# zertovitch/zip-ada

Hardware: AMD Instinct MI355X
Metric: Deflate encode MB/s (Deflate_3; stream bit-exact with the CPU restatement of the reference, Ada parity unpinned) (higher is better)
Workload: dtype u8

## Files before the change

__graft_entry__.py:

```python
import importlib
import os
import subprocess
import sys

ROOT = os.path.dirname(os.path.abspath(__file__))
if ROOT not in sys.path:
    sys.path.insert(0, ROOT)


def build():
    env = dict(os.environ)
    subprocess.run(["make", "-C", os.path.join(ROOT, "zip-ada_amd", "csrc"), "-j4"], check=True, env=env)
    subprocess.run(["make", "-C", os.path.join(ROOT, "oracle")], check=True, env=env)
    subprocess.run(["g++", "-O2", "-std=c++17", "-fPIC", "-shared", "-o",
                    os.path.join(ROOT, "tests", "hostcheck", "libzada_hostcheck.so"),
                    os.path.join(ROOT, "tests", "hostcheck", "hostcheck.cpp")], check=True)
    subprocess.run(["gcc", "-O2", "-fPIC", "-shared", "-o", os.path.join(ROOT, "tests", "hostcheck", "libzada_mix.so"),
                    os.path.join(ROOT, "zip-ada_amd", "csrc", "silesia_mix.c"), "-lm"], check=True)
    subprocess.run(["gcc", "-O2", "-fPIC", "-shared", "-o", os.path.join(ROOT, "tests", "crypt", "libcrypt_model.so"),
                    os.path.join(ROOT, "tests", "crypt", "crypt_model.c")], check=True)
    subprocess.run(["g++", "-O2", "-std=c++17", "-fPIC", "-shared", "-o", os.path.join(ROOT, "tests", "inflate", "libinflate_host.so"),
                    os.path.join(ROOT, "tests", "inflate", "inflate_host.cpp")], check=True)
    subprocess.run(["g++", "-O2", "-std=c++17", "-fPIC", "-shared", "-o", os.path.join(ROOT, "tests", "inflate_par", "libinflate_par_host.so"),
                    os.path.join(ROOT, "tests", "inflate_par", "inflate_par_host.cpp")], check=True)
    subprocess.run(["g++", "-O2", "-std=c++17", "-fPIC", "-shared", "-o", os.path.join(ROOT, "tests", "bunzip2", "libbunzip2_host.so"),
                    os.path.join(ROOT, "tests", "bunzip2", "bunzip2_host.cpp")], check=True)
    subprocess.run(["g++", "-O2", "-std=c++17", "-fPIC", "-shared", "-o", os.path.join(ROOT, "tests", "unlzma", "libunlzma_host.so"),
                    os.path.join(ROOT, "tests", "unlzma", "unlzma_host.cpp")], check=True)
    subprocess.run(["g++", "-O2", "-std=c++17", "-fPIC", "-shared", "-o", os.path.join(ROOT, "tests", "unzip", "libunzip_plan_host.so"),
                    os.path.join(ROOT, "tests", "unzip", "unzip_plan_host.cpp")], check=True)
    subprocess.run(["g++", "-O2", "-std=c++17", "-fPIC", "-shared", "-o", os.path.join(ROOT, "tests", "zip", "libzip_plan_host.so"),
                    os.path.join(ROOT, "tests", "zip", "zip_plan_host.cpp")], check=True)
    subprocess.run(["g++", "-O2", "-std=c++17", "-fPIC", "-shared", "-o", os.path.join(ROOT, "tests", "zip", "libzip_plan_ex_host.so"),
                    os.path.join(ROOT, "tests", "zip", "zip_plan_ex_host.cpp")], check=True)
    subprocess.run(["g++", "-O2", "-std=c++17", "-fPIC", "-shared", "-o", os.path.join(ROOT, "tests", "rezip", "librezip_plan_host.so"),
                    os.path.join(ROOT, "tests", "rezip", "rezip_plan_host.cpp")], check=True)
    subprocess.run(["g++", "-O2", "-std=c++17", "-fPIC", "-shared", "-o", os.path.join(ROOT, "tests", "find", "libfind_plan_host.so"),
                    os.path.join(ROOT, "tests", "find", "find_plan_host.cpp")], check=True)
    subprocess.run(["g++", "-O2", "-std=c++17", "-fPIC", "-shared", "-o", os.path.join(ROOT, "tests", "trained", "libtrained_host.so"),
                    os.path.join(ROOT, "tests", "trained", "trained_host.cpp")], check=True)
    for name in ("shrink_model", "reduce_model"):
        subprocess.run(["gcc", "-O2", "-fPIC", "-shared", "-o", os.path.join(ROOT, "tests", "legacy", "lib%s.so" % name),
                        os.path.join(ROOT, "tests", "legacy", name + ".c")], check=True)
    subprocess.run(["g++", "-O2", "-std=c++17", "-fPIC", "-shared", "-o", os.path.join(ROOT, "tests", "unlegacy", "libunlegacy_host.so"),
                    os.path.join(ROOT, "tests", "unlegacy", "unlegacy_host.cpp")], check=True)
    subprocess.run(["g++", "-O2", "-std=c++17", "-fPIC", "-shared", "-o", os.path.join(ROOT, "tests", "unlegacy", "libunzip_legacy_plan_host.so"),
                    os.path.join(ROOT, "tests", "unlegacy", "unzip_legacy_plan_host.cpp")], check=True)
    subprocess.run(["gcc", "-O2", "-fPIC", "-shared", "-o", os.path.join(ROOT, "tests", "unlegacy", "libunlegacy_model.so"),
                    os.path.join(ROOT, "tests", "unlegacy", "unlegacy_model.c")], check=True)
    subprocess.run(["g++", "-O2", "-std=c++17", "-fPIC", "-shared", "-o", os.path.join(ROOT, "tests", "zip_legacy", "libzip_legacy_plan_host.so"),
                    os.path.join(ROOT, "tests", "zip_legacy", "zip_legacy_plan_host.cpp")], check=True)
    za = importlib.import_module("zip-ada_amd")
    za.load_library()
    return None


def smoke():
    import zlib
    sys.path.insert(0, os.path.join(ROOT, "tests"))
    from _common import oracle_deflate
    za = importlib.import_module("zip-ada_amd")
    enc = za.Encoder(0)
    for n, mask in ((1 << 20, 0x1F), (1 << 20, 1), (1, 1), (0, 1)):
        d = za.silesia_mix(n, class_mask=mask).tobytes()
        for method in (za.Method.Deflate_3, za.Method.Deflate_1):
            rc, ref, crc = oracle_deflate(d, method)
            try:
                out, c2 = enc.deflate(d, method)
                rc2 = 0
            except za.CompressionInefficient:
                rc2, out, c2 = 1, b"", crc
            assert rc == rc2, (n, method, rc, rc2)
            if rc == 0:
                assert out == ref, "GPU stream differs from the oracle (n=%d method=%d)" % (n, method)
                assert zlib.decompress(out, -15) == d
            assert c2 == crc
    datas = [za.silesia_mix(k, class_mask=1).tobytes() for k in (0, 1, 5000, 40000, 70000)]
    for d, (rc2, out, c2) in zip(datas, enc.deflate_batch(datas, za.Method.Deflate_1)):
        rc, ref, crc = oracle_deflate(d, za.Method.Deflate_1)
        assert rc == rc2 and crc == c2 and (rc != 0 or out == ref), "batch entry differs from the oracle (n=%d)" % len(d)
    packed = [(d, out, c2) for d, (rc2, out, c2) in zip(datas, enc.deflate_batch(datas, za.Method.Deflate_1)) if rc2 == 0]
    assert len(packed) >= 3
    for (d, out, c2), (rc, back, _, used, reg) in zip(packed, enc.inflate_batch([p[1] for p in packed], [len(p[0]) for p in packed])):
        assert rc == 0 and back == d and used == len(out) and reg == c2, "inflated entry differs from the input (n=%d)" % len(d)
    d = za.silesia_mix(1 << 20).tobytes()
    s, c2 = enc.deflate(d, za.Method.Deflate_3)
    enc.set_knob("inflate_par_chunk_kib", 16)
    assert enc.inflate_par(s, len(d)) == (d, len(s), c2), "stream read back on many waves differs from the input"
    assert enc.inflate_par_last()["fell_back"] == 0 and enc.inflate_par_last()["live_chunks"] >= 2, "the stream did not run on many waves"
    enc.set_knob("inflate_par_chunk_kib", 64)
    import bz2
    from _bzip2 import oracle_encode
    d = za.silesia_mix(1 << 20).tobytes()
    ref, blocks = oracle_encode(d, 2)
    rc, out, crc = enc.bzip2(d, 14)
    assert rc == 0 and out == ref and enc.bz2_last_blocks() == blocks, "GPU BZip2 stream differs from the oracle"
    assert bz2.decompress(out) == d and (crc ^ 0xFFFFFFFF) == zlib.crc32(d)
    back, used, reg = enc.bunzip2(out, len(d))
    assert back == d and used == len(out) and reg == crc, "BZip2 stream read back differs from the input"
    from _lzmah import oracle_lzma, lzma_decode
    datas = [d[i * 6000:i * 6000 + k] for i, k in enumerate((0, 1, 300, 6000, 6000, 6000))]
    for e, got in zip(datas, enc.lzma_batch(datas, 18)):
        assert got == oracle_lzma(e, 18), "GPU LZMA payload differs from the oracle (n=%d)" % len(e)
        assert lzma_decode(got[1], 4) == e
    packed = enc.lzma_batch(datas, 18)
    for e, p, (rc, back, _, used, reg) in zip(datas, packed, enc.unlzma_batch([p[1] for p in packed], [len(e) for e in datas], True)):
        assert rc == 0 and back == e and used == len(p[1]) and reg == p[2], "LZMA entry read back differs from the input (n=%d)" % len(e)
    enc.set_knob("lzma_chunk", 3000)
    seen = []
    assert enc.lzma(d[:20000], 18, feedback=lambda pct: seen.append(pct) and False) == oracle_lzma(d[:20000], 18), "chunked LZMA stream differs from the oracle"
    assert seen[0] == 0 and seen[-1] == 100 and seen == sorted(seen) and len(seen) > 5
    from _crypt import compress_data_pw
    h11 = bytes(range(1, 12))
    for e in (d[:300000], d[:1], b""):
        want, crc, zt, _ = compress_data_pw(e, za.Method.Deflate_3, "smoke", h11)
        assert enc.compress_data(e, za.Method.Deflate_3, password="smoke", header=h11) == (want, crc, zt), "encrypted payload differs from the model (n=%d)" % len(e)
    import io
    import zipfile
    b = io.BytesIO()
    with zipfile.ZipFile(b, "w", zipfile.ZIP_DEFLATED) as z:
        z.writestr("a.txt", d[:40000])
        z.writestr("b.txt", b"x" + d[1000:1020].lower())
    r = za.FindZip(enc).find(b.getvalue(), b" X" + d[1000:1008])
    assert [(e[4], e[1], e[2]) for e in r.entries] == [(b"a.txt", 0, 40000), (b"b.txt", 1, 8)] and r.damaged == 0, "Find_Zip on the device differs from the host's search"
    from _trained import message_of, stub_of
    tc = za.TrainedCompression(enc, d[:20000])
    msgs = tc.encode([d[20000:23000], b""])
    assert tc.stub == stub_of(d[:20000]) and msgs == [message_of(d[:20000], e, tc.skip) for e in (d[20000:23000], b"")], "trained messages differ from the oracle"
    td = za.TrainedCompression.for_decoding(enc, tc.stub, tc.skip, tc.trainer_len)
    assert td.decode(msgs, [3000, 0]) == [d[20000:23000], b""] and td.info()["forked"] == 2, "trained messages read back differ from the data"
    tc.close(); td.close()
    from _legacy import model_result
    datas = [d[:6000], d[6000:6300] * 20, d[:1], b""]
    assert enc.shrink_batch(datas) == [(r, s if r == 0 else None, c) for r, s, c in (model_result(e, za.Method.Shrink_1) for e in datas)], "Shrink_1 batch differs from the model"
    assert enc.reduce_batch(datas, za.Method.Reduce_4) == [(r, s if r == 0 else None, c) for r, s, c in (model_result(e, za.Method.Reduce_4) for e in datas)], "Reduce_4 batch differs from the model"
    packed = [(e, s, 1) for e, (r, s, _) in zip(datas, enc.shrink_batch(datas)) if r == 0] + [(e, s, 5) for e, (r, s, _) in zip(datas, enc.reduce_batch(datas, za.Method.Reduce_4)) if r == 0]
    assert len(packed) >= 3
    for (e, s, m), (rc, back, _, used, reg) in zip(packed, enc.unlegacy_batch([p[1] for p in packed], [len(p[0]) for p in packed], [p[2] for p in packed])):
        assert rc == 0 and back == e and used == len(s) and reg == zlib.crc32(e) ^ 0xFFFFFFFF, "Shrink / Reduce entry read back differs from the input (n=%d)" % len(e)
    enc.close()
    print("smoke ok")
    return None


if __name__ == "__main__":
    build()
    if len(sys.argv) > 1 and sys.argv[1] == "smoke":
        smoke()
```

zip-ada_amd/csrc/zada_api.hip:

```cpp
#include <hip/hip_runtime.h>
#include <stdint.h>
#include <stdio.h>
#include <string.h>
#include <algorithm>
#include <new>
#include <atomic>
#include <mutex>
#include <condition_variable>
#include <functional>
#include <thread>
#include "../../include/zada.h"
#include "zada_internal.h"
#include "zada_bt4.h"
#include "zada_legacy.h"

struct zada_ctx { zada::Ctx c; };

namespace zada {

thread_local std::string *tls_err = nullptr;
int hip_check(Ctx *c, hipError_t e, const char *what) {
  if (e == hipSuccess) return 0;
  char buf[256];
  snprintf(buf, sizeof buf, "%s: %s", what, hipGetErrorString(e));
  if (tls_err) *tls_err = buf; else c->err = buf;
  return ZADA_E_HIP_;
}

void Ctx::tbegin() {
  marks.clear();
  timing.clear();
}
void Ctx::tmark(const char *name) {
  if (!timing_on) return;
  size_t k = marks.size();
  if (k >= ev_pool.size()) { hipEvent_t e; hipEventCreate(&e); ev_pool.push_back(e); }
  hipEventRecord(ev_pool[k], stream);
  marks.push_back({name, ev_pool[k]});
}
void Ctx::tend() {
  if (!timing_on || marks.empty()) return;
  hipEventSynchronize(marks.back().second);
  for (size_t i = 1; i < marks.size(); i++) {
    float ms = 0;
    hipEventElapsedTime(&ms, marks[i - 1].second, marks[i].second);
    timing.push_back({marks[i].first, ms});
  }
  timing.push_back({"#demand_rounds", (float)demand_rounds});
  timing.push_back({"#splice_rounds", (float)parse_rounds});
  timing.push_back({"#bt4_reruns", (float)bt4_reruns});
  timing.push_back({"#lzma_launches", (float)lzma_launches});
  timing.push_back({"#bt4_pool_grown", (float)bt4_pool_grown});
  timing.push_back({"#atoms_grown", (float)atoms_grown});
  timing.push_back({"#fix_grown", (float)fix_grown});
}

#ifndef ZADA_COPY_LANES
#define ZADA_COPY_LANES 4
#endif
constexpr int ARR_LANES = ZADA_COPY_LANES;
struct Arrival {
  Ctx *c; const uint8_t *src; uint8_t *dst; uint64_t n; int T;
  std::vector<std::thread> th;
  std::mutex m; std::condition_variable cv;
  uint64_t sent[ARR_LANES] = {};
  bool failed = false;
  void lane(int t) {
    hipSetDevice(c->device);
    uint64_t i = 0;
    for (uint64_t o = (uint64_t)t * STAGE_BYTES; o < n; o += (uint64_t)T * STAGE_BYTES, i++) {
      const int b = 2 * t + (int)(i & 1);
      if (i >= 2) hipEventSynchronize(c->ev_stage[b]);
      const uint64_t k = n - o < STAGE_BYTES ? n - o : STAGE_BYTES;
      memcpy(c->stage[b], src + o, k);
      const bool ok = hipMemcpyAsync(dst + o, c->stage[b], k, hipMemcpyHostToDevice, c->stream_in[t]) == hipSuccess &&
                      hipEventRecord(c->ev_stage[b], c->stream_in[t]) == hipSuccess;
      std::lock_guard<std::mutex> g(m);
      if (!ok || hipEventRecord(c->ev_in[t], c->stream_in[t]) != hipSuccess) failed = true;
      sent[t]++;
      cv.notify_all();
    }
  }
  void start() { for (int t = 0; t < T; t++) th.emplace_back([this, t] { lane(t); }); }
  void join() { for (auto &x : th) if (x.joinable()) x.join(); th.clear(); }
  ~Arrival() { join(); }
};
static bool ensure_arrival_streams(Ctx *c) {
  for (int t = 0; t < ARR_LANES; t++) {
    if (c->stream_in[t]) continue;
    if (hipStreamCreateWithFlags(&c->stream_in[t], hipStreamNonBlocking) != hipSuccess || hipEventCreateWithFlags(&c->ev_in[t], hipEventDisableTiming) != hipSuccess) {
      (void)hipGetLastError();
      return false;
    }
  }
  return true;
}
static int arrival_order(Ctx *c, hipStream_t st, uint64_t upto) {
  Arrival *A = (Arrival *)c->arrival;
  if (!A) return 0;
  if (upto > A->n) upto = A->n;
  const uint64_t P = (upto + STAGE_BYTES - 1) / STAGE_BYTES;
  std::unique_lock<std::mutex> g(A->m);
  for (int t = 0; t < A->T; t++) {
    const uint64_t want = P > (uint64_t)t ? (P - 1 - t) / A->T + 1 : 0;
    if (want == 0) continue;
    A->cv.wait(g, [&] { return A->sent[t] >= want || A->failed; });
    if (A->failed) { c->err = "host to device copy of the input"; return ZADA_E_HIP; }
    if (hipStreamWaitEvent(st, c->ev_in[t], 0) != hipSuccess) { c->err = "hipStreamWaitEvent (input arrival)"; return ZADA_E_HIP; }
  }
  return 0;
}


template <typename T>
static int dalloc(Ctx *c, std::vector<void *> &group, T **p, uint64_t count) {
  void *q = nullptr;
  hipError_t e = hipMalloc(&q, count * sizeof(T) + 256);
  if (e != hipSuccess) { hip_check(c, e, "hipMalloc"); (void)hipGetLastError(); return ZADA_E_NOMEM; }
  group.push_back(q);
  *p = (T *)q;
  return 0;
}

static void free_group(std::vector<void *> &group) {
  for (void *p : group) hipFree(p);
  group.clear();
}

int ensure_lz_workspace(Ctx *c, uint64_t nbuf) {
  Workspace &W = c->ws;
  if (W.cap_n >= nbuf && W.cap_n > 0) return 0;
  hipStreamSynchronize(c->stream); hipStreamSynchronize(c->stream2);
  free_group(W.allocs);
  W.cap_n = 0;
  uint64_t cap = nbuf < (1u << 20) ? (1u << 20) : nbuf;
  cap = (cap + 65535) & ~65535ull;
  const uint64_t nch = cap / PCHUNK + 2, nseg32 = cap / 32768 + 2;
  int rc = 0;
#define A(ptr, cnt) if (!rc) rc = dalloc(c, W.allocs, &W.ptr, (cnt))
#define A2(ptr, cnt) if (!rc) rc = dalloc(c, W.allocs, &ptr, (cnt))
  A(in, cap + IN_PAD + 64);
  static_assert(NLEVELS >= 2, "spec_tok shares the block of ltails[0], S3, T3, bsc3: the first level's tails table must be dead when the first parse starts");
  {
    const uint64_t b_tails0 = nseg32 * 65536 * 2, b_s3 = nseg32 * 32768 * 2, b_t3 = nseg32 * 32768, b_bsc = nseg32 * 32768 * 4, b_spec = nch * (uint64_t)PTOK_STRIDE * 4;
    const uint64_t links = b_tails0 + b_s3 + b_t3 + b_bsc + 1024, bytes = links > b_spec ? links : b_spec;
    uint8_t *blk = nullptr;
    A2(blk, bytes);
    if (!rc) {
      uint8_t *q = blk;
      W.ltails[0] = (uint16_t *)q; q += b_tails0 + 256;
      W.S3 = (uint16_t *)q; q += b_s3 + 256;
      W.bsc3 = (uint32_t *)q; q += b_bsc + 256;
      W.T3 = q;
      W.spec_tok = (uint32_t *)blk;
    }
  }
  for (int l = 0; l < NLEVELS; l++) { A(lprev[l], cap + IN_PAD); if (l > 0) A(ltails[l], nseg32 * 65536); }
  A(segmax, nseg32 + 16); A(heavy, nseg32 * 2048);
  A(bloom4, nseg32 * 4096);
  W.cd_cap = cap / 256 + 4096; A(cd_list, W.cd_cap + W.cd_cap / 4);
  for (int l = 0; l < NLEVELS; l++) A(dplane[l], cap + 64);
  A(dlim, cap + 64); A(dlim_bits, cap / 32 + 64);
  A(M, cap + 64);
  A(SK, nseg32 * 32768); A(idxK, cap + 64); A(cntK, cap + 64);
  W.fix_stride = c->knob_fix_stride > 0 ? (uint32_t)c->knob_fix_stride : FIX_STRIDE_SMALL;
  if (W.fix_stride > PTOK_STRIDE) W.fix_stride = PTOK_STRIDE;
  A(fix_tok, nch * W.fix_stride);
  A(spec_cnt, nch); A(fix_cnt, nch); A(take_from, nch); A(start_pos, nch); A(counts, nch); A(offsets, nch);
  A(scan_sums, nch / 1024 + 1024);
  A(Fbits, cap / 32 + 64); A(Lbits, cap / 32 + 64);
  A(spec_exits, nch); A(true_exits, nch);
  A(dirty[0], nch + 64); A(dirty[1], nch + 64);
  A(n_changed, 16);
  A(blk_demand, cap / 4096 + 64); A(dbits, cap / 32 + 4096); A(n_demand, 16); A(chg, nch + 64);
  A(dbg, 128);
#undef A
#undef A2
  if (rc) { free_group(W.allocs); return rc; }
  W.cap_n = cap;
  hipMemsetAsync(W.dbg, 0, 128 * 8, c->stream);
  return hip_check(c, hipStreamSynchronize(c->stream), "workspace init");
}

int ensure_entropy_workspace(Ctx *c, uint64_t atoms, uint64_t flushes, uint64_t out_bytes) {
  Workspace &W = c->ws;
  const EntropyRoom room = sizing_entropy_room(EntropyRequest{atoms, out_bytes});
  if (out_bytes < atoms) out_bytes = atoms;
  if (W.cap_atoms >= atoms && W.cap_flush >= flushes && W.cap_atoms > 0 && W.cap_out >= room.out_need) return 0;
  hipStreamSynchronize(c->stream); hipStreamSynchronize(c->stream2);
  free_group(W.en_allocs);
  W.cap_atoms = 0; W.cap_flush = 0;
  const uint64_t cap = room.cap_atoms;
  const uint64_t nflush = (cap / FLUSH > flushes ? cap / FLUSH : flushes + flushes / 4) + 3;
  int rc = 0;
#define A(ptr, cnt) if (!rc) rc = dalloc(c, W.en_allocs, &W.ptr, (cnt))
  A(ea_atoms, LB_CAP + cap + LA_CAP + 64); A(ea_apos, LB_CAP + cap + LA_CAP + 64);
  A(descr, nflush * SLOTS * 320);
  A(seg_nblk, nflush); A(seg_cut, nflush * MAXBLK_PER_SEG); A(seg_blk_off, nflush);
  A(cut_trace, nflush * SLOTS * 2);
  W.cap_blocks = nflush * MAXBLK_PER_SEG;
  A(blocks, W.cap_blocks);
  A(binfo, W.cap_blocks);
  A(emit, W.cap_blocks);
  A(chrec, W.cap_blocks * 16 + 16);
  A(chw, W.cap_blocks * 4 + 16); A(piece_base, W.cap_blocks + 16);
  A(codes, (W.cap_blocks + 2) * 320);
  W.cap_pieces = cap / 2048 + W.cap_blocks + 64;
  A(pieces, W.cap_pieces);
  W.cap_tiles = cap / TILE + W.cap_blocks + 64;
  A(tile_block, W.cap_tiles); A(tile_bitpos, W.cap_tiles); A(tile_bits, W.cap_tiles);
  A(blk_entry, W.cap_blocks + 16);
  A(chooser, 1); A(carry, 2);
  A(scan2, nflush / 1024 + 1024); A(total2, 16);
  W.cap_out = room.cap_out;
  A(out, W.cap_out);
#undef A
  if (!rc) rc = ensure_crc_workspace(c, out_bytes > cap ? out_bytes : cap);
  if (rc) { free_group(W.en_allocs); return rc; }
  W.cap_atoms = cap; W.cap_flush = nflush - 3;
  return 0;
}

int ensure_crc_workspace(Ctx *c, uint64_t n) {
  Workspace &W = c->ws;
  if (W.cap_crc >= n && W.cap_crc > 0) return 0;
  hipStreamSynchronize(c->stream); hipStreamSynchronize(c->stream2);
  free_group(W.crc_allocs);
  W.cap_crc = 0;
  const uint64_t cap = ((n < (1u << 20) ? (1u << 20) : n) + 65535) & ~65535ull;
  int rc = 0;
  for (int l = 0; l < 4 && !rc; l++) rc = dalloc(c, W.crc_allocs, &W.crc_lvl[l], (cap >> (4 * l)) / CRC_SUB + 64);
  if (!rc) rc = dalloc(c, W.crc_allocs, &W.crc_mat, 128);
  W.crc_mat_ready = false;
  if (rc) { free_group(W.crc_allocs); return rc; }
  W.cap_crc = cap;
  return 0;
}

int ensure_batch_workspace(Ctx *c, uint64_t entries, uint64_t fslots, uint64_t segs) {
  Workspace &W = c->ws;
  if (W.cap_ent >= entries && W.cap_fslots >= fslots && W.cap_bseg >= segs && W.cap_ent > 0) return 0;
  hipStreamSynchronize(c->stream); hipStreamSynchronize(c->stream2);
  free_group(W.bt_allocs);
  W.cap_ent = W.cap_fslots = W.cap_bseg = 0;
  const uint64_t ce = entries + entries / 4 + 1024, cf = fslots + fslots / 4 + 1024, cs = segs + segs / 4 + 1024;
  int rc = 0;
#define A(ptr, cnt) if (!rc) rc = dalloc(c, W.bt_allocs, &W.ptr, (cnt))
  A(ftab, cf); A(ent_out, ce);
  A(ent_chunk0, ce + 1); A(ent_fl0, ce + 1); A(ent_start, ce + 1); A(ent_len, ce + 1); A(ent_bytes, ce + 1); A(ent_base, ce + 1); A(ent_crc, ce + 1);
  A(segend, cs + 1);
#undef A
  if (rc) { free_group(W.bt_allocs); return rc; }
  W.cap_ent = ce; W.cap_fslots = cf; W.cap_bseg = cs;
  return 0;
}

static int ensure_rin(Ctx *c, uint64_t n) {
  Workspace &W = c->ws;
  if (W.cap_rin >= n && W.rin_own) return 0;
  hipStreamSynchronize(c->stream); hipStreamSynchronize(c->stream2);
  if (W.rin_own) hipFree(W.rin_own);
  W.rin_own = nullptr; W.cap_rin = 0;
  const uint64_t cap = ((n < (1u << 20) ? (1u << 20) : n) + 65535) & ~65535ull;
  if (hipMalloc((void **)&W.rin_own, cap + 256) != hipSuccess) { (void)hipGetLastError(); c->err = "hipMalloc (input)"; return ZADA_E_NOMEM; }
  W.cap_rin = cap;
  return 0;
}

static void free_workspace(Ctx *c) {
  free_group(c->ws.allocs); free_group(c->ws.en_allocs); free_group(c->ws.bt_allocs); free_group(c->ws.crc_allocs);
  if (c->ws.rin_own) hipFree(c->ws.rin_own);
  c->ws = Workspace();
}

constexpr int CRC_WG = 64, CRC_ROW = CRC_SUB + 16;
__global__ void __launch_bounds__(CRC_WG) k_crc_chunks(const uint8_t *__restrict__ in, uint64_t n, uint32_t nsub, uint32_t *__restrict__ sub) {
  __shared__ uint32_t tab[256];
  __shared__ __attribute__((aligned(16))) uint8_t rows[CRC_WG * CRC_ROW];
  for (uint32_t t = threadIdx.x; t < 256; t += CRC_WG) {
    uint32_t l = t;
    for (int b = 0; b < 8; b++) l = (l & 1) ? (l >> 1) ^ 0xEDB88320u : l >> 1;
    tab[t] = l;
  }
  const uint64_t tile0 = (uint64_t)blockIdx.x * CRC_WG * CRC_SUB;
  {
    const uint4 *src = (const uint4 *)(in + tile0);
    const uint64_t left = tile0 < n ? n - tile0 : 0, words = left / 16;
#pragma unroll
    for (int j = 0; j < CRC_SUB / 16; j++) {
      const uint32_t wq = j * CRC_WG + threadIdx.x;
      if (wq < words) *(uint4 *)(rows + (wq >> 4) * CRC_ROW + (wq & 15) * 16) = src[wq];
    }
    if (words < (uint64_t)CRC_WG * CRC_SUB / 16 && threadIdx.x < (left & 15)) {
      const uint64_t o = words * 16 + threadIdx.x;
      rows[(o / CRC_SUB) * CRC_ROW + (o % CRC_SUB)] = in[tile0 + o];
    }
  }
  __syncthreads();
  uint32_t k = blockIdx.x * CRC_WG + threadIdx.x;
  if (k >= nsub) return;
  uint64_t p0 = (uint64_t)k * CRC_SUB, p1 = p0 + CRC_SUB < n ? p0 + CRC_SUB : n;
  uint32_t r = 0;
  const uint8_t *row = rows + threadIdx.x * CRC_ROW;
  const uint4 *w = (const uint4 *)row;
  uint64_t len = p1 - p0, i = 0;
  for (; i + 16 <= len; i += 16) {
    const uint4 v = w[i >> 4];
    const uint32_t xs[4] = {v.x, v.y, v.z, v.w};
#pragma unroll
    for (int q = 0; q < 4; q++) {
      uint32_t x = xs[q];
      r = tab[(r ^ x) & 0xFF] ^ (r >> 8); x >>= 8;
      r = tab[(r ^ x) & 0xFF] ^ (r >> 8); x >>= 8;
      r = tab[(r ^ x) & 0xFF] ^ (r >> 8); x >>= 8;
      r = tab[(r ^ x) & 0xFF] ^ (r >> 8);
    }
  }
  for (; i < len; i++) r = tab[(r ^ row[i]) & 0xFF] ^ (r >> 8);
  sub[k] = r;
}

__global__ void __launch_bounds__(256) k_crc_fold(const uint32_t *__restrict__ src, uint32_t ngroups, const uint32_t *__restrict__ mat,
                                                  uint32_t *__restrict__ out) {
  __shared__ uint32_t m[32];
  if (threadIdx.x < 32) m[threadIdx.x] = mat[threadIdx.x];
  __syncthreads();
  uint32_t k = blockIdx.x * 256 + threadIdx.x;
  if (k >= ngroups) return;
  uint32_t r = 0;
  for (uint32_t j = 0; j < 16; j++) {
    uint32_t s = 0, v = r;
    for (int b = 0; v; b++, v >>= 1) if (v & 1) s ^= m[b];
    r = s ^ src[k * 16 + j];
  }
  out[k] = r;
}

static void gf2_square(uint32_t *sq, const uint32_t *m) {
  for (int i = 0; i < 32; i++) { uint32_t v = m[i], s = 0; for (int j = 0; v; j++, v >>= 1) if (v & 1) s ^= m[j]; sq[i] = s; }
}
static uint32_t gf2_apply(const uint32_t *m, uint32_t v) { uint32_t s = 0; for (int j = 0; v; j++, v >>= 1) if (v & 1) s ^= m[j]; return s; }
static void zero_advance_matrix(uint64_t len, uint32_t *out) {
  uint32_t op[32], tmp[32], acc[32];
  op[0] = 0xEDB88320u;
  for (int i = 1; i < 32; i++) op[i] = 1u << (i - 1);
  for (int i = 0; i < 32; i++) acc[i] = 1u << i;
  uint64_t bits = len * 8;
  while (bits) {
    if (bits & 1) { for (int i = 0; i < 32; i++) tmp[i] = gf2_apply(op, acc[i]); memcpy(acc, tmp, sizeof acc); }
    gf2_square(tmp, op); memcpy(op, tmp, sizeof op);
    bits >>= 1;
  }
  memcpy(out, acc, sizeof acc);
}

constexpr int CRC_NLEV = 4;
static uint32_t crc_M[CRC_NLEV][32];
int crc_launch(Ctx *c, const uint8_t *d_in, uint64_t n) {
  if (n == 0) return 0;
  Workspace &W = c->ws;
  CrcPending &P = c->crc;
  static std::once_flag mats;
  std::call_once(mats, [] { for (int l = 0; l < CRC_NLEV; l++) zero_advance_matrix((uint64_t)CRC_SUB << (4 * l), crc_M[l]); });
  hipStream_t s2 = c->stream2;
  hipEventRecord(c->ev_input, c->stream);
  hipStreamWaitEvent(s2, c->ev_input, 0);
  P.nsub = (uint32_t)((n + CRC_SUB - 1) / CRC_SUB);
  P.nfull0 = (uint32_t)(n / CRC_SUB);
  P.cnt[0] = P.nfull0;
  for (int l = 1; l < CRC_NLEV; l++) P.cnt[l] = P.cnt[l - 1] / 16;
  if (!W.crc_mat_ready) { hipMemcpyAsync(W.crc_mat, crc_M, sizeof(uint32_t) * 32 * (CRC_NLEV - 1), hipMemcpyHostToDevice, s2); W.crc_mat_ready = true; }
  hipLaunchKernelGGL(k_crc_chunks, dim3((P.nsub + CRC_WG - 1) / CRC_WG), dim3(CRC_WG), 0, s2, d_in, n, P.nsub, W.crc_lvl[0]);
  for (int l = 1; l < CRC_NLEV; l++)
    if (P.cnt[l]) hipLaunchKernelGGL(k_crc_fold, dim3((P.cnt[l] + 255) / 256), dim3(256), 0, s2, W.crc_lvl[l - 1], P.cnt[l], W.crc_mat + 32 * (l - 1), W.crc_lvl[l]);
  if (P.cnt[CRC_NLEV - 1] > CRC_HOST_TOP) { c->err = "crc: too many top-level values"; return ZADA_E_TOO_LARGE; }
  if (P.cnt[CRC_NLEV - 1]) hipMemcpyAsync(c->crc_host, W.crc_lvl[CRC_NLEV - 1], (size_t)P.cnt[CRC_NLEV - 1] * 4, hipMemcpyDeviceToHost, s2);
  for (int l = 0; l < CRC_NLEV - 1; l++) {
    const uint32_t first = P.cnt[l + 1] * 16;
    P.nrest[l] = (l == 0 ? P.nsub : P.cnt[l]) - first;
    if (P.nrest[l]) hipMemcpyAsync(c->crc_host + CRC_HOST_TOP + 16 * l, W.crc_lvl[l] + first, (size_t)P.nrest[l] * 4, hipMemcpyDeviceToHost, s2);
  }
  return hip_check(c, hipGetLastError(), "crc launch");
}

int crc_finish(Ctx *c, uint64_t n, uint32_t *crc_inout) {
  if (n == 0) return 0;
  constexpr int NLEV = CRC_NLEV;
  CrcPending &P = c->crc;
  const uint32_t *cnt = P.cnt, *nrest = P.nrest;
  const uint32_t nfull0 = P.nfull0;
  const uint32_t *top = c->crc_host; const uint32_t (*rest)[16] = (const uint32_t (*)[16])(c->crc_host + CRC_HOST_TOP); auto &M = crc_M;
  if (hip_check(c, hipStreamSynchronize(c->stream2), "crc")) return ZADA_E_HIP_;
  uint32_t r = *crc_inout;
  for (uint32_t k = 0; k < cnt[NLEV - 1]; k++) r = gf2_apply(M[NLEV - 1], r) ^ top[k];
  for (int l = NLEV - 2; l >= 0; l--) {
    for (uint32_t j = 0; j < nrest[l]; j++) {
      if (l == 0 && cnt[1] * 16 + j == nfull0) {
        uint32_t Ml[32];
        zero_advance_matrix(n - (uint64_t)nfull0 * CRC_SUB, Ml);
        r = gf2_apply(Ml, r) ^ rest[0][j];
      } else r = gf2_apply(M[l], r) ^ rest[l][j];
    }
  }
  *crc_inout = r;
  return 0;
}

static int method_level(int method) {
  switch (method) {
    case ZADA_DEFLATE_FIXED: return 4;
    case ZADA_DEFLATE_0: return 0;
    case ZADA_DEFLATE_1: return 6;
    case ZADA_DEFLATE_2: return 8;
    case ZADA_DEFLATE_3: return 10;
    case ZADA_DEFLATE_R: return RICH_LEVEL;
    default: return -1;
  }
}

uint32_t crc32_advance(uint32_t reg, uint64_t len) {
  if (len == 0) return reg;
  uint32_t m[32];
  zero_advance_matrix(len, m);
  return gf2_apply(m, reg);
}

constexpr uint32_t SHARD_HALO = 32768, SHARD_TAIL = 4096;
constexpr uint64_t RANGE_POST = 1u << 20;

__global__ void __launch_bounds__(256) k_copy16(const uint4 *__restrict__ src, uint4 *__restrict__ dst, uint64_t n16) {
  const uint64_t stride = (uint64_t)gridDim.x * 256;
  uint64_t i = (uint64_t)blockIdx.x * 256 + threadIdx.x;
  for (; i + 3 * stride < n16; i += 4 * stride) {
    const uint4 a = src[i], b = src[i + stride], c = src[i + 2 * stride], d = src[i + 3 * stride];
    dst[i] = a; dst[i + stride] = b; dst[i + 2 * stride] = c; dst[i + 3 * stride] = d;
  }
  for (; i < n16; i += stride) dst[i] = src[i];
}

struct PadArgs { uint8_t *in_end; uint32_t n_in; uint16_t *link_end[NLEVELS]; };
__global__ void k_pad_init(PadArgs a) {
  for (uint32_t i = threadIdx.x; i < a.n_in; i += blockDim.x) a.in_end[i] = 0;
  for (int l = 0; l < NLEVELS; l++)
    if (threadIdx.x < 64) a.link_end[l][threadIdx.x] = 0;
}

int range_open(Ctx *c, int method, const uint8_t *rin, uint64_t stream_size, uint64_t lo, uint64_t n, uint64_t pre, uint64_t post, uint64_t carry_atoms = 0) {
  const int level = method_level(method);
  if (level < 0) { c->err = "unsupported method"; return ZADA_E_INVALID; }
  if (lo + n > stream_size || n > stream_size) { c->err = "range outside the stream"; return ZADA_E_INVALID; }
  const uint64_t behind = stream_size - (lo + n);
  const bool pre_ok = pre == (lo > 0 ? SHARD_HALO : 0u) || (carry_atoms > 0 && pre <= lo && pre >= SHARD_HALO && (pre % 32768) == 0) || (lo > 0 && pre == 65536);
  if (!pre_ok || post != (behind < RANGE_POST ? behind : RANGE_POST) ||
      (lo % 65536) != 0 || (behind > 0 && (n % 65536) != 0) || (behind > 0 && n == 0)) {
    c->err = "range: boundaries must be multiples of 64 KiB, with 32 KiB before and min(1 MiB, rest of the stream) behind it resident";
    return ZADA_E_INVALID;
  }
  if (pre + n + post >= (1ull << 32) - (1ull << 26)) { c->err = "range too large for one context (4 GiB - 64 MiB): split the stream into ranges"; return ZADA_E_TOO_LARGE; }
  if (((uintptr_t)rin & 15) != 0) { c->err = "range: input must be 16-byte aligned"; return ZADA_E_INVALID; }
  const uint64_t shard = (uint64_t)c->knob_shard_kib << 10;
  const EntropyRequest want = sizing_range_request(n, sizing_pct(c->knob_atoms_pct), carry_atoms);
  int rc = ensure_entropy_workspace(c, want.atoms, 0, want.out_bytes);
  if (!rc) rc = ensure_lz_workspace(c, (n < shard ? n : shard) + SHARD_HALO + SHARD_TAIL);
  if (rc) return rc;
  Range &R = c->rg;
  R = Range();
// ... 2050 lines not shown
```

zip-ada_amd/csrc/zada_internal.h:

```cpp
#pragma once
#ifndef ZADA_NLEVELS
#define ZADA_NLEVELS 2
#endif
#include <hip/hip_runtime.h>
#include <stdint.h>
#include <string>
#include <functional>
#include <vector>
#include "zada_logic.h"
#include "zada_sizing.h"

struct zada_inflate_par_info;

namespace zada {

constexpr int ZADA_E_HIP_ = -3;

#ifndef ZADA_PCHUNK
#define ZADA_PCHUNK 512
#endif
constexpr uint32_t PCHUNK = ZADA_PCHUNK;
static_assert(PCHUNK > 258, "k_fix_forward: a 258-byte step crosses at most one chunk boundary");
constexpr uint32_t PTOK_STRIDE = PCHUNK + 640;
constexpr uint32_t FIX_STRIDE_SMALL = 128;
constexpr uint32_t CRC_CHUNK = 4096, CRC_SUB = 256;
constexpr uint64_t IN_PAD = 1024;

constexpr int NLEVELS = ZADA_NLEVELS;
struct LevelPtrs { uint16_t *prev[NLEVELS]; uint16_t *tails[NLEVELS]; };
struct RunPtrs { uint16_t *S, *idx, *cnt; };
struct DistPlanes {
  uint16_t *d[NLEVELS]; uint32_t *dlim; uint32_t *dlim_bits;
  __device__ __forceinline__ uint32_t limits(uint64_t p) const { return ((dlim_bits[p >> 5] >> (p & 31)) & 1u) ? dlim[p] : 0xFFFFFFFFu; }
};

constexpr uint32_t FLUSH = 65536;
static_assert(FLUSH == SIZING_FLUSH, "zada_sizing.h books the carried atoms by the flush");
constexpr uint32_t MIN_STEP = 750, HALF_SLIDER = 2048, SLIDER = 4096;
constexpr uint32_t SLOTS = 88;
constexpr uint32_t MAXBLK_PER_SEG = 86;
constexpr uint32_t TILE = 2048;

enum { FMT_STORED = 0, FMT_FIXED = 1, FMT_DYN1 = 2, FMT_DYN2 = 3, FMT_RECYCLE = 4 };
enum { BT_STORED = 0, BT_FIXED = 1, BT_DYNAMIC = 2, BT_RESERVED = 3 };

struct BlockRange { uint32_t first, count; uint32_t last_flush; uint32_t pad; };

struct BlockInfo {
  uint32_t stats[320];
  uint8_t bl1[320], bl2[320];
  uint8_t truc1[20], truc2[20];
  uint32_t hdr1_bits, hdr2_bits;
  uint64_t fixed_data, dyn1_data, dyn2_data;
  uint32_t bytes;
  uint32_t stored_possible;
};

struct EmitRec {
  uint64_t hdr_bitpos;
  uint64_t data_bitpos;
  uint64_t cost_bits;
  uint32_t fmt;
  int32_t code_block;
  uint32_t code_variant;
  uint32_t tile_base;
  uint64_t pre_pos;
  uint32_t pre_eob;
  uint32_t pre_flags;
};
constexpr int32_t CODE_FIXED = -1, CODE_CARRIED = -2;

struct StoredPiece { uint64_t dst_byte; uint32_t src_byte, nbytes; };

struct ChooserCarry {
  uint64_t pos;
  int32_t last_type, block_to_finish, last_marked;
  uint32_t cur_eob;
  uint8_t bl[320];
  uint32_t pad[2];
};
static_assert(sizeof(ChooserCarry) == 352, "ChooserCarry is exchanged between ranks as bytes");

struct ChooserOut {
  uint64_t total_bits;
  uint32_t n_tiles, n_pieces, n_blocks, overflow;
};

struct FlushGeom {
  uint32_t F, to;
  uint32_t gj;
  uint32_t flags;
  uint32_t end_byte;
  uint32_t entry;
  uint32_t pad[2];
};
enum { FG_EMPTY = 1, FG_LAST_PARTIAL = 2, FG_ENTRY_FIRST = 4, FG_ENTRY_LAST = 8 };
enum { BR_LAST_FLUSH = 1, BR_ENTRY_FIRST = 2, BR_ENTRY_LAST = 4 };
struct EntOut {
  uint64_t bits;
  uint32_t eob;
  uint32_t fake;
};

struct EntropyView {
  const FlushGeom *ftab;
  const uint32_t *atoms, *apos;
  uint32_t foff;
  uint32_t nflush;
  uint32_t lvalid;
  uint32_t stream_final;
  uint64_t j0;
};

constexpr uint32_t LB_CAP = HALF_SLIDER, LA_CAP = FLUSH;

struct Workspace {
  uint64_t cap_n = 0;
  uint8_t *in = nullptr;
  uint16_t *lprev[NLEVELS] = {}, *ltails[NLEVELS] = {};
  uint16_t *S3 = nullptr; uint8_t *T3 = nullptr; uint32_t *bsc3 = nullptr;
  uint32_t *segmax = nullptr;
  uint16_t *heavy = nullptr;
  uint32_t *bloom4 = nullptr;
  uint32_t *cd_list = nullptr; uint64_t cd_cap = 0;
  uint16_t *dplane[NLEVELS] = {}; uint32_t *dlim = nullptr, *dlim_bits = nullptr;
  uint16_t *SK = nullptr, *idxK = nullptr, *cntK = nullptr;
  MatchPair *M = nullptr;
  uint32_t *spec_tok = nullptr, *fix_tok = nullptr;
  uint32_t fix_stride = 0;
  uint32_t *spec_cnt = nullptr, *fix_cnt = nullptr, *take_from = nullptr, *start_pos = nullptr;
  uint32_t *counts = nullptr, *offsets = nullptr, *scan_sums = nullptr;
  uint32_t *Fbits = nullptr, *Lbits = nullptr;
  ExitState *spec_exits = nullptr, *true_exits = nullptr;
  uint8_t *dirty[2] = {nullptr, nullptr};
  uint32_t *n_changed = nullptr;
  uint32_t *blk_demand = nullptr, *n_demand = nullptr;
  uint32_t *dbits = nullptr;
  uint8_t *chg = nullptr;
  uint32_t *crc_lvl[4] = {nullptr, nullptr, nullptr, nullptr}, *crc_mat = nullptr;
  bool crc_mat_ready = false;
  uint64_t *dbg = nullptr;
  std::vector<void *> allocs;
  uint64_t cap_atoms = 0, cap_flush = 0;
  uint32_t *ea_atoms = nullptr, *ea_apos = nullptr;
  uint8_t *descr = nullptr;
  uint32_t *seg_nblk = nullptr, *seg_cut = nullptr, *seg_blk_off = nullptr;
  uint32_t *cut_trace = nullptr;
  BlockRange *blocks = nullptr;
  BlockInfo *binfo = nullptr;
  EmitRec *emit = nullptr;
  uint64_t *chrec = nullptr;
  uint64_t *chw = nullptr;
  uint32_t *piece_base = nullptr;
  uint32_t *codes = nullptr;
  StoredPiece *pieces = nullptr;
  uint32_t *tile_block = nullptr;
  uint64_t *tile_bitpos = nullptr;
  uint32_t *tile_bits = nullptr;
  ChooserOut *chooser = nullptr;
  ChooserCarry *carry = nullptr;
  uint32_t *scan2 = nullptr, *total2 = nullptr;
  uint64_t cap_blocks = 0, cap_tiles = 0, cap_pieces = 0;
  uint32_t *blk_entry = nullptr;
  std::vector<void *> en_allocs;
  std::vector<void *> crc_allocs;
  uint64_t cap_crc = 0;
  uint64_t cap_ent = 0, cap_fslots = 0, cap_bseg = 0;
  FlushGeom *ftab = nullptr;
  EntOut *ent_out = nullptr;
  uint32_t *ent_chunk0 = nullptr, *ent_fl0 = nullptr, *ent_start = nullptr, *ent_len = nullptr, *ent_bytes = nullptr, *ent_base = nullptr, *ent_crc = nullptr;
  uint32_t *segend = nullptr;
  std::vector<void *> bt_allocs;
  uint8_t *rin_own = nullptr; uint64_t cap_rin = 0;
  uint8_t *out = nullptr; uint64_t cap_out = 0;
};

struct GlobalState { uint64_t pos; uint32_t kind, pad; };
struct Range {
  bool open = false;
  bool batch = false;
  uint32_t n_entries = 0;
  const uint8_t *rin = nullptr;
  uint64_t lo = 0, pre = 0, n = 0, post = 0;
  bool first = true, last = true;
  int method = 0, level = 0;
  uint64_t T = 0;
  uint64_t T_carried = 0;
  uint64_t T_view = ~0ull;
  uint32_t n_lb = 0, n_la = 0;
  GlobalState exit{}, warm{};
  bool entry_known = true;
  uint64_t G = 0, T_total = 0;
  bool placed = false;
  uint32_t nflush = 0, foff = 0, nblocks = 0;
  uint64_t j0 = 0;
  uint64_t base_bits = 0;
  ChooserCarry carry_in{}, carry_out{};
  ChooserOut co{};
  bool analyzed = false, chosen = false;
  uint32_t crc_raw = 0;
};

constexpr uint32_t CRC_HOST_TOP = 4096;
struct CrcPending { uint32_t nsub = 0, nfull0 = 0, cnt[4] = {0, 0, 0, 0}, nrest[4] = {0, 0, 0, 0}; };

constexpr uint64_t STAGE_BYTES = 8ull << 20;
constexpr int MAX_COPY_LANES = 8;
struct Ctx {
  int device = 0;
  hipStream_t stream = nullptr, stream2 = nullptr;
  hipStream_t stream_in[MAX_COPY_LANES] = {};
  hipEvent_t ev_in[MAX_COPY_LANES] = {};
  void *arrival = nullptr;
  hipEvent_t ev_input = nullptr, ev_out = nullptr, ev_dlim = nullptr;
  CrcPending crc;
  uint32_t *crc_host = nullptr;
  uint8_t *stage[2 * MAX_COPY_LANES] = {};
  uint8_t *bstage = nullptr; uint64_t cap_bstage = 0;
  uint32_t *btab = nullptr; uint64_t cap_btab = 0;
  hipEvent_t ev_stage[2 * MAX_COPY_LANES] = {};
  Workspace ws;
  Range rg;
  std::string err;
  int parse_rounds = 0, demand_rounds = 0;
  int atoms_grown = 0, fix_grown = 0;
  bool lz_attrs_set = false;
  void *bz = nullptr;
  void *zc = nullptr;
  void *inf = nullptr;
  void *infp = nullptr;
  int knob_infp_chunk_kib = 64;
  int knob_infp_repair_pct = 25;
  int knob_infp_min_kib = 0;
  void *bzd = nullptr;
  void *ulz = nullptr;
  void *ulg = nullptr;
  void *uz = nullptr;
  void *zw = nullptr;
  void *rz = nullptr;
  void *fz = nullptr;
  void *lg = nullptr;
  int knob_reduce_group_mib = 4096;
  int knob_unzip_legacy = 0;
  int knob_zip_legacy = 0;
  int knob_unzip_piece = 14;
  void *lz_tab = nullptr; size_t cap_lz_tab = 0;
  void *lz_save = nullptr; size_t cap_lz_save = 0;
  void *lz_lit = nullptr; size_t cap_lz_lit = 0;
  bool lz_last_lit_hbm = false;
  int knob_lzma_lit_mib = 12288;
  int lzma_launches = 0;
  std::vector<uint8_t> lz_resume;
  bool lz_stopped = false;
  bool lz_run_stopped = false;
  uint64_t lz_last_n = 0, lz_last_out_off = 0;
  void *bt4 = nullptr;
  uint32_t bt4_buckets = 0, bt4_long = 0, bt4_overflow = 0;
  uint32_t bt4_pool_grown = 0;
  int knob_lzma_pool_fixed = 0;
  uint32_t bt4_reruns = 0;
  int knob_trained_fork = 1;
  int knob_lzma_waves = 0;
  int knob_lzma_segment = 0;
  int knob_lzma_pool = 0;
  std::vector<hipEvent_t> ev_pool;
  std::vector<std::pair<const char *, hipEvent_t>> marks;
  std::vector<std::pair<const char *, float>> timing;
  bool timing_on = true;
  uint32_t last_nblocks = 0;
  int knob_budget = -1;
  int knob_max_demand_rounds = 12;
  int knob_atoms_pct = 50;
  int knob_fix_stride = 0;
  int knob_cd_list_cap = 0;
  int knob_cd_filter = 1;
  int knob_exact_respec = 32768;
  int knob_bz_pipe_prio = 0;
  int knob_link_run = 0;
  int knob_inner_budget = 0;
  int knob_span_mib = 2048;
  int knob_batch_mib = 512;
  int knob_bunzip_batch_mib = 8192;
  int knob_bz_batch_mib = 256;
  int knob_bz_span_mib = 1024;
  int knob_bz_text_order = 1;
  int knob_bz_tail_pct = 0;
  int knob_bz_batch_melems = 768;
  int knob_bz_lists = -1;
  int knob_bz_pipeline = 1;
  int knob_bz_list_rows = 0;
  int knob_bz_split = 1;
  int knob_bz_small_wg = 1;
  int knob_lzma_dict = 0;
  int knob_lzma_chunk = 0;
  int knob_shard_kib = 1 << 20;
  void tmark(const char *name);
  void tbegin();
  void tend();
};

extern thread_local std::string *tls_err;
int hip_check(Ctx *c, hipError_t e, const char *what);
constexpr const char *ERR_OUTPUT_TOO_SMALL = "output buffer too small";
void bz2_destroy(Ctx *c);
void crypt_destroy(Ctx *c);
void inflate_destroy(Ctx *c);
int inflate_crc_entries(Ctx *c, uint32_t E, const uint64_t *out, const uint64_t *out_len, uint32_t *regs);
void inflate_par_destroy(Ctx *c);
int inflate_par_try(Ctx *c, int format, const void *d_in, uint64_t n_in, void *d_out, uint64_t cap, uint64_t *out_len, uint64_t *in_used, uint32_t *crc_inout);
void inflate_par_record(Ctx *c, ::zada_inflate_par_info *get, const ::zada_inflate_par_info *set);
void bunzip2_destroy(Ctx *c);
void unlzma_destroy(Ctx *c);
void unlegacy_destroy(Ctx *c);
void unzip_destroy(Ctx *c);
void zip_destroy(Ctx *c);
void rezip_destroy(Ctx *c);
void find_destroy(Ctx *c);
int unzip_store_entries(Ctx *c, uint32_t ns, const uint64_t *src, const uint64_t *dst, const uint64_t *len, uint32_t *crc);
struct ReaderJob { uint64_t in, out, n_in, cap; int32_t format; uint32_t eos; uint64_t lit_elems; int32_t index, pad; };
struct ReaderRes { int32_t rc; uint32_t crc; uint64_t out_len, in_used; };
int inflate_run_jobs(Ctx *c, uint32_t E, const ReaderJob *jobs, ReaderRes *res, bool *described);
int bunzip2_run_jobs(Ctx *c, uint32_t E, const ReaderJob *jobs, ReaderRes *res, bool *described);
int unlzma_run_jobs(Ctx *c, uint32_t E, const ReaderJob *jobs, ReaderRes *res, bool *described);
uint64_t unlzma_hbm_elems(const uint8_t *h9, uint64_t n_in);
int unlegacy_run_jobs(Ctx *c, uint32_t E, const ReaderJob *jobs, ReaderRes *res, bool *described);
struct UlzTrainedJob { uint64_t in, out, n_in, cap; };
struct UlzResult;
uint64_t unlzma_snap_bytes();
int unlzma_snap_info(const uint8_t *snap, uint64_t *in_pos, uint64_t *out_pos, uint64_t *lit_elems);
int unlzma_trained_launch(Ctx *c, const UlzTrainedJob *d_jobs, const uint32_t *d_order, uint32_t E, UlzResult *d_res, const void *d_start, void *d_stop, uint64_t stop_in);
int lzma_plain_stream(Ctx *c, const uint8_t *in, uint64_t n, uint8_t *out, uint64_t cap, uint64_t *out_len, uint32_t dictionary_size, bool end_marker);
void crypt_update_keys(uint32_t keys[3], uint8_t by);
uint8_t crypt_code(const uint32_t keys[3]);
constexpr uint64_t CRYPT_WAVE_MAX = 256u << 10;
int crypt_io(Ctx *c, uint64_t bytes, uint8_t **p);
int crypt_encode_device(Ctx *c, uint32_t keys[3], uint8_t *d_buf, uint64_t n);
struct ZcPlaceJob { uint64_t src, dst, len; uint32_t keys[3], pad; };
int crypt_encode_place(Ctx *c, uint32_t E, const ZcPlaceJob *jobs);
int crypt_encode_small(Ctx *c, const int *idx, uint32_t E, uint32_t (*keys)[3], uint8_t *const *buf, const uint64_t *n);
int bz2_encode_device(Ctx *c, int option, const uint8_t *d_in, uint64_t n, int64_t size_hint, uint8_t *d_out, uint64_t cap, uint64_t *out_len,
                      int (*fb)(int, void *), void *user);
uint64_t bz2_last_blocks(Ctx *c, uint64_t *dst, uint64_t cap_items);
int bz2_batch_encode(Ctx *c, int option, const uint8_t *d_arena, uint32_t E, const uint64_t *starts, const uint32_t *lens, uint8_t *h_out, uint64_t cap,
                     uint64_t *out_off, uint64_t *out_bytes, uint8_t **d_streams = nullptr);
int bz2_range_open(Ctx *c, int option, const uint8_t *d_buf, uint64_t buf_len, uint64_t buf_off, uint64_t stream_total, uint64_t start, uint64_t own_end,
                   uint64_t *next_start, uint64_t *nblocks);
int bz2_range_encode(Ctx *c);
uint64_t bz2_range_table(Ctx *c, uint64_t *tab, uint64_t cap_blocks);
int bz2_range_assemble(Ctx *c, const uint8_t *choice, uint64_t nblk, uint64_t bit_begin, int flags, uint32_t footer_crc, uint8_t *d_out, uint64_t cap, uint64_t *nbytes);
struct LzmaJob {
  uint64_t in_off, n;
  uint64_t tok_off, ntok;
  uint64_t out_off, cap;
  uint64_t verify;
  uint32_t sbs, hash4_size;
  int32_t level, zip_prefix;
  int32_t lc, lp, pb;
  int32_t lit_home;
  uint64_t lit_off;
};
struct Bt4Sets { const uint8_t *cnt; const uint16_t *sl; const uint32_t *sd; const uint16_t *ol; const uint32_t *od; };
int bt4_produce(Ctx *c, const std::vector<LzmaJob> &jobs, const uint8_t *d_arena, uint64_t arena_bytes, Bt4Sets *out, std::vector<uint32_t> *weights = nullptr,
                uint32_t seg_shift = 32, uint32_t *nseg = nullptr);
int bt4_walk_segment(Ctx *c, uint32_t k, hipStream_t st);
int bt4_segments_overflowed(Ctx *c, hipStream_t st, Bt4Sets *out = nullptr);
void bt4_destroy(Ctx *c);
uint32_t lzma_string_buffer_size(int level, uint64_t dictionary_size);
uint32_t lzma_hash4_size(uint32_t sbs);
int lzma_token_ranges(Ctx *c, uint32_t E, const uint32_t *d_apos, uint32_t T, const uint32_t *d_ent_start, LzmaJob *d_jobs);
int lzma_launch(Ctx *c, const LzmaJob *d_jobs, const uint32_t *d_order, uint32_t count, const uint8_t *d_in, const uint32_t *d_tok, uint8_t *d_out, const Bt4Sets &sets, uint64_t *d_result,
                uint8_t *d_save = nullptr, uint64_t budget = 0, uint64_t pos_cap = ~0ull, int waves = 1, int lit_home = 0, uint16_t *d_lit = nullptr);
uint64_t lzma_save_stride();
struct LzFork { const uint8_t *d_snap, *d_head; uint64_t head_len; const uint8_t *d_forked; };
int lzma_fork_fill(Ctx *c, const LzmaJob *d_jobs, uint32_t count, const uint8_t *d_forked, const uint8_t *d_snap, const uint8_t *d_head, uint64_t head_len, uint8_t *d_save,
                   uint8_t *d_out);
int lzma_fork_snapshot(Ctx *c, const uint8_t *d_in, uint64_t n, uint64_t pos_cap, uint32_t dictionary_size, uint8_t *d_out, uint64_t cap, uint8_t *d_snap, uint64_t *pos,
                       uint64_t *olen);
int lzma_save_info(const uint8_t *blob, uint64_t *pos, uint64_t *olen, uint64_t *n);
int lzma_save_fits(const uint8_t *blob, const LzmaJob &J);
int ensure_lz_workspace(Ctx *c, uint64_t nbuf);
int ensure_entropy_workspace(Ctx *c, uint64_t atoms, uint64_t flushes, uint64_t out_bytes = 0);
int ensure_crc_workspace(Ctx *c, uint64_t n);

struct ShardJob {
  uint64_t nbuf = 0;
  uint32_t tok_lo = 0, tok_hi = 0;
  bool final = false;
  bool entry_known = true;
  ExitState entry{0, SYNC_F};
  uint32_t *dst_atoms = nullptr, *dst_apos = nullptr;
  uint32_t apos_bias = 0;
  uint64_t cap_atoms = 0;
  std::function<int(uint64_t, uint32_t **, uint32_t **)> grow_atoms;
  const uint32_t *segend = nullptr;
  std::function<int(uint64_t)> need;
  uint64_t gpos = 0;
};
struct ShardResult { uint32_t ntok = 0; ExitState exit{0, SYNC_F}, warm{0, SYNC_F}; };
int lz_shard(Ctx *c, int level, const ShardJob &job, ShardResult *res);
constexpr int RICH_LEVEL = 11;
int rich_shard(Ctx *c, const ShardJob &job, ShardResult *res);

int ensure_batch_workspace(Ctx *c, uint64_t entries, uint64_t fslots, uint64_t segs);
struct BatchLayout { uint32_t E = 0, nseg = 0; uint64_t total = 0, nfs = 0; std::vector<uint32_t> start, len; };
int batch_layout(Ctx *c, uint32_t E, const uint64_t *n, const uint32_t *crc_in, BatchLayout &L);
void batch_segends_all(Ctx *c, const BatchLayout &L);
int batch_launch(Ctx *c, int method, const BatchLayout &L, uint64_t *obytes, uint32_t **h_bytes, uint32_t **h_base, uint32_t **h_crc);
int deflate_device_one(Ctx *c, int method, const void *d_in, uint64_t n, void *d_out, uint64_t cap, uint64_t *out_len, uint32_t *crc_inout);
int bzip2_device_one(Ctx *c, int method, const void *d_in, uint64_t n, void *d_out, uint64_t cap, uint64_t *out_len, uint32_t *crc_inout);
int lzma_device_one(Ctx *c, int method, const void *d_in, uint64_t n, void *d_out, uint64_t cap, uint64_t *out_len, uint32_t *crc_inout);
struct DevBatch {
  uint32_t E = 0;
  int kind = 0;
  uint64_t total = 0, ototal = 0, nfs = 0;
  uint8_t *d_in = nullptr, *d_out = nullptr;
  std::vector<uint64_t> start, off, bytes, cap;
  std::vector<uint32_t> len, reg;
  std::vector<uint8_t> refused;
  const LzFork *fork = nullptr;
};
int bzip2_batch_layout(Ctx *c, int method, uint32_t E, const uint64_t *n, const uint32_t *crc_in, DevBatch &D);
int bzip2_batch_launch(Ctx *c, int method, DevBatch &D, uint8_t *h_out, uint64_t h_cap);
int lzma_batch_layout(Ctx *c, int method, uint32_t E, const uint64_t *n, const uint32_t *crc_in, DevBatch &D);
int lzma_batch_launch(Ctx *c, int method, DevBatch &D);
int legacy_batch_layout(Ctx *c, uint32_t E, const uint64_t *n, const uint32_t *crc_in, DevBatch &D);
int legacy_batch_launch(Ctx *c, int method, DevBatch &D);
bool lzma_batch_refused(Ctx *c, const DevBatch &D);
int batch_geometry(Ctx *c, uint32_t E, const uint32_t *d_total_atoms);
int entropy_analyze(Ctx *c);
int entropy_choose(Ctx *c);
// ... 10 lines not shown
```

zip-ada_amd/csrc/zada_logic.h:

```cpp
#pragma once
#include <type_traits>
#include <stdint.h>

#if defined(__HIPCC__)
#define ZADA_HD __host__ __device__ __forceinline__
#else
#define ZADA_HD inline
#endif

namespace zada {

constexpr uint32_t TOK_MATCH = 0x80000000u;
ZADA_HD uint32_t tok_match(uint32_t len, uint32_t dist) { return TOK_MATCH | (len << 16) | dist; }
ZADA_HD bool tok_is_match(uint32_t t) { return (t & TOK_MATCH) != 0; }
ZADA_HD uint32_t tok_len(uint32_t t) { return tok_is_match(t) ? ((t >> 16) & 0x1FF) : 1u; }
ZADA_HD uint32_t tok_dist(uint32_t t) { return t & 0xFFFF; }

constexpr int MIN_MATCH = 3, MAX_MATCH = 258, MAX_DIST = 32506, TOO_FAR = 4096;
constexpr int WSIZE = 32768;

struct LzConfig { int good, lazy, nice, chain; };
ZADA_HD LzConfig lz_config(int level) {
  switch (level) {
    case 4: return {4, 4, 16, 16};
    case 5: return {8, 16, 32, 32};
    case 6: return {8, 16, 128, 128};
    case 7: return {8, 32, 128, 256};
    case 8: return {32, 128, 258, 1024};
    case 9: return {32, 258, 258, 4096};
    default: return {34, 258, 258, 4096};
  }
}

ZADA_HD int clz32(uint32_t x) {
#if defined(__HIP_DEVICE_COMPILE__)
  return __clz((int)x);
#else
  return x ? __builtin_clz(x) : 32;
#endif
}

ZADA_HD int len_symbol(int len) {
  if (len == 258) return 285;
  int l = len - 3;
  if (l < 8) return 257 + l;
  int k = 31 - clz32((uint32_t)l);
  return 257 + 4 * (k - 1) + ((l >> (k - 2)) & 3);
}
ZADA_HD int len_extra_bits(int len) {
  if (len == 258) return 0;
  int l = len - 3;
  if (l < 8) return 0;
  return 31 - clz32((uint32_t)l) - 2;
}
ZADA_HD uint32_t len_extra_val(int len) { int e = len_extra_bits(len); return (uint32_t)(len - 3) & ((1u << e) - 1); }
ZADA_HD int dist_symbol(int dist) {
  if (dist <= 4) return dist - 1;
  uint32_t d = (uint32_t)dist - 1;
  int k = 31 - clz32(d);
  return 2 * k + (int)((d >> (k - 1)) & 1);
}
ZADA_HD int dist_extra_bits(int dist) {
  if (dist <= 4) return 0;
  return 31 - clz32((uint32_t)dist - 1) - 1;
}
ZADA_HD uint32_t dist_extra_val(int dist) { int e = dist_extra_bits(dist); return ((uint32_t)dist - 1) & ((1u << e) - 1); }
ZADA_HD int litlen_sym_extra(int sym) { return (sym < 265 || sym == 285) ? 0 : (sym - 261) / 4; }
ZADA_HD int dist_sym_extra(int sym) { return sym < 4 ? 0 : (sym >> 1) - 1; }
ZADA_HD int fixed_litlen_bl(int i) { return i <= 143 ? 8 : i <= 255 ? 9 : i <= 279 ? 7 : 8; }

struct ParseState { uint32_t p; uint32_t avail; uint32_t mlen; uint32_t mdist; };

enum { SYNC_NONE = 0, SYNC_F = 1, SYNC_L = 2 };
ZADA_HD int sync_kind(const ParseState &s) { return !s.avail ? SYNC_F : (s.mlen == 2 ? SYNC_L : SYNC_NONE); }

ZADA_HD bool parse_need_quarter(const ParseState &s, const LzConfig &c) { return (int)s.mlen >= c.good; }
ZADA_HD bool parse_searches(const ParseState &s, const LzConfig &c, uint64_t la) { return la >= 3 && (int)s.mlen < c.lazy; }

ZADA_HD uint32_t parse_step(ParseState &s, uint32_t mfq, bool searched, uint32_t byte_before) {
  const uint32_t L0 = s.mlen, pd = s.mdist;
  bool improved = false;
  uint32_t ml = 2, md = s.mdist;
  if (searched) {
    uint32_t len = mfq >> 16, dist = mfq & 0xFFFF;
    if (len > L0) { improved = true; ml = len; md = dist; if (ml == 3 && dist > (uint32_t)TOO_FAR) ml = 2; }
  }
  if (L0 >= 3 && !improved) {
    uint32_t t = tok_match(L0, pd);
    s.p += L0 - 1; s.avail = 0; s.mlen = 2; s.mdist = 0;
    return t;
  }
  s.mlen = ml; s.mdist = md; s.p += 1;
  if (s.avail) return byte_before;
  s.avail = 1;
  return 0xFFFFFFFFu;
}


struct MatchPair { uint32_t full, quarter; };
constexpr uint32_t M_GUESS = 0x80000000u, M_DEMAND = 0x40000000u, M_BYSPEC = 0x20000000u, M_HAVEQ = 0x10000000u, M_VALUE = 0x01FFFFFFu;
constexpr uint32_t M_BEAT_SHIFT = 25, M_BEAT_MAX = 127;
struct NoGuess { ZADA_HD void operator()(uint32_t, uint32_t, uint32_t, uint32_t) const {} };
struct ParseIO { const uint8_t *in; uint64_t n; const MatchPair *M; LzConfig cfg; const uint32_t *segend; };
struct Layout { const uint32_t *segend; uint64_t n; };
struct ExitState { uint32_t pos, kind; };

struct BitmapWriter {
  uint32_t *bits; uint64_t word; uint32_t acc;
  ZADA_HD void init(uint32_t *b, uint64_t first) { bits = b; acc = 0; word = first; }
  ZADA_HD void set(uint64_t p) {
    uint64_t w = p >> 5;
    while (word < w) { bits[word] = acc; acc = 0; word++; }
    acc |= 1u << (p & 31);
  }
  ZADA_HD void finish(uint64_t last) {
    while (word < last) { bits[word] = acc; acc = 0; word++; }
    bits[word] = acc;
  }
};

struct DirectFetch { const MatchPair *M; ZADA_HD MatchPair operator()(uint32_t p) const { return M[p]; } };
template <typename F> struct has_byte { template <typename U> static auto test(int) -> decltype(((U *)0)->byte(0u), char()); template <typename U> static long test(...); static const bool value = sizeof(test<F>(0)) == 1; };
template <typename F> ZADA_HD typename std::enable_if<has_byte<typename std::remove_reference<F>::type>::value, uint32_t>::type fetch_byte(F &f, const uint8_t *, uint32_t p) { return f.byte(p); }
template <typename F> ZADA_HD typename std::enable_if<!has_byte<typename std::remove_reference<F>::type>::value, uint32_t>::type fetch_byte(F &, const uint8_t *in, uint32_t p) { return in[p]; }
struct DirectSink { uint32_t *tok; uint32_t &ntok; ZADA_HD void push(uint32_t t) { tok[ntok++] = t; } };
struct CappedSink { uint32_t *tok; uint32_t &ntok; uint32_t cap; uint32_t *overflow; ZADA_HD void push(uint32_t t) { if (ntok < cap) tok[ntok] = t; else if (overflow) *overflow = 1u; ntok++; } };
template <typename Sink, typename OnTop, typename OnGuess, typename Fetch>
ZADA_HD void run_parser(ParseState &s, const ParseIO &io, Sink &&sink, OnTop &&on_top, OnGuess &&on_guess, Fetch &&fetch) {
  for (;;) {
    if ((uint64_t)s.p >= io.n) {
      if (s.avail) { sink.push(io.in[io.n - 1]); s.avail = 0; s.mlen = 2; }
      return;
    }
    if (on_top(s)) return;
    const uint64_t la = io.n - s.p;
    const bool srch = parse_searches(s, io.cfg, la);
    uint32_t m = 0;
    if (srch) {
      const MatchPair mm = fetch(s.p);
      if (mm.full & M_GUESS) on_guess(s.p, mm.full, mm.quarter, s.mlen);
      m = (parse_need_quarter(s, io.cfg) ? mm.quarter : mm.full) & M_VALUE;
    }
    const uint32_t bb = s.avail ? fetch_byte(fetch, io.in, s.p - 1) : 0;
    const uint32_t t = parse_step(s, m, srch, bb);
    if (t != 0xFFFFFFFFu) sink.push(t);
  }
}

template <typename Sink, typename OnGuess, typename Fetch>
ZADA_HD void parse_spec_chunk_to(const ParseIO &io, uint32_t k, uint32_t chunk, Sink &&sink,
                                 uint32_t *Fbits, uint32_t *Lbits, ExitState &ex, OnGuess on_guess, Fetch &&fetch) {
  const uint64_t c0 = (uint64_t)k * chunk, c1 = (c0 + chunk < io.n) ? c0 + chunk : io.n;
  ParseState s{(uint32_t)c0, 0, 2, 0};
  BitmapWriter fw, lw;
  fw.init(Fbits, c0 >> 5); lw.init(Lbits, c0 >> 5);
  ExitState e; e.pos = (uint32_t)io.n; e.kind = SYNC_F;
  run_parser(s, io, sink, [&](const ParseState &st) {
    int kind = sync_kind(st);
    if (kind == SYNC_NONE) return false;
    if ((uint64_t)st.p >= c1) { e.pos = st.p; e.kind = (uint32_t)kind; return true; }
    if (kind == SYNC_F) fw.set(st.p); else lw.set(st.p);
    return false;
  }, on_guess, fetch);
  const uint64_t lastw = c1 > c0 ? (c1 - 1) >> 5 : c0 >> 5;
  fw.finish(lastw);
  lw.finish(lastw);
  ex = e;
}
template <typename OnGuess, typename Fetch>
ZADA_HD void parse_spec_chunk(const ParseIO &io, uint32_t k, uint32_t chunk, uint32_t *tok, uint32_t &ntok,
                              uint32_t *Fbits, uint32_t *Lbits, ExitState &ex, OnGuess on_guess, Fetch &&fetch) {
  parse_spec_chunk_to(io, k, chunk, DirectSink{tok, ntok}, Fbits, Lbits, ex, on_guess, fetch);
}
ZADA_HD void parse_spec_chunk(const ParseIO &io, uint32_t k, uint32_t chunk, uint32_t *tok, uint32_t &ntok,
                              uint32_t *Fbits, uint32_t *Lbits, ExitState &ex) {
  parse_spec_chunk_to(io, k, chunk, DirectSink{tok, ntok}, Fbits, Lbits, ex, NoGuess(), DirectFetch{io.M});
}

template <typename OnGuess, typename Fetch>
ZADA_HD void parse_fix_chunk(const ParseIO &io, uint32_t k, uint32_t chunk, ExitState entry,
                             const uint32_t *spec_tok, uint32_t spec_cnt, const uint32_t *Fbits, const uint32_t *Lbits,
                             ExitState spec_exit, uint32_t *tok, uint32_t &ntok, uint32_t &take, uint32_t &u0, ExitState &new_exit,
                             OnGuess on_guess, Fetch &&fetch, uint32_t tok_cap = 0xFFFFFFFFu, uint32_t *tok_overflow = nullptr) {
  const uint64_t c0 = (uint64_t)k * chunk, c1 = (c0 + chunk < io.n) ? c0 + chunk : io.n;
  u0 = entry.kind == SYNC_L ? entry.pos - 1 : entry.pos;
  ntok = 0;
  if ((uint64_t)entry.pos >= c1) {
    new_exit = entry; take = spec_cnt;
    return;
  }
  ParseState s{entry.pos, entry.kind == SYNC_L ? 1u : 0u, 2, 0};
  bool synced = false;
  ExitState e; e.pos = (uint32_t)io.n; e.kind = SYNC_F;
  run_parser(s, io, CappedSink{tok, ntok, tok_cap, tok_overflow}, [&](const ParseState &st) {
    int kind = sync_kind(st);
    if (kind == SYNC_NONE) return false;
    if ((uint64_t)st.p >= c1) { e.pos = st.p; e.kind = (uint32_t)kind; return true; }
    uint32_t wbits = (kind == SYNC_F ? Fbits : Lbits)[st.p >> 5];
    if ((wbits >> (st.p & 31)) & 1) { synced = true; e.pos = st.p; e.kind = (uint32_t)kind; return true; }
    return false;
  }, on_guess, fetch);
  if (synced) {
    const uint32_t u = e.kind == SYNC_L ? e.pos - 1 : e.pos;
    uint32_t cur = (uint32_t)c0, j = 0;
    while (cur < u) { cur += tok_len(spec_tok[j]); j++; }
    take = j;
    new_exit = spec_exit;
  } else {
    take = spec_cnt;
    new_exit = e;
  }
}
ZADA_HD void parse_fix_chunk(const ParseIO &io, uint32_t k, uint32_t chunk, ExitState entry,
                                    const uint32_t *spec_tok, uint32_t spec_cnt, const uint32_t *Fbits, const uint32_t *Lbits,
                                    ExitState spec_exit, uint32_t *tok, uint32_t &ntok, uint32_t &take, uint32_t &u0, ExitState &new_exit) {
  parse_fix_chunk(io, k, chunk, entry, spec_tok, spec_cnt, Fbits, Lbits, spec_exit, tok, ntok, take, u0, new_exit, NoGuess(), DirectFetch{io.M});
}

template <typename T>
ZADA_HD void patch_dist_stats(T *sd) {
  int used = 0;
  for (int i = 0; i < 32; i++) if (sd[i] != 0) used++;
  if (used == 0) { sd[0] = 1; sd[1] = 1; }
  else if (used == 1) { if (sd[0] == 0) sd[0] = 1; else sd[1] = 1; }
}

ZADA_HD void tweak_for_better_rle(uint32_t *counts, int counts_len, uint8_t *good) {
  int length = counts_len, stride;
  uint32_t symbol, sum, limit, new_count;
  for (int i = 0; i < counts_len; i++) good[i] = 0;
  for (;;) { if (length == 0) return; if (counts[length - 1] != 0) break; length--; }
  symbol = counts[0]; stride = 0;
  for (int i = 0; i <= length; i++) {
    if (i == length || counts[i] != symbol) {
      if ((symbol == 0 && stride >= 5) || (symbol != 0 && stride >= 7))
        for (int k = 0; k < stride; k++) good[i - k - 1] = 1;
      stride = 1;
      if (i != length) symbol = counts[i];
    } else stride++;
  }
  stride = 0; limit = counts[0]; sum = 0;
  for (int i = 0; i <= length; i++) {
    bool brk = (i == length) || good[i] || (i > 0 && good[i - 1]);
    if (!brk) { int64_t d = (int64_t)counts[i] - (int64_t)limit; if (d < 0) d = -d; brk = d >= 4; }
    if (brk) {
      if (stride >= 4 || (stride >= 3 && sum == 0)) {
        new_count = (sum + (uint32_t)stride / 2) / (uint32_t)stride;
        if (new_count < 1) new_count = 1;
        if (sum == 0) new_count = 0;
        for (int k = 0; k < stride; k++) counts[i - k - 1] = new_count;
      }
      stride = 0; sum = 0;
      if (i < length - 3) limit = (counts[i] + counts[i + 1] + counts[i + 2] + counts[i + 3] + 2) / 4;
      else if (i < length) limit = counts[i];
      else limit = 0;
    }
    stride++;
    if (i != length) sum += counts[i];
  }
}

ZADA_HD uint32_t bit_reverse(uint32_t code, int len) {
  uint32_t b = 0;
  for (int i = 0; i < len; i++) { b = (b << 1) | (code & 1); code >>= 1; }
  return b;
}
ZADA_HD void canonical_codes(const uint8_t *bl, int n, uint16_t *codes) {
  uint32_t bl_count[16], next_code[16];
  for (int i = 0; i < 16; i++) bl_count[i] = 0;
  for (int i = 0; i < n; i++) bl_count[bl[i]]++;
  bl_count[0] = 0;
  uint32_t code = 0; next_code[0] = 0;
  for (int bits = 1; bits <= 15; bits++) { code = (code + bl_count[bits - 1]) << 1; next_code[bits] = code; }
  for (int k = 0; k < n; k++) {
    int l = bl[k];
    codes[k] = l ? (uint16_t)bit_reverse(next_code[l]++, l) : 0;
  }
}

struct HeaderPlan {
  uint8_t cs_bl[320];
  uint16_t last_cs_bl;
  uint8_t hlit_m257, hdist_m1, a_non_zero;
  uint8_t truc_bl[19];
  uint32_t truc_freq[19];
  uint32_t bits;
};

template <typename Sink>
ZADA_HD void header_rle_walk(const uint8_t *cs_bl, int last, Sink &&sink) {
  int idx = 0;
  for (;;) {
    int rep = 1;
    for (int j = idx + 1; j < last; j++) { if (cs_bl[j] != cs_bl[idx]) break; rep++; }
    if (idx > 0 && cs_bl[idx] == cs_bl[idx - 1] && rep >= 3 && !(cs_bl[idx] == 0 && rep > 6)) {
      rep = rep < 6 ? rep : 6;
      sink(16, (uint32_t)(rep - 3));
      idx += rep;
    } else if (cs_bl[idx] == 0 && rep >= 3) {
      if (rep <= 10) sink(17, (uint32_t)(rep - 3));
      else { rep = rep < 138 ? rep : 138; sink(18, (uint32_t)(rep - 11)); }
      idx += rep;
    } else {
      sink((int)cs_bl[idx], 0u);
      idx++;
    }
    if (idx >= last) break;
  }
}

ZADA_HD int header_perm(int a) {
  const uint8_t perm[19] = {16, 17, 18, 0, 8, 7, 9, 6, 10, 5, 11, 4, 12, 3, 13, 2, 14, 1, 15};
  return perm[a];
}
ZADA_HD int header_extra_bits(int x) { return x == 16 ? 2 : x == 17 ? 3 : x == 18 ? 7 : 0; }

ZADA_HD int tweak_value(int bl) {
  const int16_t t[17] = {1600, 100, 255, 379, 490, 594, 694, 791, 885, 978, 1069, 1159, 1249, 1338, 1426, 1513, 1600};
  return t[bl];
}

}
```

zip-ada_amd/csrc/zada_lz.hip:

```cpp
#include <hip/hip_runtime.h>
#include <mutex>
#include <stdint.h>
#include "zada_logic.h"
#include "zada_internal.h"
#include <chrono>
#include <stdio.h>
#include <stdlib.h>
#include <vector>

namespace zada {

typedef uint32_t __attribute__((aligned(1))) u32u;
typedef uint64_t __attribute__((aligned(1))) u64u;
#define RL(v, j) ((uint32_t)__builtin_amdgcn_readlane((int)(v), (j)))
#define RL64(v, j) ((uint64_t)RL((uint32_t)(v), (j)) | ((uint64_t)RL((uint32_t)((v) >> 32), (j)) << 32))

#ifndef ZADA_NO_XCD_MAP
__device__ __forceinline__ uint32_t xcd_block() {
  const uint32_t n = gridDim.x, full = n & ~7u, b = blockIdx.x;
  return b < full ? (b & 7u) * (full >> 3) + (b >> 3) : b;
}
#else
__device__ __forceinline__ uint32_t xcd_block() { return blockIdx.x; }
#endif
// ... 636 lines not shown
#define ZADA_CD_THREADS 64
#endif
constexpr int CD_THREADS = ZADA_CD_THREADS;
#ifdef ZADA_CD_STATS
__device__ unsigned long long g_cd_dbg[16];
#endif
constexpr uint32_t BLOOM_BITS = 1u << 17, BLOOM_WORDS = BLOOM_BITS / 32;
__device__ __forceinline__ uint32_t bloom4_of(uint32_t x) { return (x * 0x85EBCA6Bu) >> 15; }
__global__ void __launch_bounds__(256) k_bloom4(const uint8_t *__restrict__ in, Layout L, uint32_t *__restrict__ bloom, uint32_t seg0) {
  __shared__ uint32_t bits[BLOOM_WORDS];
  const uint64_t seg = (uint64_t)blockIdx.x + seg0, base = seg * 32768ull;
  const uint32_t m = lay_inserted(L, seg);
  const int tid = threadIdx.x;
  for (int i = tid; i < (int)BLOOM_WORDS; i += 256) bits[i] = 0;
  __syncthreads();
  const uint32_t *w = (const uint32_t *)(in + base);
  for (uint32_t i = tid; i < 32768u / 4u; i += 256) {
    const uint32_t a = w[i], b = w[i + 1], e = 4u * i;
    const uint32_t x[4] = {a, __builtin_amdgcn_alignbyte(b, a, 1), __builtin_amdgcn_alignbyte(b, a, 2), __builtin_amdgcn_alignbyte(b, a, 3)};
#pragma unroll
    for (int j = 0; j < 4; j++) if (e + (uint32_t)j < m) { const uint32_t h = bloom4_of(x[j]); atomicOr(&bits[h >> 5], 1u << (h & 31u)); }
  }
  __syncthreads();
  uint4 *dst = (uint4 *)(bloom + seg * BLOOM_WORDS);
  for (int i = tid; i < (int)BLOOM_WORDS / 4; i += 256) dst[i] = ((const uint4 *)bits)[i];
}

struct CdTail { const uint32_t *bloom; uint32_t *list; uint32_t *count; uint32_t cap; uint32_t *list2; uint32_t *count2; uint32_t cap2; };
enum { CD_SWEEP = 0, CD_LIST = 1, CD_ALL = 2 };
#ifndef ZADA_CD_CAP
#define ZADA_CD_CAP 16
#endif
#ifndef ZADA_CD_CAP2
#define ZADA_CD_CAP2 256
#endif
constexpr uint32_t CD_CAP = ZADA_CD_CAP, CD_CAP2 = ZADA_CD_CAP2;
template <int MODE>
__global__ void __launch_bounds__(CD_THREADS) k_cross_dist(const uint8_t *__restrict__ in, Layout L, LevelPtrs lv,
                                                    const uint16_t *__restrict__ S3, const uint8_t *__restrict__ T3, const uint32_t *__restrict__ bsc3,
                                                    DistPlanes dp, uint64_t p0, uint64_t p1, CdTail tl) {
  uint64_t p = p0 + (uint64_t)blockIdx.x * blockDim.x + threadIdx.x;
  if (MODE == CD_LIST) {
    const uint32_t i = blockIdx.x * blockDim.x + threadIdx.x, nc = *tl.count, nl = nc < tl.cap ? nc : tl.cap;
    if (i >= nl) return;
    p = tl.list[i];
  }
  if (p >= p1 || p >= L.n) return;
  const uint64_t seg = p >> 15, pbase = (seg - 1) * 32768ull;
  if (lay_first(L, seg) || (uint32_t)(p & 32767u) >= lay_inserted(L, seg)) return;
  const bool prev_first = lay_first(L, seg - 1);
  const uint32_t d3_stored = dp.d[0][p];
  uint32_t dl_first[NLEVELS > 1 ? NLEVELS - 1 : 1], link_first[NLEVELS > 1 ? NLEVELS - 1 : 1];
#pragma unroll
  for (int l = 0; l + 1 < NLEVELS; l++) { dl_first[l] = dp.d[1 + l][p]; link_first[l] = lv.prev[l][p]; }
  const uint64_t mine = *(const u64u *)(in + p);
  const uint32_t far24 = (d3_stored == DIST3_HEADCHK || d3_stored == DIST3_CONT_FIRST) ? *(const u32u *)(in + p - (uint64_t)MAX_DIST) & 0xFFFFFFu : 0xFFFFFFFFu;
  bool need = d3_stored >= DIST3_CONT_FIRST;
#ifdef ZADA_CD_SKIP3
  need = false;
#endif
#pragma unroll
  for (int l = 0; l + 1 < NLEVELS; l++) need = need || (dl_first[l] & DISTL_CONTINUE) || dl_first[l] == DISTL_GAVEUP;
#ifdef ZADA_CD_SKIP4
  need = d3_stored >= DIST3_CONT_FIRST;
#endif
  if (!need) return;
  uint32_t bloom_bit = 1u;
  if (MODE == CD_SWEEP && tl.bloom && NLEVELS > 1 && (dl_first[0] & DISTL_CONTINUE)) {
    const uint32_t hb = bloom4_of((uint32_t)mine);
    bloom_bit = (tl.bloom[(seg - 1) * BLOOM_WORDS + (hb >> 5)] >> (hb & 31u)) & 1u;
  }
  uint32_t dprev = d3_stored >= DIST3_CONT_FIRST ? 0u : d3_stored;
  const uint32_t my24 = (uint32_t)mine & 0xFFFFFFu;
  const uint32_t b0 = my24 & 0xFF, b1 = (my24 >> 8) & 0xFF;
  const uint32_t h = ((b0 << 10) ^ (b1 << 5) ^ (my24 >> 16)) & 0x7FFFu;
#ifdef ZADA_CD_NOL3
  if (false) {
#else
  if (d3_stored == DIST3_CONTINUE || d3_stored == DIST3_CONT_FIRST) {
#endif
    const uint32_t bsc = bsc3[pbase + h];
    const uint32_t pst = bsc & 0xFFFF, pct = bsc >> 16;
    const uint16_t *ps = S3 + pbase;
    const uint8_t *pt = T3 + pbase;
    const uint32_t mytag = (b0 >> 5) | ((b1 & 7u) << 3) | ((b0 & 3u) << 6);
    uint32_t d3 = 0;
    const uint64_t tagx8 = 0x0101010101010101ull * mytag;
    for (uint32_t hi = pct; hi > 0 && d3 == 0;) {
      const uint32_t lo = hi >= 8 ? hi - 8 : 0;
      const uint64_t x = *(const u64u *)(pt + pst + lo) ^ tagx8;
      uint64_t z = ~(((x & 0x7F7F7F7F7F7F7F7Full) + 0x7F7F7F7F7F7F7F7Full) | x | 0x7F7F7F7F7F7F7F7Full);
      if (hi - lo < 8) z &= ~(~0ull << (8 * (hi - lo)));
      bool stop = false;
      while (z) {
        const int byte = 7 - (__builtin_clzll(z) >> 3);
        z &= ~(0xFFull << (8 * byte));
        const uint32_t j = lo + (uint32_t)byte;
        const uint64_t q = pbase + ps[pst + j], d = p - q;
        if ((prev_first && q == pbase) || d > (uint64_t)TOO_FAR) { stop = true; break; }
        if ((*(const u32u *)(in + q) & 0xFFFFFFu) == my24) { d3 = (uint32_t)d; break; }
      }
      if (stop) break;
      if (lo > 0 && p - (pbase + ps[pst + lo - 1]) > (uint64_t)TOO_FAR) break;
      hi = lo;
    }
    dprev = d3;
  }
  if (dprev == 0 && (d3_stored == DIST3_HEADCHK || d3_stored == DIST3_CONT_FIRST) && (p & 32767u) < (uint32_t)MAX_DIST) {
    const uint64_t q = p - (uint64_t)MAX_DIST;
    if (!(prev_first && q == pbase) && far24 == my24) {
      const uint32_t prv = bsc3[pbase + h];
      const bool q_last = (prv >> 16) != 0 && S3[pbase + (prv & 0xFFFF) + (prv >> 16) - 1] == (uint16_t)(q & 32767);
      if (q_last) dprev = (uint32_t)MAX_DIST;
    }
  }
  if (dprev != d3_stored) dp.d[0][p] = (uint16_t)dprev;
#pragma unroll
  for (int l = 0; l + 1 < NLEVELS; l++) {
    uint32_t dl = dl_first[l];
#ifdef ZADA_CD_NOL4
    if (false) {
#else
    if ((dl & DISTL_CONTINUE) || dl == DISTL_GAVEUP) {
#endif
      const bool gaveup = dl == DISTL_GAVEUP;
      uint64_t q = gaveup ? p : p - (dl & 0x7FFFu);
      dl = 0;
      bool may_list = (MODE == CD_SWEEP && tl.list != nullptr) || (MODE == CD_LIST && tl.list2 != nullptr);
      uint32_t *const o_list = MODE == CD_LIST ? tl.list2 : tl.list, *const o_count = MODE == CD_LIST ? tl.count2 : tl.count;
      const uint32_t o_cap = MODE == CD_LIST ? tl.cap2 : tl.cap, step_cap = MODE == CD_LIST ? CD_CAP2 : CD_CAP;
      auto to_list = [&]() -> bool {
        const unsigned long long act = __ballot(1);
        const int leader = __ffsll((long long)act) - 1, lane_ = (int)(threadIdx.x & 63);
        uint32_t base = 0;
        if (lane_ == leader) base = atomicAdd(o_count, (uint32_t)__popcll(act));
        base = (uint32_t)__shfl((int)base, leader);
        const uint32_t k = base + (uint32_t)__popcll(act & ((1ull << lane_) - 1ull));
        if (k < o_cap) { o_list[k] = (uint32_t)p; return true; }
        may_list = false; return false;
      };
      if (MODE == CD_SWEEP && may_list && gaveup && to_list()) return;
      if (MODE == CD_SWEEP && l == 0 && !bloom_bit) { }
      else {
        const uint64_t mask = (1ull << (8 * (4 + l))) - 1ull;
        uint32_t d = q == p ? link_first[l] : (uint32_t)lv.prev[l][q];
        uint32_t nsteps = 0;
        for (;;) {
          if (d == 0) break;
          q -= d;
          if (p - q > (uint64_t)MAX_DIST) break;
          if (may_list && nsteps == step_cap && to_list()) return;
          const uint32_t dn = lv.prev[l][q];
          const uint64_t theirs = *(const u64u *)(in + q);
          nsteps++;
          if (p - q >= (uint64_t)dprev && ((theirs ^ mine) & mask) == 0) { dl = (uint32_t)(p - q); break; }
          d = dn;
        }
#ifdef ZADA_CD_STATS
        atomicAdd(&g_cd_dbg[0], 1ull); atomicAdd(&g_cd_dbg[1], (unsigned long long)nsteps); if (dl) atomicAdd(&g_cd_dbg[2], 1ull);
        if (nsteps == 0) atomicAdd(&g_cd_dbg[3], 1ull); if (nsteps > 8) atomicAdd(&g_cd_dbg[4], 1ull); if (nsteps > 64) atomicAdd(&g_cd_dbg[5], 1ull);
        if (dl == 0) atomicAdd(&g_cd_dbg[6], (unsigned long long)nsteps);
        if (dl_first[l] == DISTL_GAVEUP) atomicAdd(&g_cd_dbg[7], 1ull);
        if (nsteps > 32) atomicAdd(&g_cd_dbg[8], 1ull); if (nsteps > 128) atomicAdd(&g_cd_dbg[9], 1ull); if (nsteps > 256) atomicAdd(&g_cd_dbg[10], 1ull);
        if (nsteps > 512) atomicAdd(&g_cd_dbg[11], 1ull); if (nsteps > 1024) atomicAdd(&g_cd_dbg[12], 1ull); atomicMax(&g_cd_dbg[13], (unsigned long long)nsteps);
#endif
      }
      dp.d[1 + l][p] = (uint16_t)dl;
    }
    dprev = dl;
  }
}

__global__ void __launch_bounds__(256) k_cross_scan(const uint8_t *__restrict__ in, Layout L, DistPlanes dp, CdTail tl) {
  const uint32_t lane = threadIdx.x & 63, nc = *tl.count2, nl = nc < tl.cap2 ? nc : tl.cap2;
  for (uint32_t i = (blockIdx.x * blockDim.x + threadIdx.x) >> 6; i < nl; i += (gridDim.x * blockDim.x) >> 6) {
    const uint64_t p = tl.list2[i], seg = p >> 15;
    uint64_t first = (seg - 1) << 15;
    if (lay_first(L, seg - 1)) first += 1;
    const uint64_t lo = p - (uint64_t)MAX_DIST > first ? p - (uint64_t)MAX_DIST : first;
    const uint32_t mine = *(const u32u *)(in + p);
    uint32_t found = 0;
    for (uint64_t hi = p; hi > lo && !found; hi = hi - lo > 2048 ? hi - 2048 : lo) {
      uint64_t v[8];
#pragma unroll
      for (int u = 0; u < 8; u++) {
        const uint64_t q0 = hi - 256ull * (uint64_t)(u + 1) + 4ull * lane;
        v[u] = (q0 < hi && q0 + 3 >= lo) ? *(const u64u *)(in + q0) : 0ull;
      }
#pragma unroll
      for (int u = 0; u < 8; u++) {
        const uint64_t q0 = hi - 256ull * (uint64_t)(u + 1) + 4ull * lane;
        uint32_t mk = 0;
        if (q0 < hi && q0 + 3 >= lo) {
#pragma unroll
          for (int j = 0; j < 4; j++) if ((uint32_t)(v[u] >> (8 * j)) == mine && q0 + (uint64_t)j >= lo && q0 + (uint64_t)j < hi) mk |= 1u << j;
        }
        const unsigned long long m = __ballot(mk != 0);
        if (m && !found) {
          const int top = 63 - __builtin_clzll(m);
          const uint32_t tm = RL(mk, top);
          const uint64_t q = hi - 256ull * (uint64_t)(u + 1) + 4ull * (uint64_t)top + (uint64_t)(31 - __builtin_clz(tm));
          found = (uint32_t)(p - q);
        }
      }
    }
    if (lane == 0) dp.d[1][p] = (uint16_t)found;
  }
}

__global__ void __launch_bounds__(256) k_bucket_limits(Layout L, int kfull, int kquarter, const uint16_t *__restrict__ S3,
                                                       const uint32_t *__restrict__ bsc3, uint32_t *__restrict__ dlim, uint32_t *__restrict__ dlim_bits, const uint32_t *__restrict__ segmax,
                                                       const uint16_t *__restrict__ heavy, uint32_t seg0) {
  __shared__ uint32_t list[2048];
  __shared__ uint32_t nlist;
  __shared__ uint32_t lbits[1024];
  const uint64_t seg = (uint64_t)blockIdx.x + seg0, base = seg * 32768ull;
  const int tid = threadIdx.x;
  const bool has_prev = !lay_first(L, seg);
  {
    const uint32_t mo = segmax[seg], mp = has_prev ? segmax[seg - 1] : 0u;
    if (mo == 0 || mo - 1 + mp < (uint32_t)kquarter) return;
  }
  for (int i = tid; i < 1024; i += 256) lbits[i] = 0;
  auto flush_bits = [&]() { __syncthreads(); for (int i = tid; i < 1024; i += 256) { const uint32_t w = lbits[i]; if (w) dlim_bits[(base >> 5) + i] = w; } };
  const uint32_t *own = bsc3 + base, *prv = has_prev ? bsc3 + base - 32768 : nullptr;
  const uint16_t *s3 = S3 + base, *p3 = has_prev ? S3 + base - 32768 : nullptr;
  auto qualifies = [&](uint32_t h) -> bool {
    const uint32_t c = own[h] >> 16, cp = prv ? prv[h] >> 16 : 0u;
    return c > 0 && c - 1 + cp >= (uint32_t)kquarter;
  };
  auto process = [&]() {
    const uint32_t nl = nlist < 2048 ? nlist : 2048;
    for (uint32_t li = 0; li < nl; li++) {
      const uint32_t h = list[li];
      const uint32_t st = own[h] & 0xFFFF, c = own[h] >> 16;
      const uint32_t pst = prv ? prv[h] & 0xFFFF : 0u, cp = prv ? prv[h] >> 16 : 0u;
      const uint32_t r0 = (uint32_t)kquarter > cp ? (uint32_t)kquarter - cp : 0u;
      for (uint32_t r = r0 + tid; r < c; r += 256) {
        const uint32_t e = s3[st + r];
        uint32_t lim[2];
        const uint32_t ks[2] = {(uint32_t)kfull, (uint32_t)kquarter};
        for (int t = 0; t < 2; t++) {
          const uint32_t k = ks[t];
          uint64_t d = 0xFFFF;
          if (r >= k) d = e - s3[st + r - k];
          else if (cp >= k - r) d = (base + e) - (base - 32768 + p3[pst + cp - (k - r)]);
          lim[t] = d < 0xFFFF ? (uint32_t)d : 0xFFFFu;
        }
        dlim[base + e] = lim[0] | (lim[1] << 16);
        atomicOr(&lbits[e >> 5], 1u << (e & 31u));
      }
    }
  };
  const uint32_t heavy_thr = kquarter / 2 > 0 ? (uint32_t)kquarter / 2 : 1u;
  const uint16_t *ho = heavy + seg * HEAVY_STRIDE, *hp = has_prev ? heavy + (seg - 1) * HEAVY_STRIDE : nullptr;
  const uint32_t no = ho[0], np = hp ? hp[0] : 0u;
  if (no != 0xFFFFu && np != 0xFFFFu) {
    for (int phase = 0; phase < 2; phase++) {
      if (tid == 0) nlist = 0;
      __syncthreads();
      const uint16_t *hl = phase == 0 ? ho : hp;
      const uint32_t nh = phase == 0 ? no : np;
      for (uint32_t i = tid; i < nh; i += 256) {
        const uint32_t h = hl[1 + i];
        if (phase == 1 && (own[h] >> 16) >= heavy_thr) continue;
        if (qualifies(h)) { const uint32_t k = atomicAdd(&nlist, 1u); if (k < 2048) list[k] = h; }
      }
      __syncthreads();
      process();
      __syncthreads();
    }
    flush_bits();
    return;
  }
  for (uint32_t h0 = 0; h0 < 32768; h0 += 2048) {
    if (tid == 0) nlist = 0;
    __syncthreads();
    for (uint32_t h = h0 + tid; h < h0 + 2048; h += 256) {
      if (qualifies(h)) { const uint32_t k = atomicAdd(&nlist, 1u); if (k < 2048) list[k] = h; }
    }
    __syncthreads();
    process();
    __syncthreads();
  }
  flush_bits();
}

#ifndef ZADA_FAST
#define ZADA_FAST 12
#endif
#ifndef ZADA_CMP_TURNS
#define ZADA_CMP_TURNS 2
#endif
static_assert(ZADA_FAST % 2 == 0, "the fast phase is unrolled in pairs of steps");
constexpr int MB = 16384;
constexpr int HALO = 32512;
constexpr int WBYTES = HALO + MB + 272;
constexpr int WLINKS = HALO + MB;
constexpr int MATCH_LDS = WBYTES + WLINKS * 2 + 16 + 16 * 128 * 8;
static_assert(MATCH_LDS <= 160 * 1024, "k_match: one workgroup per CU");

#define LDS_U16(b, o) ((uint32_t)(b)[(o)] | ((uint32_t)(b)[(o) + 1] << 8))

__global__ void __launch_bounds__(1024) k_match(const uint8_t *__restrict__ in, Layout L,
                                                const uint16_t *__restrict__ prevd,
                                                DistPlanes dp,
                                                MatchPair *__restrict__ M,
                                                int nice_cfg, int budget, unsigned long long *__restrict__ dbg,
                                                uint16_t *__restrict__ resume, int short_budget) {
  extern __shared__ __attribute__((aligned(16))) uint8_t smem[];
  uint32_t *win = (uint32_t *)smem;
  uint16_t *lnk = (uint16_t *)(smem + WBYTES);
  uint32_t *next_pos = (uint32_t *)(smem + WBYTES + WLINKS * 2);
#ifdef ZADA_MATCH_STATS
  unsigned long long t_start = clock64(), t_empty = 0, iters = 0;
#endif
  const uint64_t B = (uint64_t)xcd_block() * MB;
  const uint64_t WB = B >= (uint64_t)HALO ? B - HALO : 0;
  const uint32_t woff = (uint32_t)(B - WB);
  const uint64_t n = lay_end(L, B >> 15);
  const uint32_t cnt = n > B ? (uint32_t)((n - B) < (uint64_t)MB ? (n - B) : (uint64_t)MB) : 0u;
  const int tid = threadIdx.x;
  if (cnt == 0) return;
  {
    const uint32_t nb = woff + cnt + 272;
    const uint4 *src = (const uint4 *)(in + WB);
    uint4 *dst = (uint4 *)win;
    for (uint32_t i = tid; i < (nb + 15) / 16; i += 1024) dst[i] = src[i];
    const uint32_t nl = woff + cnt;
    const uint4 *ls = (const uint4 *)(prevd + WB);
    uint4 *ld = (uint4 *)lnk;
    auto nil2 = [](uint32_t x) -> uint32_t { return x | ((x & 0xFFFFu) ? 0u : 0xFFFFu) | ((x >> 16) ? 0u : 0xFFFF0000u); };
    for (uint32_t i = tid; i < (nl * 2 + 15) / 16; i += 1024) { uint4 v = ls[i]; v.x = nil2(v.x); v.y = nil2(v.y); v.z = nil2(v.z); v.w = nil2(v.w); ld[i] = v; }
    if (tid < 4) next_pos[tid] = 0;
  }
  __syncthreads();
  const uint8_t *win8 = (const uint8_t *)win;
  uint32_t wi = woff, cur = woff, ncur = woff, bdist = 0, rq = 0, kpos = 0, s_end = 0;
  int best = 2, la = 3, nice = 3, state = 0;
  uint32_t lim_cur = 0, lim_full = 0;
  bool have_q = false, exhausted = false;
  uint32_t cmp_off = 0;
  int age = 0, mybudget = budget;
  static_assert(NLEVELS == 2 && MB == 16384 && MAX_DIST < 32768, "packing of the queue entries");
  constexpr uint32_t QCAP = 128;
  uint32_t *queue = next_pos + 4 + (threadIdx.x >> 6) * (2 * QCAP);
  const int lane = threadIdx.x & 63;
  uint32_t q_head = 0, q_tail = 0;
  bool blk_done = false;
  for (;;) {
    const bool need = (state == 0) && !exhausted;
    const unsigned long long need_mk = __ballot(need);
    if (need_mk) {
      const uint32_t nneed = (uint32_t)__popcll(need_mk);
      if (nneed > q_tail - q_head && !blk_done) {
        uint32_t k0 = 0;
        if (lane == 0) k0 = atomicAdd(&next_pos[0], 64u);
        k0 = (uint32_t)__builtin_amdgcn_readfirstlane((int)k0);
        if (k0 >= cnt) blk_done = true;
        else {
          const uint32_t k = k0 + (uint32_t)lane;
          bool ok = false;
          uint32_t e_lo = 0, e_hi = 0;
          if (k < cnt) {
            const uint64_t rem = n - (B + k);
            const int la_ = rem < 258 ? (int)rem : 258;
            const int nice_ = nice_cfg < la_ ? nice_cfg : la_;
            const uint32_t dlimv = dp.limits(B + k);
            const uint32_t df = dlimv & 0xFFFF, dq = dlimv >> 16;
            uint32_t dl[NLEVELS];
#pragma unroll
            for (int l = 0; l < NLEVELS; l++) dl[l] = dp.d[l][B + k];
            const uint32_t lf = dl[0] == (uint32_t)MAX_DIST ? (uint32_t)MAX_DIST : (df < (uint32_t)(MAX_DIST - 1) ? df : (uint32_t)(MAX_DIST - 1));
            const uint32_t lq = dq < lf ? dq : lf;
            int b_ = 2; uint32_t bd_ = 0, qbest = 0, qlev = 0;
            bool chain_ok = true;
#pragma unroll
            for (int l = 0; l < NLEVELS; l++) {
              const bool v = la_ >= 3 + l && dl[l] != 0 && dl[l] <= lf;
              if (v) { b_ = 3 + l; bd_ = dl[l]; if (dl[l] <= lq) { qbest = ((uint32_t)(3 + l) << 16) | dl[l]; qlev = 1u + l; } }
              chain_ok = v;
            }
            const bool hq = chain_ok && bd_ > lq;
            const uint32_t d0 = lnk[woff + k];
            ok = chain_ok && b_ < nice_ && d0 <= lf;
            if (!ok) {
              const uint32_t packed = b_ >= 3 ? ((uint32_t)b_ << 16) | bd_ : 0u;
              MatchPair r; r.full = packed; r.quarter = (hq || !chain_ok) ? qbest : packed;
              M[B + k] = r;
            }
            bool inner = false;
#ifndef ZADA_NO_INNER
            if (ok && k >= 2 && short_budget > 0) { const uint32_t m1 = dp.d[NLEVELS - 1][B + k - 1], m2 = dp.d[NLEVELS - 1][B + k - 2]; inner = dl[NLEVELS - 1] == m1 && m1 == m2; }
#endif
            e_lo = k | ((uint32_t)(b_ - 2) << 14) | ((uint32_t)inner << 16) | (bd_ << 17);
            e_hi = lf | (lq << 15) | (qlev << 30);
          }
          const unsigned long long okm = __ballot(ok);
          if (ok) { uint32_t *e = queue + 2 * ((q_tail + (uint32_t)__popcll(okm & ((1ull << lane) - 1ull))) & (QCAP - 1)); e[0] = e_lo; e[1] = e_hi; }
          q_tail += (uint32_t)__popcll(okm);
        }
      }
      const uint32_t avail = q_tail - q_head, rank = (uint32_t)__popcll(need_mk & ((1ull << lane) - 1ull));
      if (need) {
        if (rank < avail) {
          const uint32_t *e = queue + 2 * ((q_head + rank) & (QCAP - 1));
          const uint32_t e_lo = e[0], e_hi = e[1];
          kpos = e_lo & 0x3FFFu; wi = woff + kpos; age = 0;
          const uint64_t rem = n - (B + kpos);
          la = rem < 258 ? (int)rem : 258;
          nice = nice_cfg < la ? nice_cfg : la;
          best = 2 + (int)((e_lo >> 14) & 3u); bdist = e_lo >> 17;
          mybudget = ((e_lo >> 16) & 1u) ? short_budget : budget;
          lim_full = e_hi & 0x7FFFu;
          const uint32_t lim_q = (e_hi >> 15) & 0x7FFFu, qlev = e_hi >> 30;
          have_q = bdist > lim_q;
          rq = 0;
          if (qlev != 0) {
            const uint32_t qd = (int)qlev + 2 == best ? bdist : (uint32_t)dp.d[0][B + kpos];
            rq = ((qlev + 2u) << 16) | qd;
          }
          lim_cur = have_q ? lim_full : lim_q;
          const uint32_t d0 = lnk[wi];
          if (!have_q && d0 > lim_q) { have_q = true; rq = ((uint32_t)best << 16) | bdist; lim_cur = lim_full; }
          cur = wi - d0;
          s_end = LDS_U16(win8, wi + (uint32_t)best - 1u);
          state = 1;
        } else if (blk_done) {
#ifdef ZADA_MATCH_STATS
          if (t_empty == 0) t_empty = clock64();
#endif
          exhausted = true;
        }
      }
      q_head += nneed < avail ? nneed : avail;
    }
    if (!__any(state != 0)) { if (__all(exhausted)) break; continue; }
    {
      bool walk = state == 1, odd_stop = false;
      typedef const __attribute__((address_space(3))) uint8_t *lds_bytes;
      const uint32_t off = (uint32_t)(uintptr_t)(lds_bytes)win8 + (uint32_t)best - 1u;
      const int lim_pos = (int)wi - (int)lim_cur;
      uint32_t ca = cur, cb = ncur;
#pragma unroll
      for (int it = 0; it < ZADA_FAST; it += 2) {
        if (walk) {
#ifdef ZADA_MATCH_STATS
          iters++;
#endif
          const uint32_t dn = lnk[ca];
          uint32_t aa = ca + off;
          asm("" : "+v"(aa));
          const lds_bytes pa = (lds_bytes)(uintptr_t)aa;
          const uint32_t c16 = (uint32_t)pa[0] | ((uint32_t)pa[1] << 8);
          cb = ca - dn;
          walk = !(c16 == s_end || (int)cb < lim_pos);
        }
        if (walk) {
#ifdef ZADA_MATCH_STATS
          iters++;
#endif
          const uint32_t dn = lnk[cb];
          uint32_t ab = cb + off;
          asm("" : "+v"(ab));
          const lds_bytes pb = (lds_bytes)(uintptr_t)ab;
          const uint32_t c16 = (uint32_t)pb[0] | ((uint32_t)pb[1] << 8);
          ca = cb - dn;
          walk = !(c16 == s_end || (int)ca < lim_pos);
          odd_stop = !walk;
        }
      }
      cur = odd_stop ? cb : ca;
      ncur = odd_stop ? ca : cb;
      if (state == 1 && !walk) state = 2;
    }
    if (__any(state >= 2)) {
      bool ev_pass = false, ev_end = false, ev_lim = false;
      if (state >= 2) {
        ev_pass = LDS_U16(win8, cur + (uint32_t)best - 1u) == s_end;
        ev_end = lnk[cur] == 0xFFFFu;
        ev_lim = (int)ncur < (int)wi - (int)lim_cur;
      }
      bool cmpa = (state >= 2) && ev_pass;
      uint32_t off = state == 3 ? cmp_off : 0u;
      int len = 0;
#pragma unroll
      for (int t = 0; t < ZADA_CMP_TURNS; t++) {
        if (cmpa) {
#ifdef ZADA_MATCH_STATS
          iters++;
#endif
          const uint64_t x = lds_u64_at(win8, cur + off) ^ lds_u64_at(win8, wi + off);
          if (x) { len = (int)off + (int)(__builtin_ctzll(x) >> 3); cmpa = false; }
          else { off += 8; if ((int)off >= la) { len = la; cmpa = false; } }
        }
      }
      if (cmpa) { cmp_off = off; state = 3; }
      else if (state == 3) state = 2;
      if (state == 2) {
        len = len < la ? len : la;
        const bool improved = ev_pass && len > best;
        if (improved) {
          best = len; bdist = wi - cur;
          const uint32_t a = wi + (uint32_t)best;
          s_end = LDS_U16(win8, a - 1);
        }
        bool fin = (improved && len >= nice) || ev_end;
        const uint32_t packed = best >= 3 ? ((uint32_t)best << 16) | bdist : 0u;
        if (!fin && ev_lim) {
          if (!have_q) { have_q = true; rq = packed; lim_cur = lim_full; }
          if (wi - ncur > lim_full) fin = true;
        }
        if (fin) {
          MatchPair r; r.full = packed; r.quarter = have_q ? rq : packed;
          M[B + kpos] = r;
          state = 0;
        } else {
          cur = ncur;
          state = 1;
        }
      }
    }
    if (state == 1 && ++age >= mybudget) {
      const uint32_t packed = best >= 3 ? ((uint32_t)best << 16) | bdist : 0u;
      MatchPair r; r.full = packed | M_GUESS | (have_q ? M_HAVEQ : 0u); r.quarter = (have_q ? rq : packed) | (M_BEAT_MAX << M_BEAT_SHIFT);
      M[B + kpos] = r;
      resume[B + kpos] = (uint16_t)(wi - cur);
      state = 0;
    }
  }
#ifdef ZADA_MATCH_STATS
  {
    unsigned long long t_end = clock64();
    atomicAdd(&dbg[0], iters);
    atomicMax(&dbg[1], t_end - t_start);
    if ((threadIdx.x & 63) == 0) { atomicAdd(&dbg[2], t_end - t_start); atomicAdd(&dbg[3], 1ull); atomicAdd(&dbg[4], t_end - t_empty); }
    __syncthreads();
    if (threadIdx.x == 0) { atomicAdd(&dbg[5], clock64() - t_start); atomicAdd(&dbg[6], 1ull); }
  }
#endif
}

#ifndef ZADA_DM_THREADS
#define ZADA_DM_THREADS 512
#endif
static_assert(NLEVELS >= 2, "the links of level 0 are dead after k_cross_dist: their array carries the resume points of the guesses");
#ifndef ZADA_DM_AHEAD
#define ZADA_DM_AHEAD 1
#endif
#ifndef ZADA_DMB
#define ZADA_DMB 4096
#endif
constexpr int DM_THREADS = ZADA_DM_THREADS, DMB = ZADA_DMB, DM_SLICE = 256, DM_AHEAD = ZADA_DM_AHEAD;
constexpr int DM_WBYTES = HALO + DMB + 272;
#ifdef ZADA_DM_STATS
__device__ unsigned long long g_dm_dbg[8];
#endif
struct ScanDesc {
  uint16_t k, la, idx1, c1, idx2, c2, lim_full, lim_q;
  uint16_t bdist, best_hq;
  uint32_t rq, og_full, og_quarter;
};
constexpr int DM_LDS = DM_WBYTES + DMB * 2 + DM_SLICE * (int)sizeof(ScanDesc) + 64;
static_assert(MB % DMB == 0 && DM_WBYTES % 16 == 0 && sizeof(ScanDesc) == 32, "demand blocks tile the first-pass blocks");
__global__ void __launch_bounds__(DM_THREADS, 6) k_match_demand(const uint8_t *__restrict__ in, Layout L, DistPlanes dp, RunPtrs rp,
                                                             const uint16_t *__restrict__ tailsK, MatchPair *__restrict__ M, int nice_cfg,
                                                             const uint32_t *__restrict__ blk_demand, uint32_t *__restrict__ dbits, uint8_t *__restrict__ chg,
                                                             const ExitState *__restrict__ spec_exits, const uint16_t *__restrict__ resume, bool use_beat) {
  if (blk_demand[xcd_block()] == 0) return;
#ifdef ZADA_DM_STATS
  unsigned long long dm_t = clock64();
#define DM_STAMP(k) do { if (threadIdx.x == 0) { const unsigned long long t_ = clock64(); atomicAdd(&g_dm_dbg[k], t_ - dm_t); dm_t = t_; } } while (0)
#else
#define DM_STAMP(k) do {} while (0)
#endif
  const uint64_t B = (uint64_t)xcd_block() * DMB;
  extern __shared__ __attribute__((aligned(16))) uint8_t smem[];
  uint32_t *win = (uint32_t *)smem;
  uint16_t *list = (uint16_t *)(smem + DM_WBYTES);
  ScanDesc *desc = (ScanDesc *)(smem + DM_WBYTES + DMB * 2);
  uint32_t *ctr = (uint32_t *)(smem + DM_WBYTES + DMB * 2 + DM_SLICE * sizeof(ScanDesc));
  const uint64_t WB = B >= (uint64_t)HALO ? B - HALO : 0;
  const uint32_t woff = (uint32_t)(B - WB);
  const uint64_t n = lay_end(L, B >> 15);
  const uint32_t cnt = n > B ? (uint32_t)((n - B) < (uint64_t)DMB ? (n - B) : (uint64_t)DMB) : 0u;
  const bool seg_first = lay_first(L, B >> 15), prev_first = (B >> 15) > 0 && lay_first(L, (B >> 15) - 1);
  const int tid = threadIdx.x, lane = tid & 63, wave = tid >> 6;
#ifdef ZADA_DM_STAGE_FIRST
  constexpr bool STAGE_BESIDE = false;
#else
  constexpr bool STAGE_BESIDE = DM_THREADS > DM_SLICE;
#endif
  auto stage = [&](uint32_t t0, uint32_t stride) {
    const uint32_t nb = woff + cnt + 272;
    const uint4 *src = (const uint4 *)(in + WB);
    uint4 *dst = (uint4 *)win;
    for (uint32_t i = t0; i < (nb + 15) / 16; i += stride) dst[i] = src[i];
  };
  if (!STAGE_BESIDE) stage((uint32_t)tid, DM_THREADS);
  const uint8_t *win8 = (const uint8_t *)win;
  auto store_result = [&](uint64_t p, uint32_t full, uint32_t quarter, uint32_t og_full, uint32_t og_quarter, bool reach) {
    MatchPair r; r.full = full; r.quarter = quarter;
    M[p] = r;
    const uint32_t beat = use_beat ? og_quarter >> M_BEAT_SHIFT : 0u, ogq = og_quarter & M_VALUE;
    if ((og_full & M_BYSPEC) && ((full != (og_full & M_VALUE) && (full >> 16) > beat) || (quarter != ogq && (quarter >> 16) > beat))) {
      const uint64_t ch = p / PCHUNK;
      chg[ch] = 1;
      if (reach) chg[ch - 1] = 1;
    }
  };
  if (tid == 0) ctr[0] = 0;
  __syncthreads();
  DM_STAMP(0);
  if (tid < DMB / 32) {
    uint32_t *wp = dbits + (B >> 5) + tid;
    uint32_t bits = *wp;
    if (bits) {
      *wp = 0;
      uint32_t o = atomicAdd(&ctr[0], (uint32_t)__popc(bits));
      while (bits) { const int j = __ffs((int)bits) - 1; bits &= bits - 1; list[o++] = (uint16_t)(tid * 32 + j); }
    }
  }
  __syncthreads();
  DM_STAMP(1);
  const uint32_t nl = ctr[0];
#ifdef ZADA_DM_STATS
  if (tid == 0) { atomicAdd(&g_dm_dbg[4], 1ull); atomicAdd(&g_dm_dbg[5], (unsigned long long)nl); }
#endif
  for (uint32_t l0 = 0; l0 < nl; l0 += DM_SLICE) {
    if (tid == 0) { ctr[1] = 0; ctr[2] = DM_THREADS / 64; }
    __syncthreads();
    if (STAGE_BESIDE && l0 == 0 && tid >= DM_SLICE) stage((uint32_t)(tid - DM_SLICE), DM_THREADS - DM_SLICE);
    const bool win_ready = !(STAGE_BESIDE && l0 == 0);
    if ((uint32_t)tid < (uint32_t)DM_SLICE && l0 + tid < nl) {
      const uint32_t k = list[l0 + tid];
      const uint64_t p = B + k;
      const uint32_t wi = woff + k;
      const uint64_t rem = n - p;
      const int la = rem < 258 ? (int)rem : 258;
      const int nice = nice_cfg < la ? nice_cfg : la;
      const uint64_t seg = p >> 15, pbase = (seg << 15) - 32768;
      const uint32_t dlimv = dp.limits(p);
      uint32_t dl[NLEVELS];
#pragma unroll
      for (int l = 0; l < NLEVELS; l++) dl[l] = dp.d[l][p];
      const MatchPair og = M[p];
      const uint32_t idx1 = rp.idx[p], c1 = rp.cnt[p];
      uint32_t t = 0xFFFFu;
      if (!seg_first) {
        const uint32_t key = hashL_of(win_ready ? lds_u64_at(win8, wi) : *(const u64u *)(in + p), 3 + NLEVELS);
        const uint32_t tt = tailsK[(seg - 1) * 65536ull + key];
        const uint64_t q = pbase + tt;
        if (tt < lay_inserted(L, seg - 1) && p - q <= (uint64_t)MAX_DIST &&
            hashL_of(win_ready ? lds_u64_at(win8, (uint32_t)(q - WB)) : *(const u64u *)(in + q), 3 + NLEVELS) == key) t = tt;
      }
      uint32_t idx2 = 0, c2 = 0;
      if (t != 0xFFFFu) { idx2 = rp.idx[pbase + t]; c2 = (uint32_t)rp.cnt[pbase + t] + 1u; }
      const uint32_t df = dlimv & 0xFFFF, dq = dlimv >> 16;
      const uint32_t lim_full = dl[0] == (uint32_t)MAX_DIST ? (uint32_t)MAX_DIST : (df < (uint32_t)(MAX_DIST - 1) ? df : (uint32_t)(MAX_DIST - 1));
      const uint32_t lim_q = dq < lim_full ? dq : lim_full;
      int best = 2;
      uint32_t bdist = 0, qbest = 0;
      bool chain_ok = true;
#pragma unroll
      for (int l = 0; l < NLEVELS; l++) {
        const bool v = la >= 3 + l && dl[l] != 0 && dl[l] <= lim_full;
        if (v) { best = 3 + l; bdist = dl[l]; if (dl[l] <= lim_q) qbest = ((uint32_t)(3 + l) << 16) | dl[l]; }
        chain_ok = v;
      }
      bool have_q = chain_ok && bdist > lim_q;
      uint32_t idx1r = idx1, c1r = c1, idx2r = idx2, c2r = c2;
      if (chain_ok) {
        const uint32_t gl = (og.full & M_VALUE) >> 16;
        if (gl >= 3) { best = (int)gl; bdist = og.full & 0xFFFFu; }
        have_q = (og.full & M_HAVEQ) != 0;
        if (have_q) qbest = og.quarter & M_VALUE;
        const uint64_t q = p - resume[p];
        const uint32_t iq = rp.idx[q];
        const uint32_t skip = q >= (seg << 15) ? idx1 - 1 - iq : c1 + (idx2 - iq);
        if (skip < c1) { idx1r = idx1 - skip; c1r = c1 - skip; }
        else { const uint32_t s2 = skip - c1 < c2 ? skip - c1 : c2; c1r = 0; idx2r = idx2 - s2; c2r = c2 - s2; }
      }
      const uint64_t chk = p / PCHUNK;
      const bool reach = chk > 0 && spec_exits[chk - 1].pos >= (uint32_t)p;
      if (chain_ok && best < nice && c1r + c2r > 0) {
        ScanDesc ds;
        ds.k = (uint16_t)k; ds.la = (uint16_t)la; ds.idx1 = (uint16_t)idx1r; ds.c1 = (uint16_t)c1r; ds.idx2 = (uint16_t)idx2r; ds.c2 = (uint16_t)c2r;
        ds.lim_full = (uint16_t)lim_full; ds.lim_q = (uint16_t)lim_q; ds.bdist = (uint16_t)bdist; ds.best_hq = (uint16_t)((uint32_t)best | ((uint32_t)reach << 14) | ((uint32_t)have_q << 15));
        ds.rq = qbest; ds.og_full = og.full; ds.og_quarter = og.quarter;
        desc[atomicAdd(&ctr[1], 1u)] = ds;
      } else {
        const uint32_t packed = best >= 3 ? ((uint32_t)best << 16) | bdist : 0u;
        store_result(p, packed, !chain_ok ? qbest : (have_q ? qbest : packed), og.full, og.quarter, reach);
      }
    }
    __syncthreads();
    DM_STAMP(2);
#ifdef ZADA_DM_STATS
    if (tid == 0) atomicAdd(&g_dm_dbg[6], (unsigned long long)ctr[1]);
#endif
    const uint32_t ns = ctr[1];
    auto cand_load = [&](const ScanDesc &ds, uint32_t c) -> uint32_t {
      const uint16_t *sprev = rp.S + ((((B + ds.k) >> 15) << 15) - 32768);
      const bool in1 = c < ds.c1, in2 = !in1 && c - ds.c1 < ds.c2;
      const uint32_t a = in1 ? 32768u + ds.idx1 - 1u - c : (in2 ? (uint32_t)ds.idx2 - (c - ds.c1) : 32768u);
      return sprev[a];
    };
    auto cand_dist = [&](const ScanDesc &ds, uint32_t c, uint32_t raw) -> uint32_t {
      const uint64_t P_ = B + ds.k;
      const uint32_t po = (uint32_t)P_ & 32767u;
      const bool in1 = c < ds.c1, in2 = !in1 && c - ds.c1 < ds.c2;
      const bool q0 = raw == 0 && ((in1 && seg_first) || (in2 && prev_first));
      return q0 ? 0u : (in1 ? po - raw : (in2 ? po + 32768u - raw : 0u));
    };
#ifndef ZADA_DM_STATIC
    auto take = [&]() -> uint32_t { uint32_t t = 0; if (lane == 0) t = atomicAdd(&ctr[2], 1u); return (uint32_t)__builtin_amdgcn_readfirstlane((int)t); };
    uint32_t si = (uint32_t)wave, nxt = si < ns ? take() : ns;
    uint32_t rnext = si < ns ? cand_load(desc[si], (uint32_t)lane) : 0u;
    for (; si < ns; si = nxt, nxt = si < ns ? take() : ns) {
      const ScanDesc ds = desc[si];
      const uint32_t r0 = rnext;
      if (nxt < ns) rnext = cand_load(desc[nxt], (uint32_t)lane);
#else
    uint32_t rnext = (uint32_t)wave < ns ? cand_load(desc[wave], (uint32_t)lane) : 0u;
    for (uint32_t si = (uint32_t)wave; si < ns; si += DM_THREADS / 64) {
      const ScanDesc ds = desc[si];
      const uint32_t r0 = rnext;
      if (si + DM_THREADS / 64 < ns) rnext = cand_load(desc[si + DM_THREADS / 64], (uint32_t)lane);
#endif
      const uint32_t WI = woff + ds.k, LF = ds.lim_full, LQ = ds.lim_q, TT = (uint32_t)ds.c1 + ds.c2;
      const int LA = ds.la, NICE = nice_cfg < LA ? nice_cfg : LA;
      int bst = ds.best_hq & 0x3FFF;
      uint32_t bd = ds.bdist, rqq = ds.rq;
      bool hq = (ds.best_hq >> 15) != 0;
      auto lds_u32 = [&](uint32_t o) -> uint32_t {
        const uint32_t *w = (const uint32_t *)(win8 + (o & ~3u));
        return __builtin_amdgcn_alignbyte(w[1], w[0], o & 3u);
      };
      uint32_t s_end = lds_u32(WI + (uint32_t)bst - 3);
      bool over = false;
      auto batch = [&](uint32_t d) {
        const bool valid = d != 0;
        const bool inr = valid && d <= LF;
        bool pass = false;
        if (inr) pass = lds_u32(WI - d + (uint32_t)bst - 3) == s_end;
        unsigned long long pm = __ballot(pass);
        while (pm) {
          const int j = __ffsll((long long)pm) - 1;
          const uint32_t dj = RL(d, j);
          if (!hq && dj > LQ) { hq = true; rqq = bst >= 3 ? ((uint32_t)bst << 16) | bd : 0u; }
          const uint32_t o = 4u * (uint32_t)lane;
          const uint32_t x = lds_u32(WI - dj + o) ^ lds_u32(WI + o);
          const unsigned long long mm = __ballot(x != 0);
          int len;
          if (mm) { const int l0 = __ffsll((long long)mm) - 1; len = 4 * l0 + (int)(__builtin_ctz(RL(x, l0)) >> 3); }
          else { const uint32_t y = LDS_U16(win8, WI - dj + 256) ^ LDS_U16(win8, WI + 256); len = 256 + (y == 0 ? 2 : ((y & 0xFF) == 0 ? 1 : 0)); }
          len = len < LA ? len : LA;
          if (len > bst) {
            bst = len; bd = dj;
            if (len >= NICE) { over = true; break; }
            s_end = lds_u32(WI + (uint32_t)bst - 3);
            pass = pass && lane > j && lds_u32(WI - d + (uint32_t)bst - 3) == s_end;
          } else pass = pass && lane > j;
          pm = __ballot(pass);
        }
        if (!over && !hq && __any(valid && d > LQ)) { hq = true; rqq = bst >= 3 ? ((uint32_t)bst << 16) | bd : 0u; }
        if (__any(!inr)) over = true;
      };
      uint32_t dq[DM_AHEAD];
      dq[0] = r0;
#pragma unroll
      for (int u = 1; u < DM_AHEAD; u++) dq[u] = 64u * u < TT ? cand_load(ds, 64u * u + (uint32_t)lane) : 0u;
      for (uint32_t c0 = 0; c0 < TT && !over; c0 += 64 * DM_AHEAD) {
#pragma unroll
        for (int u = 0; u < DM_AHEAD; u++) {
          if (c0 + 64u * u < TT && !over) {
            const uint32_t dcur = cand_dist(ds, c0 + 64u * u + (uint32_t)lane, dq[u]);
            const uint32_t cn = c0 + 64u * (u + DM_AHEAD);
            if (cn < TT) dq[u] = cand_load(ds, cn + (uint32_t)lane);
            batch(dcur);
          }
        }
      }
      if (lane == 0) {
        const uint32_t packed = bst >= 3 ? ((uint32_t)bst << 16) | bd : 0u;
        store_result(B + ds.k, packed, hq ? rqq : packed, ds.og_full, ds.og_quarter, (ds.best_hq >> 14) & 1u);
      }
    }
    __syncthreads();
    DM_STAMP(3);
  }
}

__global__ void k_demand_all(Layout L, MatchPair *__restrict__ M, uint32_t *__restrict__ blk_demand, uint32_t *__restrict__ dbits) {
  const uint64_t p = (uint64_t)blockIdx.x * blockDim.x + threadIdx.x;
  if (p >= L.n || p >= lay_end(L, p >> 15)) return;
  const uint32_t f = M[p].full;
  if (f & M_GUESS) {
    if (!(f & M_DEMAND)) M[p].full = f | M_DEMAND | M_BYSPEC;
    atomicOr(&dbits[p >> 5], 1u << (p & 31));
    blk_demand[p / DMB] = 1;
  }
}

struct DemandMarker {
  MatchPair *M; uint32_t *blk_demand; uint32_t *n_demand; uint32_t by;
  bool track = false;
  uint32_t *dbits;
  __device__ void operator()(uint32_t p, uint32_t full, uint32_t quarter, uint32_t beat) const {
    if (track && (beat < M_BEAT_MAX ? beat : M_BEAT_MAX) < (quarter >> M_BEAT_SHIFT))
      __hip_atomic_fetch_min(&M[p].quarter, (quarter & M_VALUE) | ((beat < M_BEAT_MAX ? beat : M_BEAT_MAX) << M_BEAT_SHIFT), __ATOMIC_RELAXED, __HIP_MEMORY_SCOPE_AGENT);
    const uint32_t want = M_DEMAND | by;
    if ((full & want) == want) return;
    M[p].full = full | want;
    atomicOr(&dbits[p >> 5], 1u << (p & 31));
    blk_demand[p / DMB] = 1;
    *n_demand = 1;
  }
};

#ifndef ZADA_PS_BWORDS
#define ZADA_PS_BWORDS 16
#endif
#ifndef ZADA_PS_TOKS
#define ZADA_PS_TOKS 8
#endif
constexpr uint32_t PS_BWORDS = ZADA_PS_BWORDS, PS_TOKS = ZADA_PS_TOKS;
static_assert((PS_BWORDS == 8 || PS_BWORDS == 16) && (PS_TOKS == 4 || PS_TOKS == 8), "line sizes of the parser's LDS caches");
struct LineFetch {
  const MatchPair *M; uint64_t *slot;
  uint32_t tag;
  __device__ MatchPair operator()(uint32_t p) {
    const uint32_t t = p >> 3;
    if (t != tag) {
      const uint4 *src = (const uint4 *)(M + ((uint64_t)t << 3));
      const uint4 a = src[0], b = src[1], c = src[2], d = src[3];
      slot[0 * 64] = (uint64_t)a.x | ((uint64_t)a.y << 32); slot[1 * 64] = (uint64_t)a.z | ((uint64_t)a.w << 32);
      slot[2 * 64] = (uint64_t)b.x | ((uint64_t)b.y << 32); slot[3 * 64] = (uint64_t)b.z | ((uint64_t)b.w << 32);
      slot[4 * 64] = (uint64_t)c.x | ((uint64_t)c.y << 32); slot[5 * 64] = (uint64_t)c.z | ((uint64_t)c.w << 32);
      slot[6 * 64] = (uint64_t)d.x | ((uint64_t)d.y << 32); slot[7 * 64] = (uint64_t)d.z | ((uint64_t)d.w << 32);
      tag = t;
    }
    const uint64_t v = slot[(p & 7u) * 64];
    MatchPair r; r.full = (uint32_t)v; r.quarter = (uint32_t)(v >> 32);
    return r;
  }
  const uint8_t *in; uint32_t *bslot; uint32_t btag;
  __device__ uint32_t byte(uint32_t p) {
    constexpr uint32_t SH = PS_BWORDS == 16 ? 6 : 5;
    const uint32_t t = p >> SH;
    if (t != btag) {
      const uint4 *src = (const uint4 *)(in + ((uint64_t)t << SH));
      const uint4 a = src[0], b = src[1];
      bslot[0 * 64] = a.x; bslot[1 * 64] = a.y; bslot[2 * 64] = a.z; bslot[3 * 64] = a.w;
      bslot[4 * 64] = b.x; bslot[5 * 64] = b.y; bslot[6 * 64] = b.z; bslot[7 * 64] = b.w;
      if (PS_BWORDS == 16) {
        const uint4 c = src[2], d = src[3];
        bslot[8 * 64] = c.x; bslot[9 * 64] = c.y; bslot[10 * 64] = c.z; bslot[11 * 64] = c.w;
        bslot[12 * 64] = d.x; bslot[13 * 64] = d.y; bslot[14 * 64] = d.z; bslot[15 * 64] = d.w;
      }
      btag = t;
    }
    return (bslot[((p >> 2) & (PS_BWORDS - 1u)) * 64] >> (8 * (p & 3u))) & 0xFFu;
  }
};

struct TokSink {
  uint32_t *dst; uint32_t *buf; uint32_t n;
  __device__ void push(uint32_t t) {
    buf[(n & (PS_TOKS - 1u)) * 64] = t;
    n++;
    if ((n & (PS_TOKS - 1u)) == 0) {
      uint4 a;
      a.x = buf[0]; a.y = buf[64]; a.z = buf[128]; a.w = buf[192];
      uint4 *o = (uint4 *)(dst + n - PS_TOKS);
      o[0] = a;
      if (PS_TOKS == 8) { uint4 b; b.x = buf[256]; b.y = buf[320]; b.z = buf[384]; b.w = buf[448]; o[1] = b; }
    }
  }
  __device__ void flush() { for (uint32_t i = n & ~(PS_TOKS - 1u); i < n; i++) dst[i] = buf[(i & (PS_TOKS - 1u)) * 64]; }
};

__global__ void __launch_bounds__(1024) k_list_flagged(const uint8_t *__restrict__ flag, uint32_t n, uint32_t *__restrict__ list, uint32_t *__restrict__ count) {
  __shared__ uint32_t wcnt[16], wbase;
  const uint32_t i = blockIdx.x * 1024 + threadIdx.x, lane = threadIdx.x & 63, w = threadIdx.x >> 6;
  const bool f = i < n && flag[i];
  const unsigned long long mk = __ballot(f);
  if (lane == 0) wcnt[w] = (uint32_t)__popcll(mk);
  __syncthreads();
  if (threadIdx.x == 0) {
    uint32_t t = 0;
    for (int k = 0; k < 16; k++) { const uint32_t c = wcnt[k]; wcnt[k] = t; t += c; }
    wbase = t ? atomicAdd(count, t) : 0u;
  }
  __syncthreads();
  if (f) list[wbase + wcnt[w] + (uint32_t)__popcll(mk & ((1ull << lane) - 1ull))] = i;
}

#ifdef ZADA_RESPEC_STATS
__device__ unsigned long long g_respec_dbg[4];
#endif
__global__ void k_parse_spec(ParseIO io, uint32_t nchunks, uint32_t *__restrict__ spec_tok, uint32_t *__restrict__ spec_cnt,
                             uint32_t *__restrict__ Fbits, uint32_t *__restrict__ Lbits, ExitState *__restrict__ exits,
                             DemandMarker dm, const uint32_t *__restrict__ list , const uint32_t *__restrict__ list_n,
                             uint32_t exact_max ) {
  uint32_t k = blockIdx.x * blockDim.x + threadIdx.x;
  if (list) {
    const uint32_t nl = *list_n;
    if (nl <= exact_max || k >= nl) return;
    k = list[k];
  }
  if (k >= nchunks) return;
  if (io.segend) io.n = io.segend[((uint64_t)k * PCHUNK) >> 15] & 0x7FFFFFFFu;
  uint32_t ntok = 0;
  ExitState ex;
#ifdef ZADA_RESPEC_STATS
  uint32_t old_h = 0, old_n = 0; ExitState old_ex{0, 0};
  if (list) { old_n = spec_cnt[k]; old_ex = exits[k]; const uint32_t *ot = spec_tok + (uint64_t)k * PTOK_STRIDE; for (uint32_t i = 0; i < old_n; i++) old_h = old_h * 0x9E3779B1u + ot[i]; }
#endif
  __shared__ uint64_t lines[8 * 64];
  __shared__ uint32_t tbuf[PS_TOKS * 64];
  __shared__ uint32_t blines[PS_BWORDS * 64];
  LineFetch lf; lf.M = io.M; lf.slot = lines + threadIdx.x; lf.tag = 0xFFFFFFFFu; lf.in = io.in; lf.bslot = blines + threadIdx.x; lf.btag = 0xFFFFFFFFu;
  TokSink ts; ts.dst = spec_tok + (uint64_t)k * PTOK_STRIDE; ts.buf = tbuf + threadIdx.x; ts.n = 0;
  parse_spec_chunk_to(io, k, PCHUNK, ts, Fbits, Lbits, ex, dm, lf);
  ts.flush();
  ntok = ts.n;
  spec_cnt[k] = ntok;
  exits[k] = ex;
#ifdef ZADA_RESPEC_STATS
  if (list) {
    __threadfence();
    uint32_t new_h = 0; const uint32_t *nt = spec_tok + (uint64_t)k * PTOK_STRIDE; for (uint32_t i = 0; i < ntok; i++) new_h = new_h * 0x9E3779B1u + nt[i];
    atomicAdd(&g_respec_dbg[0], 1ull);
    if (new_h == old_h && ntok == old_n && ex.pos == old_ex.pos && ex.kind == old_ex.kind) atomicAdd(&g_respec_dbg[1], 1ull);
  }
#endif
}

struct WaveExact {
  const uint8_t *in; Layout L; DistPlanes dp; RunPtrs rp; const uint16_t *tailsK; MatchPair *M; int nice_cfg; const uint16_t *resume;
  __device__ __forceinline__ uint32_t g32(uint64_t o) const { return *(const u32u *)(in + o); }
  __device__ MatchPair search(uint64_t p, MatchPair og) const {
    const int lane = threadIdx.x & 63;
    const uint64_t seg = p >> 15, n = lay_end(L, seg);
    const bool seg_first = lay_first(L, seg), prev_first = seg > 0 && lay_first(L, seg - 1);
    const uint64_t rem = n - p;
    const int la = rem < 258 ? (int)rem : 258;
    const int nice = nice_cfg < la ? nice_cfg : la;
    const uint64_t pbase = (seg << 15) - 32768;
    const uint32_t dlimv = dp.limits(p);
    uint32_t dl[NLEVELS];
#pragma unroll
    for (int l = 0; l < NLEVELS; l++) dl[l] = dp.d[l][p];
    const uint32_t idx1 = rp.idx[p], c1 = rp.cnt[p];
    uint32_t t = 0xFFFFu;
    if (!seg_first) {
      const uint32_t key = hashL_of(*(const u64u *)(in + p), 3 + NLEVELS);
      const uint32_t tt = tailsK[(seg - 1) * 65536ull + key];
      const uint64_t q = pbase + tt;
      if (tt < lay_inserted(L, seg - 1) && p - q <= (uint64_t)MAX_DIST && hashL_of(*(const u64u *)(in + q), 3 + NLEVELS) == key) t = tt;
    }
    uint32_t idx2 = 0, c2 = 0;
    if (t != 0xFFFFu) { idx2 = rp.idx[pbase + t]; c2 = (uint32_t)rp.cnt[pbase + t] + 1u; }
    const uint32_t df = dlimv & 0xFFFF, dq = dlimv >> 16;
    const uint32_t LF = dl[0] == (uint32_t)MAX_DIST ? (uint32_t)MAX_DIST : (df < (uint32_t)(MAX_DIST - 1) ? df : (uint32_t)(MAX_DIST - 1));
    const uint32_t LQ = dq < LF ? dq : LF;
    int bst = 2;
    uint32_t bd = 0, rqq = 0;
    bool chain_ok = true;
#pragma unroll
    for (int l = 0; l < NLEVELS; l++) {
      const bool v = la >= 3 + l && dl[l] != 0 && dl[l] <= LF;
      if (v) { bst = 3 + l; bd = dl[l]; if (dl[l] <= LQ) rqq = ((uint32_t)(3 + l) << 16) | dl[l]; }
      chain_ok = v;
    }
    bool hq = chain_ok && bd > LQ;
    uint32_t i1 = idx1, n1 = c1, i2 = idx2, n2 = c2;
    if (chain_ok) {
      const uint32_t gl = (og.full & M_VALUE) >> 16;
      if (gl >= 3) { bst = (int)gl; bd = og.full & 0xFFFFu; }
      hq = (og.full & M_HAVEQ) != 0;
      if (hq) rqq = og.quarter & M_VALUE;
      const uint64_t q = p - resume[p];
      const uint32_t iq = rp.idx[q];
      const uint32_t skip = q >= (seg << 15) ? idx1 - 1 - iq : c1 + (idx2 - iq);
      if (skip < c1) { i1 = idx1 - skip; n1 = c1 - skip; }
      else { const uint32_t s2 = skip - c1 < c2 ? skip - c1 : c2; n1 = 0; i2 = idx2 - s2; n2 = c2 - s2; }
    }
    MatchPair r;
    if (!(chain_ok && bst < nice && n1 + n2 > 0)) {
      const uint32_t packed = bst >= 3 ? ((uint32_t)bst << 16) | bd : 0u;
      r.full = packed; r.quarter = !chain_ok ? rqq : (hq ? rqq : packed);
      if (lane == 0) M[p] = r;
      return r;
    }
    const uint16_t *sprev = rp.S + ((seg << 15) - 32768);
    const uint32_t TT = n1 + n2, po = (uint32_t)p & 32767u;
    auto cand = [&](uint32_t c) -> uint32_t {
      const bool in1 = c < n1, in2 = !in1 && c - n1 < n2;
      const uint32_t a = in1 ? 32768u + i1 - 1u - c : (in2 ? i2 - (c - n1) : 32768u);
      const uint32_t raw = sprev[a];
      const bool q0 = raw == 0 && ((in1 && seg_first) || (in2 && prev_first));
      return q0 ? 0u : (in1 ? po - raw : (in2 ? po + 32768u - raw : 0u));
    };
    uint32_t s_end = g32(p + (uint32_t)bst - 3);
    bool over = false;
    uint32_t dnext = cand((uint32_t)lane);
    for (uint32_t c0 = 0; c0 < TT && !over; c0 += 64) {
      const uint32_t d = dnext;
      if (c0 + 64 < TT) dnext = cand(c0 + 64 + (uint32_t)lane);
      const bool valid = d != 0;
      const bool inr = valid && d <= LF;
      bool pass = false;
      if (inr) pass = g32(p - d + (uint32_t)bst - 3) == s_end;
      unsigned long long pm = __ballot(pass);
      while (pm) {
        const int j = __ffsll((long long)pm) - 1;
        const uint32_t dj = RL(d, j);
        if (!hq && dj > LQ) { hq = true; rqq = bst >= 3 ? ((uint32_t)bst << 16) | bd : 0u; }
        const uint32_t o = 4u * (uint32_t)lane;
        const uint32_t x = g32(p - dj + o) ^ g32(p + o);
        const unsigned long long mm = __ballot(x != 0);
        int len;
        if (mm) { const int l0 = __ffsll((long long)mm) - 1; len = 4 * l0 + (int)(__builtin_ctz(RL(x, l0)) >> 3); }
        else { const uint32_t y = (g32(p - dj + 256) ^ g32(p + 256)) & 0xFFFFu; len = 256 + (y == 0 ? 2 : ((y & 0xFF) == 0 ? 1 : 0)); }
        len = len < la ? len : la;
        if (len > bst) {
          bst = len; bd = dj;
          if (len >= nice) { over = true; break; }
          s_end = g32(p + (uint32_t)bst - 3);
          pass = pass && lane > j && g32(p - d + (uint32_t)bst - 3) == s_end;
        } else pass = pass && lane > j;
        pm = __ballot(pass);
      }
      if (!over && !hq && __any(valid && d > LQ)) { hq = true; rqq = bst >= 3 ? ((uint32_t)bst << 16) | bd : 0u; }
      if (__any(!inr)) over = true;
    }
    const uint32_t packed = bst >= 3 ? ((uint32_t)bst << 16) | bd : 0u;
    r.full = packed; r.quarter = hq ? rqq : packed;
    if (lane == 0) M[p] = r;
    return r;
  }
};

constexpr uint32_t PX_RECS = PCHUNK + 320;
struct WaveFetch {
  const uint64_t *recs; uint32_t c0; const MatchPair *Mg; const WaveExact *wx;
  __device__ MatchPair operator()(uint32_t p) const {
    MatchPair r;
    if (p - c0 < PX_RECS) { const uint64_t v = recs[p - c0]; r.full = (uint32_t)v; r.quarter = (uint32_t)(v >> 32); }
    else r = Mg[p];
    if (r.full & M_GUESS) r = wx->search(p, r);
    return r;
  }
};
struct WaveSink {
  uint32_t *dst; uint32_t n;
  __device__ void push(uint32_t t) { if ((threadIdx.x & 63) == 0) dst[n] = t; n++; }
};
constexpr int PX_WAVES = 4;
__global__ void __launch_bounds__(64 * PX_WAVES) k_parse_spec_exact(ParseIO io, uint32_t nchunks, uint32_t *__restrict__ spec_tok, uint32_t *__restrict__ spec_cnt,
                                                                     uint32_t *__restrict__ Fbits, uint32_t *__restrict__ Lbits, ExitState *__restrict__ exits,
                                                                     WaveExact wx, const uint32_t *__restrict__ list, const uint32_t *__restrict__ list_n, uint32_t exact_max) {
  __shared__ uint64_t recs[PX_WAVES][PX_RECS];
  const int lane = threadIdx.x & 63, w = threadIdx.x >> 6;
  const uint32_t nl = *list_n, stride = gridDim.x * PX_WAVES;
  if (nl > exact_max) return;
  for (uint32_t i = blockIdx.x * PX_WAVES + w; i < nl; i += stride) {
    const uint32_t k = list[i];
    if (k >= nchunks) continue;
    ParseIO cio = io;
    if (io.segend) cio.n = io.segend[((uint64_t)k * PCHUNK) >> 15] & 0x7FFFFFFFu;
    const uint32_t c0 = k * PCHUNK;
    {
      const uint64_t *src = (const uint64_t *)(io.M + c0);
      const uint32_t have = (uint64_t)c0 + PX_RECS <= io.n ? PX_RECS : (uint32_t)(io.n - c0);
      for (uint32_t j = lane; j < have; j += 64) recs[w][j] = src[j];
    }
    __builtin_amdgcn_wave_barrier();
    WaveFetch wf; wf.recs = recs[w]; wf.c0 = c0; wf.Mg = io.M; wf.wx = &wx;
    WaveSink ts; ts.dst = spec_tok + (uint64_t)k * PTOK_STRIDE; ts.n = 0;
    ExitState ex;
    parse_spec_chunk_to(cio, k, PCHUNK, ts, Fbits, Lbits, ex, NoGuess(), wf);
    if (lane == 0) { spec_cnt[k] = ts.n; exits[k] = ex; }
    __builtin_amdgcn_wave_barrier();
  }
}

__global__ void k_parse_fix(ParseIO io, uint32_t nchunks, const uint32_t *__restrict__ spec_tok, const uint32_t *__restrict__ spec_cnt,
                            const uint32_t *__restrict__ Fbits, const uint32_t *__restrict__ Lbits,
                            const ExitState *__restrict__ spec_exits, ExitState *__restrict__ true_exits,
                            uint32_t *__restrict__ fix_tok, uint32_t *__restrict__ fix_cnt,
                            uint32_t *__restrict__ take_from, uint32_t *__restrict__ start_pos,
                            const uint8_t *__restrict__ dirty_in, uint8_t *__restrict__ dirty_out,
                            uint32_t *__restrict__ n_changed, DemandMarker dm, ExitState entry0, uint32_t fix_stride, uint32_t *__restrict__ fix_overflow) {
  uint32_t k = blockIdx.x * blockDim.x + threadIdx.x;
  if (k >= nchunks) return;
  if (!dirty_in[k]) return;
  ExitState entry = entry0;
  if (k > 0) entry = true_exits[k - 1];
  if (io.segend) {
    const uint32_t se = io.segend[((uint64_t)k * PCHUNK) >> 15];
    io.n = se & 0x7FFFFFFFu;
    if ((se >> 31) && ((k * PCHUNK) & 32767u) == 0) entry = ExitState{k * PCHUNK, SYNC_F};
  }
  const ExitState old_exit = true_exits[k];
  ExitState new_exit;
  uint32_t ntok = 0, take = 0, u0 = 0;
  parse_fix_chunk(io, k, PCHUNK, entry, spec_tok + (uint64_t)k * PTOK_STRIDE, spec_cnt[k], Fbits, Lbits, spec_exits[k],
                  fix_tok + (uint64_t)k * fix_stride, ntok, take, u0, new_exit, dm, DirectFetch{io.M}, fix_stride, fix_overflow);
  fix_cnt[k] = ntok;
  take_from[k] = take;
  start_pos[k] = u0;
  true_exits[k] = new_exit;
  if (k + 1 < nchunks && (new_exit.pos != old_exit.pos || new_exit.kind != old_exit.kind)) {
    dirty_out[k + 1] = 1;
    atomicAdd(n_changed, 1u);
    atomicMin(n_changed + 1, k);
  }
}

__global__ void __launch_bounds__(64) k_fix_forward(ParseIO io, uint32_t nchunks, ExitState *__restrict__ true_exits,
                                                    uint8_t *__restrict__ dirty_out, uint32_t *__restrict__ n_changed) {
  const uint32_t k = n_changed[1];
  if (k >= nchunks || 258 < io.cfg.lazy || io.segend) return;
  const ExitState e0 = true_exits[k];
  if (e0.kind != SYNC_F) return;
  const int lane = threadIdx.x;
  for (uint64_t q0 = e0.pos;; q0 += 258ull * 64) {
    const uint64_t q = q0 + 258ull * lane;
    bool good = false;
    if (q + 258 <= io.n) { const uint32_t f = io.M[q].full; good = !(f & M_GUESS) && ((f & M_VALUE) >> 16) == 258u; }
    const unsigned long long bad = ~__ballot(good);
    const int nvalid = bad ? __ffsll((long long)bad) - 1 : 64;
    if (lane <= nvalid && (lane > 0 || q0 != e0.pos)) {
      const uint64_t c1 = (q / PCHUNK) * PCHUNK;
      if (q - c1 < 258 && c1 >= PCHUNK) {
        const uint32_t kk = (uint32_t)(c1 / PCHUNK) - 1;
        if (kk > k && kk < nchunks) {
          const ExitState old = true_exits[kk];
          if (old.pos != (uint32_t)q || old.kind != SYNC_F) {
            ExitState ne; ne.pos = (uint32_t)q; ne.kind = SYNC_F;
            true_exits[kk] = ne;
            if (kk + 1 < nchunks) dirty_out[kk + 1] = 1;
            atomicAdd(n_changed, 1u);
          }
        }
      }
    }
    if (nvalid < 64) break;
  }
}

__global__ void k_seed_entry(ExitState *__restrict__ true_exits, uint32_t kE, ExitState e) {
  const uint32_t k = blockIdx.x * blockDim.x + threadIdx.x;
  if (k < kE) true_exits[k] = e;
}

__global__ void k_tok_count(uint32_t nchunks, const uint32_t *__restrict__ spec_cnt, const uint32_t *__restrict__ fix_cnt,
                            const uint32_t *__restrict__ take_from, uint32_t *__restrict__ counts) {
  uint32_t k = blockIdx.x * blockDim.x + threadIdx.x;
  if (k < nchunks) counts[k] = fix_cnt[k] + (spec_cnt[k] - take_from[k]);
}

__global__ void __launch_bounds__(256) k_tok_compact(uint32_t nchunks, const uint32_t *__restrict__ spec_tok,
                                                     const uint32_t *__restrict__ spec_cnt, const uint32_t *__restrict__ fix_tok,
                                                     const uint32_t *__restrict__ fix_cnt, const uint32_t *__restrict__ take_from,
                                                     const uint32_t *__restrict__ start_pos, const uint32_t *__restrict__ offsets,
                                                     uint32_t *__restrict__ atoms, uint32_t *__restrict__ apos, uint32_t k0, uint32_t apos_bias, uint32_t fix_stride) {
  const uint32_t kk = (blockIdx.x * blockDim.x + threadIdx.x) >> 6;
  const int lane = threadIdx.x & 63;
  if (kk >= nchunks) return;
  const uint32_t k = k0 + kk;
  const uint32_t nf = fix_cnt[k], tf = take_from[k], ns = spec_cnt[k] - tf;
  const uint32_t *ft = fix_tok + (uint64_t)k * fix_stride;
  const uint32_t *st = spec_tok + (uint64_t)k * PTOK_STRIDE + tf;
  uint32_t out = offsets[kk];
  uint32_t pos = start_pos[k] + apos_bias;
  const uint32_t total = nf + ns;
  for (uint32_t b = 0; b < total; b += 64) {
    uint32_t i = b + lane;
    uint32_t t = 0, len = 0;
    if (i < total) { t = i < nf ? ft[i] : st[i - nf]; len = tok_len(t); }
    uint32_t incl = len;
    for (int off = 1; off < 64; off <<= 1) { uint32_t v = __shfl_up(incl, off); if (lane >= off) incl += v; }
    if (i < total) { atoms[out + i] = t; apos[out + i] = pos + incl - len; }
    pos += __shfl(incl, 63);
  }
}

__global__ void __launch_bounds__(1024) k_scan_block(const uint32_t *__restrict__ in, uint32_t *__restrict__ out,
                                                     uint32_t *__restrict__ block_sums, uint32_t n) {
  __shared__ uint32_t wsum[16];
  const int tid = threadIdx.x, lane = tid & 63, w = tid >> 6;
  uint32_t i = blockIdx.x * 1024 + tid;
  uint32_t v = i < n ? in[i] : 0, incl = v;
  for (int off = 1; off < 64; off <<= 1) { uint32_t t = __shfl_up(incl, off); if (lane >= off) incl += t; }
  if (lane == 63) wsum[w] = incl;
  __syncthreads();
  uint32_t base = 0;
  for (int k = 0; k < w; k++) base += wsum[k];
  if (i < n) out[i] = base + incl - v;
  if (tid == 1023) block_sums[blockIdx.x] = base + incl;
}
__global__ void __launch_bounds__(1024) k_scan_sums(uint32_t *__restrict__ block_sums, uint32_t nb, uint32_t *__restrict__ total) {
  __shared__ uint32_t wsum[16];
  __shared__ uint32_t carry;
  const int tid = threadIdx.x, lane = tid & 63, w = tid >> 6;
  if (tid == 0) carry = 0;
  __syncthreads();
  for (uint32_t b = 0; b < nb; b += 1024) {
    uint32_t i = b + tid;
    uint32_t v = i < nb ? block_sums[i] : 0, incl = v;
    for (int off = 1; off < 64; off <<= 1) { uint32_t t = __shfl_up(incl, off); if (lane >= off) incl += t; }
    if (lane == 63) wsum[w] = incl;
    __syncthreads();
    uint32_t base = carry;
    for (int k = 0; k < w; k++) base += wsum[k];
    if (i < nb) block_sums[i] = base + incl - v;
    __syncthreads();
    if (tid == 1023) carry = base + incl;
    __syncthreads();
  }
  if (tid == 0) *total = carry;
}
__global__ void k_scan_add(uint32_t *__restrict__ out, const uint32_t *__restrict__ block_sums, uint32_t n) {
  uint32_t i = blockIdx.x * blockDim.x + threadIdx.x;
  if (i < n) out[i] += block_sums[i >> 10];
}

__global__ void k_literal_atoms(const uint8_t *__restrict__ in, uint64_t n, uint32_t *__restrict__ atoms, uint32_t *__restrict__ apos, uint32_t bias) {
  uint64_t stride = (uint64_t)gridDim.x * blockDim.x;
  for (uint64_t i = (uint64_t)blockIdx.x * blockDim.x + threadIdx.x; i < n; i += stride) { atoms[i] = in[i]; apos[i] = (uint32_t)i + bias; }
}

__global__ void k_literal_counts(uint32_t nchunks, Layout L, uint32_t *__restrict__ counts) {
  const uint32_t k = blockIdx.x * blockDim.x + threadIdx.x;
  if (k >= nchunks) return;
  const uint64_t c0 = (uint64_t)k * PCHUNK, e = lay_end(L, c0 >> 15);
  counts[k] = e > c0 ? (uint32_t)(e - c0 < PCHUNK ? e - c0 : PCHUNK) : 0u;
}
__global__ void __launch_bounds__(256) k_literal_atoms_batch(uint32_t nchunks, const uint8_t *__restrict__ in, const uint32_t *__restrict__ counts,
                                                             const uint32_t *__restrict__ offsets, uint32_t *__restrict__ atoms, uint32_t *__restrict__ apos) {
  const uint32_t k = (blockIdx.x * blockDim.x + threadIdx.x) >> 6, lane = threadIdx.x & 63;
  if (k >= nchunks) return;
  const uint32_t cnt = counts[k], o = offsets[k], c0 = k * PCHUNK;
  for (uint32_t i = lane; i < cnt; i += 64) { atoms[o + i] = in[c0 + i]; apos[o + i] = c0 + i; }
}

void exclusive_scan_u32(hipStream_t st, const uint32_t *d_in, uint32_t *d_out, uint32_t *d_sums, uint32_t *d_total, uint32_t n) {
  uint32_t nb = (n + 1023) / 1024;
  hipLaunchKernelGGL(k_scan_block, dim3(nb), dim3(1024), 0, st, d_in, d_out, d_sums, n);
  hipLaunchKernelGGL(k_scan_sums, dim3(1), dim3(1024), 0, st, d_sums, nb, d_total);
  hipLaunchKernelGGL(k_scan_add, dim3((n + 255) / 256), dim3(256), 0, st, d_out, d_sums, n);
}

int lz_shard(Ctx *c, int level, const ShardJob &job, ShardResult *res) {
  hipStream_t st = c->stream;
  Workspace &W = c->ws;
  const uint64_t n = job.nbuf;
  res->ntok = 0; res->exit = ExitState{(uint32_t)n, SYNC_F}; res->warm = ExitState{job.tok_lo, SYNC_F};
  if (n == 0) return 0;
  if (level == RICH_LEVEL) return rich_shard(c, job, res);
  if (job.need && (level == 0 || n < 32768 + 2)) { if (int rn = job.need(n)) return rn; }
  if (level == 0 && job.segend) {
    const uint32_t nch = (uint32_t)((n + PCHUNK - 1) / PCHUNK);
    const Layout L{job.segend, n};
    hipLaunchKernelGGL(k_literal_counts, dim3((nch + 255) / 256), dim3(256), 0, st, nch, L, W.counts);
    exclusive_scan_u32(st, W.counts, W.offsets, W.scan_sums, W.n_changed, nch);
    uint32_t total = 0;
    hipMemcpyAsync(&total, W.n_changed, 4, hipMemcpyDeviceToHost, st);
    if (hip_check(c, hipStreamSynchronize(st), "literal counts")) return ZADA_E_HIP_;
    if (total > job.cap_atoms) { c->err = "atom array overflow"; return -2; }
    hipLaunchKernelGGL(k_literal_atoms_batch, dim3((nch + 3) / 4), dim3(256), 0, st, nch, W.in, W.counts, W.offsets, job.dst_atoms, job.dst_apos);
    res->ntok = total;
    return hip_check(c, hipGetLastError(), "k_literal_atoms_batch");
  }
  if (level == 0) {
    const uint64_t hi = job.final ? n : job.tok_hi, cnt = hi - job.tok_lo;
    uint32_t *dst_atoms = job.dst_atoms, *dst_apos = job.dst_apos;
    if (cnt > job.cap_atoms) {
      if (!job.grow_atoms) { c->err = "atom array overflow"; return -2; }
      if (int rg = job.grow_atoms(cnt, &dst_atoms, &dst_apos)) return rg;
    }
    if (cnt) hipLaunchKernelGGL(k_literal_atoms, dim3(2048), dim3(256), 0, st, W.in + job.tok_lo, cnt, dst_atoms, dst_apos, job.apos_bias + job.tok_lo);
    res->ntok = (uint32_t)cnt;
    res->exit = ExitState{(uint32_t)hi, SYNC_F};
    return hip_check(c, hipGetLastError(), "k_literal_atoms");
  }
  const LzConfig cfg = lz_config(level);
  const Layout L{job.segend, n};
  const uint64_t n_ins = job.segend ? n : (n >= 2 ? n - 2 : 0);
  const uint32_t nseg = (uint32_t)((n_ins + 32767) / 32768);
  c->tmark("lz:begin");
  if (!c->lz_attrs_set) {
    hipFuncSetAttribute((const void *)k_prev_links<true>, hipFuncAttributeMaxDynamicSharedMemorySize, PL_LDS_RUNS);
    hipFuncSetAttribute((const void *)k_prev_links<false>, hipFuncAttributeMaxDynamicSharedMemorySize, PL_LDS);
    hipFuncSetAttribute((const void *)k_cross_links, hipFuncAttributeMaxDynamicSharedMemorySize, CL_LDS_PLANE);
    hipFuncSetAttribute((const void *)k_match, hipFuncAttributeMaxDynamicSharedMemorySize, MATCH_LDS);
    hipFuncSetAttribute((const void *)k_match_demand, hipFuncAttributeMaxDynamicSharedMemorySize, DM_LDS);
    c->lz_attrs_set = true;
  }
  LevelPtrs lv;
  DistPlanes dpl;
  RunPtrs rpt; rpt.S = W.SK; rpt.idx = W.idxK; rpt.cnt = W.cntK;
  for (int l = 0; l < NLEVELS; l++) dpl.d[l] = W.dplane[l];
  dpl.dlim = W.dlim; dpl.dlim_bits = W.dlim_bits;
  if (nseg > 0) {
    for (int l = 0; l < NLEVELS; l++) { lv.prev[l] = W.lprev[l]; lv.tails[l] = W.ltails[l]; }
#ifndef ZADA_OLD_INIT
    hipEventRecord(c->ev_dlim, st);
    hipStreamWaitEvent(c->stream2, c->ev_dlim, 0);
    hipMemsetAsync(W.dlim_bits, 0, (size_t)(n / 32 + 2) * 4, c->stream2);
    hipEventRecord(c->ev_dlim, c->stream2);
#endif
    uint32_t R = 1;
    if (c->knob_link_run > 0) R = (uint32_t)c->knob_link_run;
    else {
      while (R < 16 && nseg / (2 * R) >= 1024) R *= 2;
      if (job.need && R > 8) R = 8;
    }
    if ((R & (R - 1)) || R > 64) { c->err = "link_run is not a power of two up to 64"; return -1; }
    auto prev_links = [&](uint32_t s0, uint32_t s1) {
      if (R > 1) hipLaunchKernelGGL(k_prev_links<true>, dim3((s1 - s0 + R - 1) / R), dim3(1024), PL_LDS_RUNS, st, W.in, L, cfg.chain, cfg.chain >> 2, lv,
                                    W.S3, W.T3, W.bsc3, dpl, rpt, (unsigned long long *)W.dbg, W.segmax, W.heavy, s0, R, s1);
      else hipLaunchKernelGGL(k_prev_links<false>, dim3(s1 - s0), dim3(1024), PL_LDS, st, W.in, L, cfg.chain, cfg.chain >> 2, lv,
                              W.S3, W.T3, W.bsc3, dpl, rpt, (unsigned long long *)W.dbg, W.segmax, W.heavy, s0, 1u, s1);
    };
    auto cross_links = [&](uint32_t from, uint32_t to) {
      const uint32_t first = (from + R - 1) / R * R;
      if (first < to) hipLaunchKernelGGL(k_cross_links, dim3((to - first + R - 1) / R, NLEVELS), dim3(1024), CL_LDS_PLANE, st, W.in, L, lv, dpl, first, R);
    };
    static_assert(BLOOM_WORDS == 4096, "Workspace::bloom4 is sized in zada_api.hip");
    auto cross_dist = [&]() {
      const uint32_t nb = (uint32_t)((n_ins - 32768 + CD_THREADS - 1) / CD_THREADS);
      if (!c->knob_cd_filter) {
        hipLaunchKernelGGL(k_cross_dist<CD_ALL>, dim3(nb), dim3(CD_THREADS), 0, st, W.in, L, lv, W.S3, W.T3, W.bsc3, dpl, (uint64_t)32768, (uint64_t)n, CdTail{nullptr, nullptr, W.n_changed + 4, 0u, nullptr, W.n_changed + 5, 0u});
        return;
      }
      hipMemsetAsync(W.n_changed + 4, 0, 4, st);
      hipLaunchKernelGGL(k_bloom4, dim3(nseg - 1), dim3(256), 0, st, W.in, L, W.bloom4, 0u);
      hipMemsetAsync(W.n_changed + 5, 0, 4, st);
      const uint32_t lcap = c->knob_cd_list_cap > 0 && (uint64_t)c->knob_cd_list_cap < W.cd_cap ? (uint32_t)c->knob_cd_list_cap : (uint32_t)W.cd_cap;
      const CdTail tl{W.bloom4, W.cd_list, W.n_changed + 4, lcap, W.cd_list + W.cd_cap, W.n_changed + 5, lcap / 4};
      hipLaunchKernelGGL(k_cross_dist<CD_SWEEP>, dim3(nb), dim3(CD_THREADS), 0, st, W.in, L, lv, W.S3, W.T3, W.bsc3, dpl, (uint64_t)32768, (uint64_t)n, tl);
      hipLaunchKernelGGL(k_cross_dist<CD_LIST>, dim3((uint32_t)((W.cd_cap + CD_THREADS - 1) / CD_THREADS)), dim3(CD_THREADS), 0, st, W.in, L, lv, W.S3, W.T3, W.bsc3, dpl, (uint64_t)0, (uint64_t)n, tl);
      hipLaunchKernelGGL(k_cross_scan, dim3(2048), dim3(256), 0, st, W.in, L, dpl, tl);
    };
    if (job.need) {
      constexpr uint32_t PIECE = 2048;
      static_assert(PIECE % 64 == 0, "pieces start at multiples of every run length (a power of two up to 64)");
      constexpr double SLOW_PIECE_S = 2.0e-3;
      uint32_t cl_from = 1;
      auto cross_links_upto = [&](uint32_t s1) {
        if (s1 > cl_from) cross_links(cl_from, s1);
        if (s1 > cl_from) cl_from = s1;
      };
      auto t_prev = std::chrono::steady_clock::now();
      for (uint32_t s0 = 0; s0 < nseg;) {
        const uint32_t s1 = s0 + PIECE < nseg ? s0 + PIECE : nseg;
        const uint64_t upto = (uint64_t)s1 * 32768 + 64 < n ? (uint64_t)s1 * 32768 + 64 : n;
        if (int rn = job.need(upto)) return rn;
        const auto t_now = std::chrono::steady_clock::now();
        const bool slow = s0 > 0 && std::chrono::duration<double>(t_now - t_prev).count() >= SLOW_PIECE_S;
        t_prev = t_now;
        prev_links(s0, s1);
#ifndef ZADA_OLD_INIT
        if (s0 == 0) hipStreamWaitEvent(st, c->ev_dlim, 0);
#endif
        if (slow) cross_links_upto(s1);
        hipLaunchKernelGGL(k_bucket_limits, dim3(s1 - s0), dim3(256), 0, st, L, cfg.chain, cfg.chain >> 2, W.S3, W.bsc3, W.dlim, W.dlim_bits, W.segmax, W.heavy, s0);
        s0 = s1;
      }
      if (int rn = job.need(n)) return rn;
      cross_links_upto(nseg);
      if (nseg > 1) cross_dist();
    } else
    prev_links(0, nseg);
#ifndef ZADA_OLD_INIT
    if (!job.need) hipStreamWaitEvent(st, c->ev_dlim, 0);
#endif
#ifdef ZADA_PL_STATS
    { unsigned long long h[32]; hipMemcpy(h, W.dbg, sizeof h, hipMemcpyDeviceToHost); fprintf(stderr, "[prev_links cycles/segment] init %.0f |", (double)h[8] / nseg); for (int q = 9; q < 9 + 4 * (NLEVELS + 1) - 1; q++) fprintf(stderr, " %.0f", (double)h[q] / nseg); fprintf(stderr, "  (per level 3..: sort, links, first candidates, queue rounds)\n"); fprintf(stderr, "[level 4 walks per segment] rounds %.2f  entries %.1f  entries of the last round %.1f  hops there %.1f (max %llu over all segments; walks over 64 hops %.3f)  first-queue overflow %.1f  cycles of the last round %.0f\n", (double)h[24] / nseg, (double)h[25] / nseg, (double)h[26] / nseg, (double)h[27] / nseg, h[28], (double)h[29] / nseg, (double)h[30] / nseg, (double)h[31] / nseg); hipMemset(W.dbg, 0, 256);
      unsigned long long sd[8]; hipMemcpyFromSymbol(sd, HIP_SYMBOL(g_sort_dbg), sizeof sd); fprintf(stderr, "[sort_pass cycles/segment, all six passes] clear %.0f  rank (LDS atomics) %.0f  scan %.0f  scatter %.0f\n", (double)sd[0] / nseg, (double)sd[1] / nseg, (double)sd[2] / nseg, (double)sd[3] / nseg); for (int q = 0; q < 8; q++) sd[q] = 0; hipMemcpyToSymbol(HIP_SYMBOL(g_sort_dbg), sd, sizeof sd); }
#endif
    c->tmark("prev_links");
    if (!job.need) {
      if (nseg > 1) {
        cross_links(1, nseg);
        cross_dist();
      }
      hipLaunchKernelGGL(k_bucket_limits, dim3(nseg), dim3(256), 0, st, L, cfg.chain, cfg.chain >> 2, W.S3, W.bsc3, W.dlim, W.dlim_bits, W.segmax, W.heavy, 0u);
    }
  }
#ifdef ZADA_CD_STATS
  { unsigned long long h[16]; hipDeviceSynchronize(); hipMemcpyFromSymbol(h, HIP_SYMBOL(g_cd_dbg), sizeof h);
    fprintf(stderr, "[k_cross_dist level-4 walks] %llu walks (%.1f %% of the positions), %llu steps (%.2f per walk), found %llu (%.1f %%), no step %llu, > 8 steps %llu, > 64 steps %llu, steps of the walks that found nothing %llu, gave-up restarts %llu\n",
            h[0], 100.0 * h[0] / n, h[1], (double)h[1] / (h[0] ? h[0] : 1), h[2], 100.0 * h[2] / (h[0] ? h[0] : 1), h[3], h[4], h[5], h[6], h[7]);
    fprintf(stderr, "[k_cross_dist level-4 walks] > 32 steps %llu, > 128 %llu, > 256 %llu, > 512 %llu, > 1024 %llu, longest %llu\n", h[8], h[9], h[10], h[11], h[12], h[13]);
    for (int q = 0; q < 16; q++) h[q] = 0; hipMemcpyToSymbol(HIP_SYMBOL(g_cd_dbg), h, sizeof h); }
#endif
  c->tmark("cross_links");
  const uint32_t nbm = (uint32_t)((n + MB - 1) / MB);
  const uint32_t nch = (uint32_t)((n + PCHUNK - 1) / PCHUNK);
  const int max_rounds = c->knob_max_demand_rounds;
  int budget_env = c->knob_budget >= 0 ? c->knob_budget : (n < (2u << 20) ? 0 : n < (512u << 20) ? 8 : 6);
  if (budget_env < 1) budget_env = 1 << 20;
  const uint32_t nbd = (uint32_t)((n + DMB - 1) / DMB);
  hipMemsetAsync(W.blk_demand, 0, (size_t)nbd * 4, st);
  hipMemsetAsync(W.dbits, 0, (size_t)nbd * (DMB / 8), st);
  hipMemsetAsync(W.n_demand, 0, 4, st);
  hipLaunchKernelGGL(k_match, dim3(nbm), dim3(1024), MATCH_LDS, st, W.in, L, W.lprev[NLEVELS - 1], dpl, W.M, cfg.nice,
                     budget_env, (unsigned long long *)W.dbg, W.lprev[0], budget_env > c->knob_inner_budget ? c->knob_inner_budget : 0);
  c->tmark("match");
  ParseIO io; io.in = W.in; io.n = n; io.M = W.M; io.cfg = cfg; io.segend = job.segend;
  DemandMarker dm; dm.M = W.M; dm.blk_demand = W.blk_demand; dm.n_demand = W.n_demand; dm.by = M_BYSPEC; dm.dbits = W.dbits;
  DemandMarker dmf = dm; dmf.by = 0;
  int rounds = 0, demand_rounds = 0;
  bool valve_used = false;
  static const bool round_stats = getenv("ZADA_ROUND_STATS") != nullptr;
  const ExitState entry0 = job.entry_known ? job.entry : ExitState{0, SYNC_F};
  const uint32_t kE = job.entry_known ? (entry0.pos / PCHUNK < nch ? entry0.pos / PCHUNK : nch) : 0u;
  hipMemsetAsync(W.n_changed + 6, 0, 4, st);
  bool restart = false, first_again = false;
  for (bool first = true;; first = false) {
    if (first_again) { first = true; first_again = false; }
    const bool beat_valid = !first;
    if (first) hipLaunchKernelGGL(k_parse_spec, dim3((nch + 63) / 64), dim3(64), 0, st, io, nch,
                                  W.spec_tok, W.spec_cnt, W.Fbits, W.Lbits, W.spec_exits, dm, (const uint32_t *)nullptr, (const uint32_t *)nullptr, 0u);
    else {
      hipMemsetAsync(W.n_changed + 2, 0, 4, st);
      hipLaunchKernelGGL(k_list_flagged, dim3((nch + 1023) / 1024), dim3(1024), 0, st, W.chg, nch, W.offsets, W.n_changed + 2);
      const uint32_t exact_max = c->knob_exact_respec > 0 ? (uint32_t)c->knob_exact_respec : 0u;
      if (exact_max) {
        WaveExact wx; wx.in = W.in; wx.L = L; wx.dp = dpl; wx.rp = rpt; wx.tailsK = W.ltails[NLEVELS - 1]; wx.M = W.M; wx.nice_cfg = cfg.nice; wx.resume = W.lprev[0];
        hipLaunchKernelGGL(k_parse_spec_exact, dim3(256 * 5), dim3(64 * PX_WAVES), 0, st, io, nch, W.spec_tok, W.spec_cnt, W.Fbits, W.Lbits, W.spec_exits,
                           wx, (const uint32_t *)W.offsets, (const uint32_t *)(W.n_changed + 2), exact_max);
      }
      DemandMarker dmt = dm; dmt.track = true;
      hipLaunchKernelGGL(k_parse_spec, dim3((nch + 63) / 64), dim3(64), 0, st, io, nch,
                         W.spec_tok, W.spec_cnt, W.Fbits, W.Lbits, W.spec_exits, dmt, (const uint32_t *)W.offsets, (const uint32_t *)(W.n_changed + 2), exact_max);
    }
    hipMemcpyAsync(W.true_exits, W.spec_exits, (size_t)nch * sizeof(ExitState), hipMemcpyDeviceToDevice, st);
    if (kE > 0) hipLaunchKernelGGL(k_seed_entry, dim3((kE + 255) / 256), dim3(256), 0, st, W.true_exits, kE, entry0);
    hipMemsetAsync(W.dirty[0], 1, nch, st);
    int cur = 0, it = 0;
    uint32_t ndem = 0;
    bool slow = false;
    for (;;) {
      hipMemsetAsync(W.dirty[cur ^ 1], 0, nch, st);
      hipMemsetAsync(W.n_changed, 0, 4, st);
      hipMemsetAsync(W.n_changed + 1, 0xFF, 4, st);
      hipLaunchKernelGGL(k_parse_fix, dim3((nch + 63) / 64), dim3(64), 0, st, io, nch,
                         W.spec_tok, W.spec_cnt, W.Fbits, W.Lbits, W.spec_exits, W.true_exits, W.fix_tok, W.fix_cnt,
                         W.take_from, W.start_pos, W.dirty[cur], W.dirty[cur ^ 1], W.n_changed, dmf, entry0, W.fix_stride, W.n_changed + 6);
      hipLaunchKernelGGL(k_fix_forward, dim3(1), dim3(64), 0, st, io, nch, W.true_exits, W.dirty[cur ^ 1], W.n_changed);
      uint32_t changed = 0, fix_ovf = 0;
      hipMemcpyAsync(&changed, W.n_changed, 4, hipMemcpyDeviceToHost, st);
      hipMemcpyAsync(&ndem, W.n_demand, 4, hipMemcpyDeviceToHost, st);
      if (W.fix_stride < PTOK_STRIDE) hipMemcpyAsync(&fix_ovf, W.n_changed + 6, 4, hipMemcpyDeviceToHost, st);
      if (hip_check(c, hipStreamSynchronize(st), "parse_fix")) return ZADA_E_HIP_;
      rounds++;
      if (fix_ovf) {
        uint32_t *bigger = nullptr;
        const uint64_t nch_cap = W.cap_n / PCHUNK + 2;
        if (hipMalloc(&bigger, nch_cap * (uint64_t)PTOK_STRIDE * 4) != hipSuccess) { (void)hipGetLastError(); c->err = "out of device memory (splice tokens)"; return -2; }
        W.allocs.push_back(bigger);
        W.fix_tok = bigger; W.fix_stride = PTOK_STRIDE;
        c->fix_grown++;
        hipMemsetAsync(W.n_changed + 6, 0, 4, st);
        restart = true;
        break;
      }
      if (changed == 0) break;
      if (++it >= 32 && !valve_used) { slow = true; break; }
      cur ^= 1;
    }
    if (round_stats) {
      uint32_t nl = 0, nmark = 0;
      if (!first) hipMemcpy(&nl, W.n_changed + 2, 4, hipMemcpyDeviceToHost);
      { std::vector<uint32_t> hb(nbd); hipMemcpy(hb.data(), W.blk_demand, (size_t)nbd * 4, hipMemcpyDeviceToHost); for (uint32_t v : hb) nmark += v != 0; }
      fprintf(stderr, "[lz round %d] %s parse of %u chunks, splice iterations so far %d, blocks with demanded positions %u of %u, demand %u%s\n", demand_rounds, first || nl > (uint32_t)(c->knob_exact_respec > 0 ? c->knob_exact_respec : 0) ? "speculative" : "exact",
              first ? nch : nl, rounds, nmark, nbd, ndem, slow ? " (slow splice)" : "");
    }
#ifdef ZADA_RESPEC_STATS
    if (!first) { unsigned long long h[4]; hipDeviceSynchronize(); hipMemcpyFromSymbol(h, HIP_SYMBOL(g_respec_dbg), sizeof h); fprintf(stderr, "[respec round %d] %llu chunks parsed again, %llu of them with the same tokens and exit as before\n", demand_rounds, h[0], h[1]); h[0] = h[1] = 0; hipMemcpyToSymbol(HIP_SYMBOL(g_respec_dbg), h, sizeof h); }
#endif
    if (restart) { restart = false; first_again = true; continue; }
    if (ndem == 0 && !slow) break;
    demand_rounds++;
    if (demand_rounds > 1000) { c->err = "demand loop did not converge"; return ZADA_E_HIP_; }
    hipMemsetAsync(W.n_demand, 0, 4, st);
    hipMemsetAsync(W.chg, 0, nch, st);
    if ((demand_rounds == max_rounds || slow) && !valve_used) {
      valve_used = true;
      hipLaunchKernelGGL(k_demand_all, dim3((uint32_t)((n + 255) / 256)), dim3(256), 0, st, L, W.M, W.blk_demand, W.dbits);
    }
    hipLaunchKernelGGL(k_match_demand, dim3(nbd), dim3(DM_THREADS), DM_LDS, st, W.in, L, dpl, rpt, W.ltails[NLEVELS - 1], W.M, cfg.nice,
                       W.blk_demand, W.dbits, W.chg, W.spec_exits, W.lprev[0], beat_valid);
    hipMemsetAsync(W.blk_demand, 0, (size_t)nbd * 4, st);
#ifdef ZADA_DM_STATS
    { unsigned long long h[8]; hipDeviceSynchronize(); hipMemcpyFromSymbol(h, HIP_SYMBOL(g_dm_dbg), sizeof h);
      fprintf(stderr, "[k_match_demand round %d] %llu blocks, %.1f marked positions and %.1f scans per block; cycles per block: staging %.0f, list %.0f, phase A %.0f, phase B %.0f\n", demand_rounds, h[4],
              (double)h[5] / (h[4] ? h[4] : 1), (double)h[6] / (h[4] ? h[4] : 1), (double)h[0] / (h[4] ? h[4] : 1), (double)h[1] / (h[4] ? h[4] : 1), (double)h[2] / (h[4] ? h[4] : 1), (double)h[3] / (h[4] ? h[4] : 1));
      for (int q = 0; q < 8; q++) h[q] = 0; hipMemcpyToSymbol(HIP_SYMBOL(g_dm_dbg), h, sizeof h); }
#endif
  }
  c->demand_rounds += demand_rounds;
  c->parse_rounds += rounds;
  c->tmark("parse");
  const uint32_t k0 = job.tok_lo / PCHUNK, k1 = job.final ? nch : job.tok_hi / PCHUNK, nk = k1 - k0;
  if (nk == 0) { c->err = "empty shard"; return -1; }
  hipLaunchKernelGGL(k_tok_count, dim3((nch + 255) / 256), dim3(256), 0, st, nch, W.spec_cnt, W.fix_cnt, W.take_from, W.counts);
  exclusive_scan_u32(st, W.counts + k0, W.offsets, W.scan_sums, W.n_changed, nk);
  struct { uint32_t total; ExitState ex, warm; } h;
  h.ex = ExitState{(uint32_t)n, SYNC_F}; h.warm = ExitState{0, SYNC_F};
  hipMemcpyAsync(&h.total, W.n_changed, 4, hipMemcpyDeviceToHost, st);
  if (!job.final) hipMemcpyAsync(&h.ex, W.true_exits + (k1 - 1), sizeof(ExitState), hipMemcpyDeviceToHost, st);
  if (k0 > 0) hipMemcpyAsync(&h.warm, W.true_exits + (k0 - 1), sizeof(ExitState), hipMemcpyDeviceToHost, st);
  if (hip_check(c, hipStreamSynchronize(st), "tok_scan")) return ZADA_E_HIP_;
  uint32_t *dst_atoms = job.dst_atoms, *dst_apos = job.dst_apos;
  if (h.total > job.cap_atoms) {
    if (!job.grow_atoms) { c->err = "atom array overflow"; return -2; }
    if (int rg = job.grow_atoms(h.total, &dst_atoms, &dst_apos)) return rg;
  }
  hipLaunchKernelGGL(k_tok_compact, dim3((nk + 3) / 4), dim3(256), 0, st, nk, W.spec_tok, W.spec_cnt, W.fix_tok, W.fix_cnt,
                     W.take_from, W.start_pos, W.offsets, dst_atoms, dst_apos, k0, job.apos_bias, W.fix_stride);
  c->tmark("compact");
  res->ntok = h.total; res->exit = h.ex; res->warm = h.warm;
  return hip_check(c, hipGetLastError(), "lz_shard");
}

}
```

Measured before the change: 9378.

## Split match records into full and sparse quarter planes to halve parser traffic

```diff
diff --git a/__graft_entry__.py b/__graft_entry__.py
--- a/__graft_entry__.py
+++ b/__graft_entry__.py
@@ -50,6 +50,8 @@
                     os.path.join(ROOT, "tests", "unlegacy", "unlegacy_model.c")], check=True)
     subprocess.run(["g++", "-O2", "-std=c++17", "-fPIC", "-shared", "-o", os.path.join(ROOT, "tests", "zip_legacy", "libzip_legacy_plan_host.so"),
                     os.path.join(ROOT, "tests", "zip_legacy", "zip_legacy_plan_host.cpp")], check=True)
+    subprocess.run(["g++", "-O2", "-std=c++17", "-fPIC", "-shared", "-o", os.path.join(ROOT, "tests", "match_records", "libquarter_dep.so"),
+                    os.path.join(ROOT, "tests", "match_records", "quarter_dep.cpp")], check=True)
     za = importlib.import_module("zip-ada_amd")
     za.load_library()
     return None
diff --git a/zip-ada_amd/csrc/zada_api.hip b/zip-ada_amd/csrc/zada_api.hip
--- a/zip-ada_amd/csrc/zada_api.hip
+++ b/zip-ada_amd/csrc/zada_api.hip
@@ -161,7 +161,7 @@
   W.cd_cap = cap / 256 + 4096; A(cd_list, W.cd_cap + W.cd_cap / 4);
   for (int l = 0; l < NLEVELS; l++) A(dplane[l], cap + 64);
   A(dlim, cap + 64); A(dlim_bits, cap / 32 + 64);
-  A(M, cap + 64);
+  A(M, 2 * (cap + 64));
   A(SK, nseg32 * 32768); A(idxK, cap + 64); A(cntK, cap + 64);
   W.fix_stride = c->knob_fix_stride > 0 ? (uint32_t)c->knob_fix_stride : FIX_STRIDE_SMALL;
   if (W.fix_stride > PTOK_STRIDE) W.fix_stride = PTOK_STRIDE;
diff --git a/zip-ada_amd/csrc/zada_internal.h b/zip-ada_amd/csrc/zada_internal.h
--- a/zip-ada_amd/csrc/zada_internal.h
+++ b/zip-ada_amd/csrc/zada_internal.h
@@ -125,7 +125,7 @@
   uint32_t *cd_list = nullptr; uint64_t cd_cap = 0;
   uint16_t *dplane[NLEVELS] = {}; uint32_t *dlim = nullptr, *dlim_bits = nullptr;
   uint16_t *SK = nullptr, *idxK = nullptr, *cntK = nullptr;
-  MatchPair *M = nullptr;
+  uint32_t *M = nullptr;
   uint32_t *spec_tok = nullptr, *fix_tok = nullptr;
   uint32_t fix_stride = 0;
   uint32_t *spec_cnt = nullptr, *fix_cnt = nullptr, *take_from = nullptr, *start_pos = nullptr;
diff --git a/zip-ada_amd/csrc/zada_logic.h b/zip-ada_amd/csrc/zada_logic.h
--- a/zip-ada_amd/csrc/zada_logic.h
+++ b/zip-ada_amd/csrc/zada_logic.h
@@ -123,6 +123,9 @@
 template <typename F> struct has_byte { template <typename U> static auto test(int) -> decltype(((U *)0)->byte(0u), char()); template <typename U> static long test(...); static const bool value = sizeof(test<F>(0)) == 1; };
 template <typename F> ZADA_HD typename std::enable_if<has_byte<typename std::remove_reference<F>::type>::value, uint32_t>::type fetch_byte(F &f, const uint8_t *, uint32_t p) { return f.byte(p); }
 template <typename F> ZADA_HD typename std::enable_if<!has_byte<typename std::remove_reference<F>::type>::value, uint32_t>::type fetch_byte(F &, const uint8_t *in, uint32_t p) { return in[p]; }
+template <typename F> struct has_rec { template <typename U> static auto test(int) -> decltype(((U *)0)->rec(0u, false), char()); template <typename U> static long test(...); static const bool value = sizeof(test<F>(0)) == 1; };
+template <typename F> ZADA_HD typename std::enable_if<has_rec<typename std::remove_reference<F>::type>::value, MatchPair>::type fetch_rec(F &f, uint32_t p, bool need_quarter) { return f.rec(p, need_quarter); }
+template <typename F> ZADA_HD typename std::enable_if<!has_rec<typename std::remove_reference<F>::type>::value, MatchPair>::type fetch_rec(F &f, uint32_t p, bool) { return f(p); }
 struct DirectSink { uint32_t *tok; uint32_t &ntok; ZADA_HD void push(uint32_t t) { tok[ntok++] = t; } };
 struct CappedSink { uint32_t *tok; uint32_t &ntok; uint32_t cap; uint32_t *overflow; ZADA_HD void push(uint32_t t) { if (ntok < cap) tok[ntok] = t; else if (overflow) *overflow = 1u; ntok++; } };
 template <typename Sink, typename OnTop, typename OnGuess, typename Fetch>
@@ -137,9 +140,10 @@
     const bool srch = parse_searches(s, io.cfg, la);
     uint32_t m = 0;
     if (srch) {
-      const MatchPair mm = fetch(s.p);
+      const bool needq = parse_need_quarter(s, io.cfg);
+      const MatchPair mm = fetch_rec(fetch, s.p, needq);
       if (mm.full & M_GUESS) on_guess(s.p, mm.full, mm.quarter, s.mlen);
-      m = (parse_need_quarter(s, io.cfg) ? mm.quarter : mm.full) & M_VALUE;
+      m = (needq ? mm.quarter : mm.full) & M_VALUE;
     }
     const uint32_t bb = s.avail ? fetch_byte(fetch, io.in, s.p - 1) : 0;
     const uint32_t t = parse_step(s, m, srch, bb);
diff --git a/zip-ada_amd/csrc/zada_lz.hip b/zip-ada_amd/csrc/zada_lz.hip
--- a/zip-ada_amd/csrc/zada_lz.hip
+++ b/zip-ada_amd/csrc/zada_lz.hip
@@ -962,10 +962,22 @@
 
 #define LDS_U16(b, o) ((uint32_t)(b)[(o)] | ((uint32_t)(b)[(o) + 1] << 8))
 
+struct MatchPlanes {
+  uint32_t *F, *Q;
+  __device__ __forceinline__ void put_exact(uint64_t p, uint32_t full, uint32_t quarter) const {
+    if (quarter != full) { Q[p] = quarter; F[p] = full | M_HAVEQ; } else F[p] = full;
+  }
+  __device__ __forceinline__ MatchPair get(uint64_t p) const {
+    MatchPair r; r.full = F[p];
+    r.quarter = (r.full & (M_GUESS | M_HAVEQ)) ? Q[p] : (r.full & M_VALUE);
+    return r;
+  }
+};
+
 __global__ void __launch_bounds__(1024) k_match(const uint8_t *__restrict__ in, Layout L,
                                                 const uint16_t *__restrict__ prevd,
                                                 DistPlanes dp,
-                                                MatchPair *__restrict__ M,
+                                                MatchPlanes M,
                                                 int nice_cfg, int budget, unsigned long long *__restrict__ dbg,
                                                 uint16_t *__restrict__ resume, int short_budget) {
   extern __shared__ __attribute__((aligned(16))) uint8_t smem[];
@@ -1046,8 +1058,7 @@
             ok = chain_ok && b_ < nice_ && d0 <= lf;
             if (!ok) {
               const uint32_t packed = b_ >= 3 ? ((uint32_t)b_ << 16) | bd_ : 0u;
-              MatchPair r; r.full = packed; r.quarter = (hq || !chain_ok) ? qbest : packed;
-              M[B + k] = r;
+              M.put_exact(B + k, packed, (hq || !chain_ok) ? qbest : packed);
             }
             bool inner = false;
 #ifndef ZADA_NO_INNER
@@ -1172,8 +1183,7 @@
           if (wi - ncur > lim_full) fin = true;
         }
         if (fin) {
-          MatchPair r; r.full = packed; r.quarter = have_q ? rq : packed;
-          M[B + kpos] = r;
+          M.put_exact(B + kpos, packed, have_q ? rq : packed);
           state = 0;
         } else {
           cur = ncur;
@@ -1183,8 +1193,8 @@
     }
     if (state == 1 && ++age >= mybudget) {
       const uint32_t packed = best >= 3 ? ((uint32_t)best << 16) | bdist : 0u;
-      MatchPair r; r.full = packed | M_GUESS | (have_q ? M_HAVEQ : 0u); r.quarter = (have_q ? rq : packed) | (M_BEAT_MAX << M_BEAT_SHIFT);
-      M[B + kpos] = r;
+      M.Q[B + kpos] = (have_q ? rq : packed) | (M_BEAT_MAX << M_BEAT_SHIFT);
+      M.F[B + kpos] = packed | M_GUESS | (have_q ? M_HAVEQ : 0u);
       resume[B + kpos] = (uint16_t)(wi - cur);
       state = 0;
     }
@@ -1224,7 +1234,7 @@
 constexpr int DM_LDS = DM_WBYTES + DMB * 2 + DM_SLICE * (int)sizeof(ScanDesc) + 64;
 static_assert(MB % DMB == 0 && DM_WBYTES % 16 == 0 && sizeof(ScanDesc) == 32, "demand blocks tile the first-pass blocks");
 __global__ void __launch_bounds__(DM_THREADS, 6) k_match_demand(const uint8_t *__restrict__ in, Layout L, DistPlanes dp, RunPtrs rp,
-                                                             const uint16_t *__restrict__ tailsK, MatchPair *__restrict__ M, int nice_cfg,
+                                                             const uint16_t *__restrict__ tailsK, MatchPlanes M, int nice_cfg,
                                                              const uint32_t *__restrict__ blk_demand, uint32_t *__restrict__ dbits, uint8_t *__restrict__ chg,
                                                              const ExitState *__restrict__ spec_exits, const uint16_t *__restrict__ resume, bool use_beat) {
   if (blk_demand[xcd_block()] == 0) return;
@@ -1260,8 +1270,7 @@
   if (!STAGE_BESIDE) stage((uint32_t)tid, DM_THREADS);
   const uint8_t *win8 = (const uint8_t *)win;
   auto store_result = [&](uint64_t p, uint32_t full, uint32_t quarter, uint32_t og_full, uint32_t og_quarter, bool reach) {
-    MatchPair r; r.full = full; r.quarter = quarter;
-    M[p] = r;
+    M.put_exact(p, full, quarter);
     const uint32_t beat = use_beat ? og_quarter >> M_BEAT_SHIFT : 0u, ogq = og_quarter & M_VALUE;
     if ((og_full & M_BYSPEC) && ((full != (og_full & M_VALUE) && (full >> 16) > beat) || (quarter != ogq && (quarter >> 16) > beat))) {
       const uint64_t ch = p / PCHUNK;
@@ -1304,7 +1313,7 @@
       uint32_t dl[NLEVELS];
 #pragma unroll
       for (int l = 0; l < NLEVELS; l++) dl[l] = dp.d[l][p];
-      const MatchPair og = M[p];
+      const MatchPair og = M.get(p);
       const uint32_t idx1 = rp.idx[p], c1 = rp.cnt[p];
       uint32_t t = 0xFFFFu;
       if (!seg_first) {
@@ -1452,27 +1461,27 @@
   }
 }
 
-__global__ void k_demand_all(Layout L, MatchPair *__restrict__ M, uint32_t *__restrict__ blk_demand, uint32_t *__restrict__ dbits) {
+__global__ void k_demand_all(Layout L, uint32_t *__restrict__ F, uint32_t *__restrict__ blk_demand, uint32_t *__restrict__ dbits) {
   const uint64_t p = (uint64_t)blockIdx.x * blockDim.x + threadIdx.x;
   if (p >= L.n || p >= lay_end(L, p >> 15)) return;
-  const uint32_t f = M[p].full;
+  const uint32_t f = F[p];
   if (f & M_GUESS) {
-    if (!(f & M_DEMAND)) M[p].full = f | M_DEMAND | M_BYSPEC;
+    if (!(f & M_DEMAND)) F[p] = f | M_DEMAND | M_BYSPEC;
     atomicOr(&dbits[p >> 5], 1u << (p & 31));
     blk_demand[p / DMB] = 1;
   }
 }
 
 struct DemandMarker {
-  MatchPair *M; uint32_t *blk_demand; uint32_t *n_demand; uint32_t by;
+  MatchPlanes M; uint32_t *blk_demand; uint32_t *n_demand; uint32_t by;
   bool track = false;
   uint32_t *dbits;
   __device__ void operator()(uint32_t p, uint32_t full, uint32_t quarter, uint32_t beat) const {
     if (track && (beat < M_BEAT_MAX ? beat : M_BEAT_MAX) < (quarter >> M_BEAT_SHIFT))
-      __hip_atomic_fetch_min(&M[p].quarter, (quarter & M_VALUE) | ((beat < M_BEAT_MAX ? beat : M_BEAT_MAX) << M_BEAT_SHIFT), __ATOMIC_RELAXED, __HIP_MEMORY_SCOPE_AGENT);
+      __hip_atomic_fetch_min(&M.Q[p], (quarter & M_VALUE) | ((beat < M_BEAT_MAX ? beat : M_BEAT_MAX) << M_BEAT_SHIFT), __ATOMIC_RELAXED, __HIP_MEMORY_SCOPE_AGENT);
     const uint32_t want = M_DEMAND | by;
     if ((full & want) == want) return;
-    M[p].full = full | want;
+    M.F[p] = full | want;
     atomicOr(&dbits[p >> 5], 1u << (p & 31));
     blk_demand[p / DMB] = 1;
     *n_demand = 1;
@@ -1480,30 +1489,43 @@
 };
 
 #ifndef ZADA_PS_BWORDS
-#define ZADA_PS_BWORDS 16
+#define ZADA_PS_BWORDS 8
 #endif
 #ifndef ZADA_PS_TOKS
 #define ZADA_PS_TOKS 8
 #endif
 constexpr uint32_t PS_BWORDS = ZADA_PS_BWORDS, PS_TOKS = ZADA_PS_TOKS;
 static_assert((PS_BWORDS == 8 || PS_BWORDS == 16) && (PS_TOKS == 4 || PS_TOKS == 8), "line sizes of the parser's LDS caches");
+#ifndef ZADA_PS_RECS
+#define ZADA_PS_RECS 8
+#endif
+constexpr uint32_t PS_RECS = ZADA_PS_RECS;
+static_assert(PS_RECS == 8 || PS_RECS == 16, "full words per cached line of match records");
+__device__ __forceinline__ MatchPair rec_of(uint32_t f, const uint32_t *__restrict__ Q, uint32_t p, bool need_quarter, bool track) {
+  MatchPair r; r.full = f;
+  if ((need_quarter && (f & M_HAVEQ)) || (track && (f & M_GUESS))) r.quarter = Q[p];
+  else r.quarter = f & M_VALUE;
+  return r;
+}
 struct LineFetch {
-  const MatchPair *M; uint64_t *slot;
-  uint32_t tag;
-  __device__ MatchPair operator()(uint32_t p) {
-    const uint32_t t = p >> 3;
+  MatchPlanes M; uint32_t *slot;
+  uint32_t tag; bool track;
+  __device__ MatchPair rec(uint32_t p, bool need_quarter) {
+    constexpr uint32_t SH = PS_RECS == 16 ? 4 : 3;
+    const uint32_t t = p >> SH;
     if (t != tag) {
-      const uint4 *src = (const uint4 *)(M + ((uint64_t)t << 3));
-      const uint4 a = src[0], b = src[1], c = src[2], d = src[3];
-      slot[0 * 64] = (uint64_t)a.x | ((uint64_t)a.y << 32); slot[1 * 64] = (uint64_t)a.z | ((uint64_t)a.w << 32);
-      slot[2 * 64] = (uint64_t)b.x | ((uint64_t)b.y << 32); slot[3 * 64] = (uint64_t)b.z | ((uint64_t)b.w << 32);
-      slot[4 * 64] = (uint64_t)c.x | ((uint64_t)c.y << 32); slot[5 * 64] = (uint64_t)c.z | ((uint64_t)c.w << 32);
-      slot[6 * 64] = (uint64_t)d.x | ((uint64_t)d.y << 32); slot[7 * 64] = (uint64_t)d.z | ((uint64_t)d.w << 32);
+      const uint4 *src = (const uint4 *)(M.F + ((uint64_t)t << SH));
+      const uint4 a = src[0], b = src[1];
+      slot[0 * 64] = a.x; slot[1 * 64] = a.y; slot[2 * 64] = a.z; slot[3 * 64] = a.w;
+      slot[4 * 64] = b.x; slot[5 * 64] = b.y; slot[6 * 64] = b.z; slot[7 * 64] = b.w;
+      if (PS_RECS == 16) {
+        const uint4 c = src[2], d = src[3];
+        slot[8 * 64] = c.x; slot[9 * 64] = c.y; slot[10 * 64] = c.z; slot[11 * 64] = c.w;
+        slot[12 * 64] = d.x; slot[13 * 64] = d.y; slot[14 * 64] = d.z; slot[15 * 64] = d.w;
+      }
       tag = t;
     }
-    const uint64_t v = slot[(p & 7u) * 64];
-    MatchPair r; r.full = (uint32_t)v; r.quarter = (uint32_t)(v >> 32);
-    return r;
+    return rec_of(slot[(p & (PS_RECS - 1u)) * 64], M.Q, p, need_quarter, track);
   }
   const uint8_t *in; uint32_t *bslot; uint32_t btag;
   __device__ uint32_t byte(uint32_t p) {
@@ -1578,10 +1600,10 @@
   uint32_t old_h = 0, old_n = 0; ExitState old_ex{0, 0};
   if (list) { old_n = spec_cnt[k]; old_ex = exits[k]; const uint32_t *ot = spec_tok + (uint64_t)k * PTOK_STRIDE; for (uint32_t i = 0; i < old_n; i++) old_h = old_h * 0x9E3779B1u + ot[i]; }
 #endif
-  __shared__ uint64_t lines[8 * 64];
+  __shared__ uint32_t lines[PS_RECS * 64];
   __shared__ uint32_t tbuf[PS_TOKS * 64];
   __shared__ uint32_t blines[PS_BWORDS * 64];
-  LineFetch lf; lf.M = io.M; lf.slot = lines + threadIdx.x; lf.tag = 0xFFFFFFFFu; lf.in = io.in; lf.bslot = blines + threadIdx.x; lf.btag = 0xFFFFFFFFu;
+  LineFetch lf; lf.M = dm.M; lf.track = dm.track; lf.slot = lines + threadIdx.x; lf.tag = 0xFFFFFFFFu; lf.in = io.in; lf.bslot = blines + threadIdx.x; lf.btag = 0xFFFFFFFFu;
   TokSink ts; ts.dst = spec_tok + (uint64_t)k * PTOK_STRIDE; ts.buf = tbuf + threadIdx.x; ts.n = 0;
   parse_spec_chunk_to(io, k, PCHUNK, ts, Fbits, Lbits, ex, dm, lf);
   ts.flush();
@@ -1599,8 +1621,13 @@
 }
 
 struct WaveExact {
-  const uint8_t *in; Layout L; DistPlanes dp; RunPtrs rp; const uint16_t *tailsK; MatchPair *M; int nice_cfg; const uint16_t *resume;
+  const uint8_t *in; Layout L; DistPlanes dp; RunPtrs rp; const uint16_t *tailsK; MatchPlanes M; int nice_cfg; const uint16_t *resume;
   __device__ __forceinline__ uint32_t g32(uint64_t o) const { return *(const u32u *)(in + o); }
+  __device__ __forceinline__ void publish(uint64_t p, uint32_t full, uint32_t quarter) const {
+    uint32_t f = full;
+    if (quarter != full) { M.Q[p] = quarter; f |= M_HAVEQ; }
+    __hip_atomic_store(&M.F[p], f, __ATOMIC_RELEASE, __HIP_MEMORY_SCOPE_AGENT);
+  }
   __device__ MatchPair search(uint64_t p, MatchPair og) const {
     const int lane = threadIdx.x & 63;
     const uint64_t seg = p >> 15, n = lay_end(L, seg);
@@ -1652,7 +1679,7 @@
     if (!(chain_ok && bst < nice && n1 + n2 > 0)) {
       const uint32_t packed = bst >= 3 ? ((uint32_t)bst << 16) | bd : 0u;
       r.full = packed; r.quarter = !chain_ok ? rqq : (hq ? rqq : packed);
-      if (lane == 0) M[p] = r;
+      if (lane == 0) publish(p, r.full, r.quarter);
       return r;
     }
     const uint16_t *sprev = rp.S + ((seg << 15) - 32768);
@@ -1699,19 +1726,19 @@
     }
     const uint32_t packed = bst >= 3 ? ((uint32_t)bst << 16) | bd : 0u;
     r.full = packed; r.quarter = hq ? rqq : packed;
-    if (lane == 0) M[p] = r;
+    if (lane == 0) publish(p, r.full, r.quarter);
     return r;
   }
 };
 
 constexpr uint32_t PX_RECS = PCHUNK + 320;
 struct WaveFetch {
-  const uint64_t *recs; uint32_t c0; const MatchPair *Mg; const WaveExact *wx;
-  __device__ MatchPair operator()(uint32_t p) const {
-    MatchPair r;
-    if (p - c0 < PX_RECS) { const uint64_t v = recs[p - c0]; r.full = (uint32_t)v; r.quarter = (uint32_t)(v >> 32); }
-    else r = Mg[p];
-    if (r.full & M_GUESS) r = wx->search(p, r);
+  const uint32_t *recs; uint32_t c0; const WaveExact *wx;
+  __device__ MatchPair rec(uint32_t p, bool need_quarter) const {
+    const uint32_t f = p - c0 < PX_RECS ? recs[p - c0] : __hip_atomic_load(&wx->M.F[p], __ATOMIC_ACQUIRE, __HIP_MEMORY_SCOPE_AGENT);
+    MatchPair r; r.full = f;
+    r.quarter = ((f & M_HAVEQ) && (need_quarter || (f & M_GUESS))) ? wx->M.Q[p] : (f & M_VALUE);
+    if (f & M_GUESS) r = wx->search(p, r);
     return r;
   }
 };
@@ -1723,7 +1750,7 @@
 __global__ void __launch_bounds__(64 * PX_WAVES) k_parse_spec_exact(ParseIO io, uint32_t nchunks, uint32_t *__restrict__ spec_tok, uint32_t *__restrict__ spec_cnt,
                                                                      uint32_t *__restrict__ Fbits, uint32_t *__restrict__ Lbits, ExitState *__restrict__ exits,
                                                                      WaveExact wx, const uint32_t *__restrict__ list, const uint32_t *__restrict__ list_n, uint32_t exact_max) {
-  __shared__ uint64_t recs[PX_WAVES][PX_RECS];
+  __shared__ uint32_t recs[PX_WAVES][PX_RECS];
   const int lane = threadIdx.x & 63, w = threadIdx.x >> 6;
   const uint32_t nl = *list_n, stride = gridDim.x * PX_WAVES;
   if (nl > exact_max) return;
@@ -1734,12 +1761,13 @@
     if (io.segend) cio.n = io.segend[((uint64_t)k * PCHUNK) >> 15] & 0x7FFFFFFFu;
     const uint32_t c0 = k * PCHUNK;
     {
-      const uint64_t *src = (const uint64_t *)(io.M + c0);
+      const uint32_t *src = wx.M.F + c0;
       const uint32_t have = (uint64_t)c0 + PX_RECS <= io.n ? PX_RECS : (uint32_t)(io.n - c0);
-      for (uint32_t j = lane; j < have; j += 64) recs[w][j] = src[j];
+      for (uint32_t j = lane; j < have; j += 64) recs[w][j] = __hip_atomic_load(src + j, __ATOMIC_RELAXED, __HIP_MEMORY_SCOPE_AGENT);
+      __builtin_amdgcn_fence(__ATOMIC_ACQUIRE, "agent");
     }
     __builtin_amdgcn_wave_barrier();
-    WaveFetch wf; wf.recs = recs[w]; wf.c0 = c0; wf.Mg = io.M; wf.wx = &wx;
+    WaveFetch wf; wf.recs = recs[w]; wf.c0 = c0; wf.wx = &wx;
     WaveSink ts; ts.dst = spec_tok + (uint64_t)k * PTOK_STRIDE; ts.n = 0;
     ExitState ex;
     parse_spec_chunk_to(cio, k, PCHUNK, ts, Fbits, Lbits, ex, NoGuess(), wf);
@@ -1748,6 +1776,10 @@
   }
 }
 
+struct PlaneFetch {
+  MatchPlanes M; bool track;
+  __device__ MatchPair rec(uint32_t p, bool need_quarter) const { return rec_of(M.F[p], M.Q, p, need_quarter, track); }
+};
 __global__ void k_parse_fix(ParseIO io, uint32_t nchunks, const uint32_t *__restrict__ spec_tok, const uint32_t *__restrict__ spec_cnt,
                             const uint32_t *__restrict__ Fbits, const uint32_t *__restrict__ Lbits,
                             const ExitState *__restrict__ spec_exits, ExitState *__restrict__ true_exits,
@@ -1769,7 +1801,7 @@
   ExitState new_exit;
   uint32_t ntok = 0, take = 0, u0 = 0;
   parse_fix_chunk(io, k, PCHUNK, entry, spec_tok + (uint64_t)k * PTOK_STRIDE, spec_cnt[k], Fbits, Lbits, spec_exits[k],
-                  fix_tok + (uint64_t)k * fix_stride, ntok, take, u0, new_exit, dm, DirectFetch{io.M}, fix_stride, fix_overflow);
+                  fix_tok + (uint64_t)k * fix_stride, ntok, take, u0, new_exit, dm, PlaneFetch{dm.M, dm.track}, fix_stride, fix_overflow);
   fix_cnt[k] = ntok;
   take_from[k] = take;
   start_pos[k] = u0;
@@ -1781,7 +1813,7 @@
   }
 }
 
-__global__ void __launch_bounds__(64) k_fix_forward(ParseIO io, uint32_t nchunks, ExitState *__restrict__ true_exits,
+__global__ void __launch_bounds__(64) k_fix_forward(ParseIO io, const uint32_t *__restrict__ F, uint32_t nchunks, ExitState *__restrict__ true_exits,
                                                     uint8_t *__restrict__ dirty_out, uint32_t *__restrict__ n_changed) {
   const uint32_t k = n_changed[1];
   if (k >= nchunks || 258 < io.cfg.lazy || io.segend) return;
@@ -1791,7 +1823,7 @@
   for (uint64_t q0 = e0.pos;; q0 += 258ull * 64) {
     const uint64_t q = q0 + 258ull * lane;
     bool good = false;
-    if (q + 258 <= io.n) { const uint32_t f = io.M[q].full; good = !(f & M_GUESS) && ((f & M_VALUE) >> 16) == 258u; }
+    if (q + 258 <= io.n) { const uint32_t f = F[q]; good = !(f & M_GUESS) && ((f & M_VALUE) >> 16) == 258u; }
     const unsigned long long bad = ~__ballot(good);
     const int nvalid = bad ? __ffsll((long long)bad) - 1 : 64;
     if (lane <= nvalid && (lane > 0 || q0 != e0.pos)) {
@@ -2071,11 +2103,12 @@
   hipMemsetAsync(W.blk_demand, 0, (size_t)nbd * 4, st);
   hipMemsetAsync(W.dbits, 0, (size_t)nbd * (DMB / 8), st);
   hipMemsetAsync(W.n_demand, 0, 4, st);
-  hipLaunchKernelGGL(k_match, dim3(nbm), dim3(1024), MATCH_LDS, st, W.in, L, W.lprev[NLEVELS - 1], dpl, W.M, cfg.nice,
+  const MatchPlanes mp{W.M, W.M + (W.cap_n + 64)};
+  hipLaunchKernelGGL(k_match, dim3(nbm), dim3(1024), MATCH_LDS, st, W.in, L, W.lprev[NLEVELS - 1], dpl, mp, cfg.nice,
                      budget_env, (unsigned long long *)W.dbg, W.lprev[0], budget_env > c->knob_inner_budget ? c->knob_inner_budget : 0);
   c->tmark("match");
-  ParseIO io; io.in = W.in; io.n = n; io.M = W.M; io.cfg = cfg; io.segend = job.segend;
-  DemandMarker dm; dm.M = W.M; dm.blk_demand = W.blk_demand; dm.n_demand = W.n_demand; dm.by = M_BYSPEC; dm.dbits = W.dbits;
+  ParseIO io; io.in = W.in; io.n = n; io.M = nullptr; io.cfg = cfg; io.segend = job.segend;
+  DemandMarker dm; dm.M = mp; dm.blk_demand = W.blk_demand; dm.n_demand = W.n_demand; dm.by = M_BYSPEC; dm.dbits = W.dbits;
   DemandMarker dmf = dm; dmf.by = 0;
   int rounds = 0, demand_rounds = 0;
   bool valve_used = false;
@@ -2094,7 +2127,7 @@
       hipLaunchKernelGGL(k_list_flagged, dim3((nch + 1023) / 1024), dim3(1024), 0, st, W.chg, nch, W.offsets, W.n_changed + 2);
       const uint32_t exact_max = c->knob_exact_respec > 0 ? (uint32_t)c->knob_exact_respec : 0u;
       if (exact_max) {
-        WaveExact wx; wx.in = W.in; wx.L = L; wx.dp = dpl; wx.rp = rpt; wx.tailsK = W.ltails[NLEVELS - 1]; wx.M = W.M; wx.nice_cfg = cfg.nice; wx.resume = W.lprev[0];
+        WaveExact wx; wx.in = W.in; wx.L = L; wx.dp = dpl; wx.rp = rpt; wx.tailsK = W.ltails[NLEVELS - 1]; wx.M = mp; wx.nice_cfg = cfg.nice; wx.resume = W.lprev[0];
         hipLaunchKernelGGL(k_parse_spec_exact, dim3(256 * 5), dim3(64 * PX_WAVES), 0, st, io, nch, W.spec_tok, W.spec_cnt, W.Fbits, W.Lbits, W.spec_exits,
                            wx, (const uint32_t *)W.offsets, (const uint32_t *)(W.n_changed + 2), exact_max);
       }
@@ -2115,7 +2148,7 @@
       hipLaunchKernelGGL(k_parse_fix, dim3((nch + 63) / 64), dim3(64), 0, st, io, nch,
                          W.spec_tok, W.spec_cnt, W.Fbits, W.Lbits, W.spec_exits, W.true_exits, W.fix_tok, W.fix_cnt,
                          W.take_from, W.start_pos, W.dirty[cur], W.dirty[cur ^ 1], W.n_changed, dmf, entry0, W.fix_stride, W.n_changed + 6);
-      hipLaunchKernelGGL(k_fix_forward, dim3(1), dim3(64), 0, st, io, nch, W.true_exits, W.dirty[cur ^ 1], W.n_changed);
+      hipLaunchKernelGGL(k_fix_forward, dim3(1), dim3(64), 0, st, io, (const uint32_t *)mp.F, nch, W.true_exits, W.dirty[cur ^ 1], W.n_changed);
       uint32_t changed = 0, fix_ovf = 0;
       hipMemcpyAsync(&changed, W.n_changed, 4, hipMemcpyDeviceToHost, st);
       hipMemcpyAsync(&ndem, W.n_demand, 4, hipMemcpyDeviceToHost, st);
@@ -2155,9 +2188,9 @@
     hipMemsetAsync(W.chg, 0, nch, st);
     if ((demand_rounds == max_rounds || slow) && !valve_used) {
       valve_used = true;
-      hipLaunchKernelGGL(k_demand_all, dim3((uint32_t)((n + 255) / 256)), dim3(256), 0, st, L, W.M, W.blk_demand, W.dbits);
-    }
-    hipLaunchKernelGGL(k_match_demand, dim3(nbd), dim3(DM_THREADS), DM_LDS, st, W.in, L, dpl, rpt, W.ltails[NLEVELS - 1], W.M, cfg.nice,
+      hipLaunchKernelGGL(k_demand_all, dim3((uint32_t)((n + 255) / 256)), dim3(256), 0, st, L, mp.F, W.blk_demand, W.dbits);
+    }
+    hipLaunchKernelGGL(k_match_demand, dim3(nbd), dim3(DM_THREADS), DM_LDS, st, W.in, L, dpl, rpt, W.ltails[NLEVELS - 1], mp, cfg.nice,
                        W.blk_demand, W.dbits, W.chg, W.spec_exits, W.lprev[0], beat_valid);
     hipMemsetAsync(W.blk_demand, 0, (size_t)nbd * 4, st);
 #ifdef ZADA_DM_STATS
```

Result: no change. 9389, median of 2 (+0.1%).
